# gist-ailab/QuBER

Hardware: AMD Instinct MI355X
Metric: refined masks/sec on 640x480 RGB-D (N=20 inst) (higher is better)
Workload: dtype f32; 1 GPU; batch=16 640x480 RGB-D, 20 initial instances/frame, ResNet-50 RGB-D refiner (boundary-error -> fg/centre/offset), encode+network+grouping+mask extraction; parallelism=dp1, hipgraph=False, foreground_filter=False

## Files before the change

### include/quber_hip.h

```cpp
#ifndef QUBER_HIP_H
#define QUBER_HIP_H

#include <stddef.h>
#include <stdint.h>

#ifdef __cplusplus
extern "C" {
#endif

typedef struct quber_ctx quber_ctx;

typedef struct quber_config {
    int32_t height, width;
    int32_t max_batch;
    int32_t max_instances;
    int32_t resnet_depth;
    int32_t res5_dilation;
    int32_t backbone_fusion_layers;
    int32_t head_fusion_layers;
    int32_t error_classes;
    int32_t gaussian_sigma;
    int32_t nms_kernel;
    int32_t top_k;
    int32_t stuff_area;
// ... 80 lines not shown

int quber_relabel_panoptic(quber_ctx* ctx, const float* dev_panoptic, const float* dev_labels, const int32_t* dev_count,
                           int32_t batch, int32_t mirror, int32_t* dev_ids, void* stream);
int quber_overlap_masks(quber_ctx* ctx, const uint8_t* dev_masks, const int32_t* dev_ids, int32_t batch, int32_t n_masks,
                        int32_t n_ids, uint32_t* dev_table, uint32_t* dev_area, void* stream);
int quber_overlap_ids(quber_ctx* ctx, const int32_t* dev_a, const int32_t* dev_b, int32_t batch, int32_t n_a, int32_t n_b,
                      uint32_t* dev_table, void* stream);

int quber_cleanup_ids(quber_ctx* ctx, int32_t* dev_ids, int32_t batch, int32_t n_ids, int32_t connectivity, int32_t keep_largest,
                      int32_t min_island_area, int32_t max_hole_area, uint32_t* dev_report, void* stream);
int quber_cleanup_postprocess(quber_ctx* ctx, const float* dev_logits, int32_t n_planes, int32_t batch, float* dev_panoptic,
                              const float* dev_labels, const int32_t* dev_count, float* dev_scores, float* dev_boxes,
                              int32_t connectivity, int32_t keep_largest, int32_t min_island_area, int32_t max_hole_area,
                              uint32_t* dev_report, void* stream);

int quber_perturb_masks(quber_ctx* ctx, const uint8_t* dev_masks, int32_t batch, int32_t n_masks, const int32_t* dev_programs,
                        int32_t n_ops, int32_t ops_per_round, const double* dev_iou_targets, uint8_t* dev_out, uint32_t* dev_report,
                        int32_t placement, void* stream);

int quber_mask_nms(quber_ctx* ctx, const uint8_t* dev_masks, const float* dev_scores, int32_t batch, int32_t n_masks, float thresh,
                   int32_t on_top, uint8_t* dev_out_masks, int32_t* dev_ids, int32_t* dev_source, float* dev_out_scores,
                   int32_t* dev_report, void* stream);

int quber_zoom_rois(quber_ctx* ctx, const int32_t* dev_ids, int32_t batch, int32_t n_ids, float padding, int32_t* dev_rois, void* stream);
int quber_zoom_crop(quber_ctx* ctx, const uint8_t* dev_bgr, const uint8_t* dev_depth, const int32_t* dev_ids, const int32_t* dev_slots,
                    const int32_t* dev_rois, int32_t batch, int32_t n_ids, int32_t n_slots, int32_t crop, uint8_t* dev_bgr_crop,
                    uint8_t* dev_depth_crop, uint8_t* dev_mask_crop, void* stream);
int quber_zoom_paste(quber_ctx* ctx, const int32_t* dev_crop_ids, const float* dev_crop_scores, const uint32_t* dev_table,
                     const uint32_t* dev_area, const uint8_t* dev_depth_crop, const int32_t* dev_slots, const int32_t* dev_rois,
                     int32_t batch, int32_t n_ids, int32_t n_slots, int32_t crop, int32_t n_crop_ids, float min_overlap, int32_t max_inst,
                     int32_t* dev_out_ids, uint8_t* dev_out_masks, int32_t* dev_source, float* dev_out_scores, float* dev_boxes,
                     int32_t* dev_report, void* stream);

int64_t quber_contingency_workspace_bytes(int32_t cap);
int quber_label_contingency(const int32_t* dev_pred, const int32_t* dev_gt, int64_t n_pixels, int32_t cap,
                            void* dev_workspace, void* stream);

int64_t quber_boundary_workspace_bytes(int32_t h, int32_t w, int32_t n_masks);
int quber_boundary_overlap(const int32_t* dev_pred, const int32_t* dev_gt, int32_t h, int32_t w, const int32_t* dev_labels,
                           int32_t n_pred, int32_t n_gt, int32_t bound_pix, void* dev_workspace, uint32_t* dev_out,
                           void* stream);

int64_t quber_eval_batch_workspace_bytes(int32_t batch, int32_t h, int32_t w, int32_t cap, int32_t with_boundary);
int quber_eval_batch(const int32_t* dev_pred, const int32_t* dev_gt, int32_t batch, int32_t h, int32_t w, int32_t cap, int32_t bound_pix,
                     int32_t with_boundary, int32_t placement, void* dev_workspace, void* dev_out, void* stream);
int quber_munkres_batch(const double* dev_score, const int32_t* dev_rows, const int32_t* dev_cols, int32_t batch, int32_t cap,
                        int32_t placement, void* dev_workspace, int32_t* dev_assign, int32_t* dev_status, void* stream);

int quber_foreground_filter(const float* dev_fg_logits, int32_t n_classes, int32_t fg_class, const uint8_t* dev_masks,
                            int32_t batch, int32_t n_masks, int64_t hw, uint8_t* dev_fg_mask, uint64_t* dev_counts,
                            void* stream);

int quber_normalize_depth(const void* dev_depth, int32_t is_float32, int64_t n_pixels, double min_val, double max_val,
                          uint8_t* dev_out3, uint8_t* dev_zero, void* stream);

int quber_resize_u8(const uint8_t* dev_src, int32_t src_h, int32_t src_w, int32_t channels, uint8_t* dev_dst,
                    int32_t dst_h, int32_t dst_w, int32_t linear, void* stream);

int quber_inpaint_telea_u8(const uint8_t* host_img, const uint8_t* host_mask, int32_t h, int32_t w, int32_t radius,
                           uint8_t* host_out);
int quber_inpaint_depth_u8(const uint8_t* host_depth3, int32_t h, int32_t w, int32_t kernel, uint8_t* host_out3);
int64_t quber_inpaint_depth_workspace_bytes(int32_t batch, int32_t h, int32_t w);
int quber_inpaint_depth_device(const uint8_t* dev_depth3, int32_t batch, int32_t h, int32_t w, int32_t kernel, void* dev_workspace,
                               int64_t workspace_bytes, uint8_t* dev_out3, void* stream);

int quber_debug_tensor(quber_ctx* ctx, const char* name, float** dev_ptr, int32_t* dims4, int32_t* channel_stride);
int32_t quber_debug_tensor_elem_size(quber_ctx* ctx, const char* name);
double quber_forward_flops(quber_ctx* ctx);
double quber_forward_flops_executed(quber_ctx* ctx);
double quber_forward_flops_padding(quber_ctx* ctx);
int quber_set_option(quber_ctx* ctx, int32_t key, int32_t value);
int quber_get_option(quber_ctx* ctx, int32_t key, int32_t* value);
void quber_set_tuning(int32_t key, int32_t value);
int32_t quber_debug_persistent_segments(int32_t tiles, int32_t blocks, int32_t k_slices, int32_t min_share, int32_t block,
                                        int32_t* out4, int32_t cap);
int32_t quber_debug_persistent_fixup(int32_t tiles, int32_t blocks, int32_t k_slices, int32_t min_share, int32_t xcd, int32_t j,
                                     int32_t* tile, int32_t* slots, int32_t cap);
int quber_num_ops(quber_ctx* ctx);
int quber_op_info(quber_ctx* ctx, int index, const char** name, int32_t* kind, double* flops, int32_t* launches);
int quber_op_conv2d(const float* dev_x, int32_t batch, int32_t h, int32_t w, int32_t cin, const float* dev_w_oihw,
                    int32_t cout, int32_t ksize, int32_t stride, int32_t pad, int32_t dil, const float* dev_scale,
                    const float* dev_shift, const float* dev_residual, int32_t relu, float* dev_packed_scratch,
                    float* dev_y, void* stream);
int quber_op_conv1x1_f16(const void* dev_x, int32_t batch, int32_t h, int32_t w, int32_t cin, const void* dev_w_oi,
                         int32_t cout, const float* dev_scale, const float* dev_shift, const void* dev_residual,
                         int32_t relu, void* dev_y, void* stream);
int quber_op_conv2d_f16(const void* dev_x, int32_t batch, int32_t h, int32_t w, int32_t cin, const void* dev_w_packed,
                        int32_t cout, int32_t ksize, int32_t stride, int32_t pad, int32_t dil, int32_t kmode,
                        const float* dev_scale, const float* dev_shift, const void* dev_residual, int32_t relu,
                        double* dev_gn_sums, int32_t gn_groups, void* dev_y, void* stream);
int quber_op_conv1x1_dual(const float* dev_y, const float* dev_x, int32_t batch, int32_t oh, int32_t ow, int32_t mid,
                          int32_t h2, int32_t w2, int32_t cin, int32_t stride, const float* dev_w, const float* dev_shift,
                          const float* dev_ones, int32_t cout, int32_t relu, float* dev_out, void* stream);
int quber_op_conv3x3_winograd(const float* dev_x, int32_t batch, int32_t h, int32_t w, int32_t cin,
                              const float* dev_w_oihw, int32_t cout, int32_t dil, int32_t m, const float* dev_scale,
                              const float* dev_shift,
                              int32_t relu, float* dev_u_scratch, float* dev_ws, int64_t ws_floats, float* dev_y,
                              void* stream);
int quber_op_groupnorm(const float* dev_x, int32_t batch, int32_t h, int32_t w, int32_t c, int32_t groups,
                       const float* dev_gamma, const float* dev_beta, float eps, int32_t relu,
                       double* dev_stats_scratch, float* dev_y, void* stream);
int quber_op_bilinear(const float* dev_x, int32_t batch, int32_t h, int32_t w, int32_t c, int32_t oh, int32_t ow,
                      float* dev_y, void* stream);
int quber_op_maxpool3x3s2(const float* dev_x, int32_t batch, int32_t h, int32_t w, int32_t c, float* dev_y,
                          void* stream);
int32_t quber_debug_gn_pixels_per_block(int32_t hw, int32_t c, int32_t batch, int32_t groups_of_launch, int32_t stats_pass);
int quber_op_gn_stats(const void* dev_x, int32_t x_cs, int64_t x_gs, int32_t es, int32_t batch, int32_t h, int32_t w, int32_t c,
                      int32_t groups_of_launch, int32_t groups, double* dev_stats, int32_t zero, void* stream);
int quber_op_gn_apply(const void* dev_x, int32_t x_cs, int64_t x_gs, int32_t x_es, void* dev_y, int32_t y_cs, int64_t y_gs, int32_t y_es,
                      int32_t batch, int32_t h, int32_t w, int32_t c, int32_t groups_of_launch, int32_t groups, const double* dev_stats,
                      const float* dev_gamma, const float* dev_beta, int32_t param_gs, float eps, int32_t relu, void* stream);
int quber_op_maxpool_view(const void* dev_x, int32_t x_cs, int64_t x_gs, int32_t x_es, void* dev_y, int32_t y_cs, int64_t y_gs, int32_t y_es,
                          int32_t batch, int32_t h, int32_t w, int32_t c, int32_t groups_of_launch, void* stream);
int quber_op_bilinear_view(const void* dev_x, int32_t x_cs, int32_t x_es, void* dev_y, int32_t y_cs, int32_t y_es, int32_t batch, int32_t h,
                           int32_t w, int32_t c, int32_t oh, int32_t ow, void* stream);
int quber_op_avgpool(const void* dev_x, int32_t x_cs, int32_t x_es, void* dev_y, int32_t y_cs, int32_t y_es, int32_t batch, int32_t h, int32_t w,
                     int32_t c, void* stream);
int quber_op_add_channels(const void* dev_a, int32_t a_cs, int32_t a_es, const void* dev_b, int32_t b_cs, int32_t b_es, void* dev_y, int32_t y_cs,
                          int32_t y_es, int32_t batch, int32_t h, int32_t w, int32_t c, void* stream);
int quber_op_copy_channels(const void* dev_x, int32_t x_cs, int32_t x_es, void* dev_y, int32_t y_cs, int32_t y_es, int32_t batch, int32_t h,
                           int32_t w, int32_t c, void* stream);
int quber_op_predictors(int32_t n, const void* const* dev_feat, const float* const* dev_w, const float* const* dev_bias, void* const* dev_act_dst,
                        const int32_t* cout, const int32_t* q_ch0, const int32_t* act, int32_t c, int32_t feat_cs, int32_t es, int32_t batch,
                        int32_t h, int32_t w, float* dev_q, int32_t q_nch, int32_t act_cs, void* stream);
int quber_op_upsample_logits(const float* dev_q, float* dev_out, int32_t batch, int32_t nch, int32_t h, int32_t w, int32_t scale, int32_t oh,
                             int32_t ow, uint32_t mul_mask, void* stream);
int quber_op_preprocess(const uint8_t* dev_bgr, const uint8_t* dev_depth, const float* dev_offsets, void* dev_x, int32_t x_c, int32_t es,
                        int32_t batch, int32_t batch_cap, int32_t h, int32_t w, const float* mean6, const float* std6, int32_t streams,
                        void* stream);
int quber_op_lmff_preprocess(const uint8_t* dev_bgr, const uint8_t* dev_depth, int64_t pixels, float* dev_x, void* stream);
int quber_op_lmff_dwconv(const float* dev_x, int32_t x_cs, float* dev_y, int32_t y_cs, int32_t batch, int32_t h, int32_t w, int32_t c, int32_t dil,
                         const float* dev_w9, const float* dev_scale, const float* dev_shift, const float* dev_slope, void* stream);
int quber_op_lmff_pool(const float* dev_x, int32_t x_cs, float* dev_y, int32_t y_cs, int32_t batch, int32_t h, int32_t w, int32_t c, int32_t oh,
                       int32_t ow, int32_t mode, void* stream);
int quber_op_lmff_affine(const float* dev_a, int32_t a_cs, const float* dev_b, int32_t b_cs, float* dev_y, int32_t y_cs, int32_t batch, int32_t h,
                         int32_t w, int32_t c, const float* dev_scale, const float* dev_shift, const float* dev_slope, void* stream);
int quber_op_lmff_pmca(const float* dev_x, int32_t x_cs, int32_t batch, int32_t h, int32_t w, int32_t c, const float* dev_w2x2, const float* dev_fc0,
                       const float* dev_alpha, const float* dev_fc2, float* dev_wts, double* dev_sums, void* stream);
int quber_op_lmff_scale(const float* dev_x, int32_t x_cs, const float* dev_wts, float* dev_y, int32_t y_cs, int32_t batch, int32_t h, int32_t w,
                        int32_t c, void* stream);
int quber_op_lmff_gate(const float* dev_o, int32_t o_cs, const float* dev_att, int32_t att_cs, float* dev_q, int32_t batch, int32_t h, int32_t w,
                       int32_t c, void* stream);
int quber_op_group_pixels(const float* dev_logits, int32_t n_planes, int32_t batch, int32_t h, int32_t w, int32_t cap,
                          const int32_t* dev_centers, const int32_t* dev_ncenters, uint8_t* dev_ids, uint32_t* dev_area,
                          void* stream);

#ifdef __cplusplus
}
#endif
#endif
```

### quber_amd/_lib.py

```python
import ctypes as C
import os

_HERE = os.path.dirname(os.path.abspath(__file__))
LIB_PATH = os.environ.get("QUBER_LIB") or os.path.join(_HERE, "libquber_hip.so")


class QuberConfig(C.Structure):
    _fields_ = [
        ("height", C.c_int32), ("width", C.c_int32), ("max_batch", C.c_int32), ("max_instances", C.c_int32),
        ("resnet_depth", C.c_int32), ("res5_dilation", C.c_int32), ("backbone_fusion_layers", C.c_int32),
        ("head_fusion_layers", C.c_int32), ("error_classes", C.c_int32), ("gaussian_sigma", C.c_int32),
        ("nms_kernel", C.c_int32), ("top_k", C.c_int32), ("stuff_area", C.c_int32),
        ("min_instance_area", C.c_int32), ("label_divisor", C.c_int32), ("with_network", C.c_int32),
        ("center_threshold", C.c_float), ("boundary_ratio", C.c_float),
        ("pixel_mean", C.c_float * 6), ("pixel_std", C.c_float * 6),
        ("eee_mask_on", C.c_int32), ("eee_boundary_on", C.c_int32), ("hierarchical", C.c_int32),
        ("fusion_feat", C.c_int32), ("fusion_pred", C.c_int32), ("n_levels", C.c_int32),
        ("level_heads", (C.c_int32 * 5) * 5), ("fusion_add", C.c_int32), ("streams", C.c_int32),
        ("compute_dtype", C.c_int32), ("encode_legacy_f32", C.c_int32),
        ("convs_dim", C.c_int32), ("head_channels", C.c_int32),
    ]


class QuberError(RuntimeError):
    pass


_P = C.c_void_p
_I = C.c_int32
SIGNATURES = {
    "quber_default_config": (None, [C.POINTER(QuberConfig)]),
    "quber_last_error": (C.c_char_p, []),
    "quber_version": (C.c_char_p, []),
    "quber_create": (C.c_int, [C.POINTER(QuberConfig), C.POINTER(_P)]),
    "quber_destroy": (None, [_P]),
    "quber_set_weight": (C.c_int, [_P, C.c_char_p, _P, C.c_int64]),
    "quber_finalize_weights": (C.c_int, [_P]),
    "quber_num_weights": (C.c_int, [_P]),
    "quber_weight_spec": (C.c_int, [_P, C.c_int, C.POINTER(C.c_char_p), C.POINTER(C.c_int64)]),
    "quber_encode_initial_masks": (C.c_int, [_P, _P, _I, _I, _P, _P]),
    "quber_encode_label_map": (C.c_int, [_P, _P, _I, _I, _P, _P]),
    "quber_workspace_bytes": (C.c_int64, [_P]),
    "quber_explicit_error_maps": (C.c_int, [_P, _P, _I, _P, _I, _I, _P, _P]),
    "quber_forward": (C.c_int, [_P, _P, _P, _P, _I, _P, _P]),
    "quber_forward_profiled": (C.c_int, [_P, _P, _P, _P, _I, _P, _P, C.POINTER(C.c_double * 3), C.POINTER(_I * 3)]),
    "quber_profile_begin": (C.c_int, [_P]),
    "quber_profile_end": (C.c_int, [_P, _P]),
    "quber_profile_num_stages": (C.c_int, [_P]),
    "quber_profile_stage": (C.c_int, [_P, C.c_int, C.POINTER(C.c_char_p), C.POINTER(C.c_double), C.POINTER(C.c_double),
                                      C.POINTER(C.c_double), C.POINTER(_I)]),
    "quber_postprocess": (C.c_int, [_P, _P, _I, _I, _P, _P, _P, _P, _P, _P, _P, _P]),
    "quber_extract_masks": (C.c_int, [_P, _P, _P, _I, _I, _P, _P]),
    "quber_tta_flip_inputs": (C.c_int, [_P, _P, _P, _P, _I, _I, _P]),
    "quber_tta_merge": (C.c_int, [_P, _P, _I, _I, _P, _P]),
    "quber_error_decode": (C.c_int, [_P, _P, _I, _I, _I, _I, _P, _P, _P]),
    "quber_error_mask_hist": (C.c_int, [_P, _P, _P, _I, _I, _I, _P, _P]),
    "quber_error_score": (C.c_int, [_P, _P, _P, _I, _I, _I, _I, _P, _P]),
    "quber_error_overlay": (C.c_int, [_P, _P, _P, _I, C.c_uint32, C.c_uint32, C.c_uint32, C.c_uint32, _P, _P]),
    "quber_relabel_panoptic": (C.c_int, [_P, _P, _P, _P, _I, _I, _P, _P]),
    "quber_overlap_masks": (C.c_int, [_P, _P, _P, _I, _I, _I, _P, _P, _P]),
    "quber_overlap_ids": (C.c_int, [_P, _P, _P, _I, _I, _I, _P, _P]),
    "quber_cleanup_ids": (C.c_int, [_P, _P, _I, _I, _I, _I, _I, _I, _P, _P]),
    "quber_cleanup_postprocess": (C.c_int, [_P, _P, _I, _I, _P, _P, _P, _P, _P, _I, _I, _I, _I, _P, _P]),
    "quber_perturb_masks": (C.c_int, [_P, _P, _I, _I, _P, _I, _I, _P, _P, _P, _I, _P]),
    "quber_mask_nms": (C.c_int, [_P, _P, _P, _I, _I, C.c_float, _I, _P, _P, _P, _P, _P, _P]),
    "quber_zoom_rois": (C.c_int, [_P, _P, _I, _I, C.c_float, _P, _P]),
    "quber_zoom_crop": (C.c_int, [_P, _P, _P, _P, _P, _P, _I, _I, _I, _I, _P, _P, _P, _P]),
    "quber_zoom_paste": (C.c_int, [_P, _P, _P, _P, _P, _P, _P, _P, _I, _I, _I, _I, _I, C.c_float, _I, _P, _P, _P, _P, _P, _P, _P]),
    "quber_contingency_workspace_bytes": (C.c_int64, [_I]),
    "quber_label_contingency": (C.c_int, [_P, _P, C.c_int64, _I, _P, _P]),
    "quber_boundary_workspace_bytes": (C.c_int64, [_I, _I, _I]),
    "quber_boundary_overlap": (C.c_int, [_P, _P, _I, _I, _P, _I, _I, _I, _P, _P, _P]),
    "quber_eval_batch_workspace_bytes": (C.c_int64, [_I, _I, _I, _I, _I]),
    "quber_eval_batch": (C.c_int, [_P, _P, _I, _I, _I, _I, _I, _I, _I, _P, _P, _P]),
    "quber_munkres_batch": (C.c_int, [_P, _P, _P, _I, _I, _I, _P, _P, _P, _P]),
    "quber_foreground_filter": (C.c_int, [_P, _I, _I, _P, _I, _I, C.c_int64, _P, _P, _P]),
    "quber_normalize_depth": (C.c_int, [_P, _I, C.c_int64, C.c_double, C.c_double, _P, _P, _P]),
    "quber_inpaint_telea_u8": (C.c_int, [_P, _P, _I, _I, _I, _P]),
    "quber_inpaint_depth_u8": (C.c_int, [_P, _I, _I, _I, _P]),
    "quber_inpaint_depth_workspace_bytes": (C.c_int64, [_I, _I, _I]),
    "quber_inpaint_depth_device": (C.c_int, [_P, _I, _I, _I, _I, _P, C.c_int64, _P, _P]),
    "quber_resize_u8": (C.c_int, [_P, _I, _I, _I, _P, _I, _I, _I, _P]),
    "quber_debug_tensor": (C.c_int, [_P, C.c_char_p, C.POINTER(_P), C.POINTER(_I * 4), C.POINTER(_I)]),
    "quber_debug_tensor_elem_size": (C.c_int32, [_P, C.c_char_p]),
    "quber_forward_flops": (C.c_double, [_P]),
    "quber_forward_flops_executed": (C.c_double, [_P]),
    "quber_forward_flops_padding": (C.c_double, [_P]),
    "quber_set_tuning": (None, [_I, _I]),
    "quber_set_option": (C.c_int, [_P, _I, _I]),
    "quber_get_option": (C.c_int, [_P, _I, C.POINTER(_I)]),
    "quber_num_ops": (C.c_int, [_P]),
    "quber_op_info": (C.c_int, [_P, C.c_int, C.POINTER(C.c_char_p), C.POINTER(_I), C.POINTER(C.c_double), C.POINTER(_I)]),
    "quber_debug_persistent_segments": (C.c_int32, [_I, _I, _I, _I, _I, _P, _I]),
    "quber_debug_persistent_fixup": (C.c_int32, [_I, _I, _I, _I, _I, _I, _P, _P, _I]),
    "quber_op_conv1x1_f16": (C.c_int, [_P, _I, _I, _I, _I, _P, _I, _P, _P, _P, _I, _P, _P]),
    "quber_op_conv2d_f16": (C.c_int, [_P, _I, _I, _I, _I, _P, _I, _I, _I, _I, _I, _I, _P, _P, _P, _I, _P, _I, _P, _P]),
    "quber_op_conv1x1_dual": (C.c_int, [_P, _P, _I, _I, _I, _I, _I, _I, _I, _I, _P, _P, _P, _I, _I, _P, _P]),
    "quber_op_conv2d": (C.c_int, [_P, _I, _I, _I, _I, _P, _I, _I, _I, _I, _I, _P, _P, _P, _I, _P, _P, _P]),
    "quber_op_conv3x3_winograd": (C.c_int, [_P, _I, _I, _I, _I, _P, _I, _I, _I, _P, _P, _I, _P, _P, C.c_int64, _P, _P]),
    "quber_op_groupnorm": (C.c_int, [_P, _I, _I, _I, _I, _I, _P, _P, C.c_float, _I, _P, _P, _P]),
    "quber_op_bilinear": (C.c_int, [_P, _I, _I, _I, _I, _I, _I, _P, _P]),
    "quber_op_maxpool3x3s2": (C.c_int, [_P, _I, _I, _I, _I, _P, _P]),
    "quber_debug_gn_pixels_per_block": (C.c_int32, [_I, _I, _I, _I, _I]),
    "quber_op_gn_stats": (C.c_int, [_P, _I, C.c_int64, _I, _I, _I, _I, _I, _I, _I, _P, _I, _P]),
    "quber_op_gn_apply": (C.c_int, [_P, _I, C.c_int64, _I, _P, _I, C.c_int64, _I, _I, _I, _I, _I, _I, _I, _P, _P, _P, _I, C.c_float, _I, _P]),
    "quber_op_maxpool_view": (C.c_int, [_P, _I, C.c_int64, _I, _P, _I, C.c_int64, _I, _I, _I, _I, _I, _I, _P]),
    "quber_op_bilinear_view": (C.c_int, [_P, _I, _I, _P, _I, _I, _I, _I, _I, _I, _I, _I, _P]),
    "quber_op_avgpool": (C.c_int, [_P, _I, _I, _P, _I, _I, _I, _I, _I, _I, _P]),
    "quber_op_add_channels": (C.c_int, [_P, _I, _I, _P, _I, _I, _P, _I, _I, _I, _I, _I, _I, _P]),
    "quber_op_copy_channels": (C.c_int, [_P, _I, _I, _P, _I, _I, _I, _I, _I, _I, _P]),
    "quber_op_predictors": (C.c_int, [_I, _P, _P, _P, _P, _P, _P, _P, _I, _I, _I, _I, _I, _I, _P, _I, _I, _P]),
    "quber_op_upsample_logits": (C.c_int, [_P, _P, _I, _I, _I, _I, _I, _I, _I, C.c_uint32, _P]),
    "quber_op_preprocess": (C.c_int, [_P, _P, _P, _P, _I, _I, _I, _I, _I, _I, _P, _P, _I, _P]),
    "quber_op_group_pixels": (C.c_int, [_P, _I, _I, _I, _I, _I, _P, _P, _P, _P, _P]),
    "quber_op_lmff_preprocess": (C.c_int, [_P, _P, C.c_int64, _P, _P]),
    "quber_op_lmff_dwconv": (C.c_int, [_P, _I, _P, _I, _I, _I, _I, _I, _I, _P, _P, _P, _P, _P]),
    "quber_op_lmff_pool": (C.c_int, [_P, _I, _P, _I, _I, _I, _I, _I, _I, _I, _I, _P]),
    "quber_op_lmff_affine": (C.c_int, [_P, _I, _P, _I, _P, _I, _I, _I, _I, _I, _P, _P, _P, _P]),
    "quber_op_lmff_pmca": (C.c_int, [_P, _I, _I, _I, _I, _I, _P, _P, _P, _P, _P, _P, _P]),
    "quber_op_lmff_scale": (C.c_int, [_P, _I, _P, _P, _I, _I, _I, _I, _I, _P]),
    "quber_op_lmff_gate": (C.c_int, [_P, _I, _P, _I, _P, _I, _I, _I, _I, _P]),
}

_lib = None


def load():
    global _lib
    if _lib is not None:
        return _lib
    if not os.path.exists(LIB_PATH):
        raise QuberError(
            f"{LIB_PATH} not found: build it with `make -C quber_amd/csrc` (or __graft_entry__.build()); "
            "quber_amd has no CPU fallback")
    import torch
    lib = C.CDLL(LIB_PATH)
    for name, (res, args) in SIGNATURES.items():
        fn = getattr(lib, name)
        fn.restype = res
        fn.argtypes = args
    mode = os.environ.get("QUBER_WINOGRAD", "auto").lower()
    if mode not in ("auto", "f6", "f4", "f2", "off"):
        raise QuberError(f"QUBER_WINOGRAD={mode!r}: expected auto, f6, f4, f2 or off")
    lib.quber_set_tuning(6, 1 if mode == "off" else 0)
    lib.quber_set_tuning(9, {"f2": 2, "f4": 4, "f6": 6}.get(mode, 0))
    if "QUBER_PERSIST" in os.environ:
        lib.quber_set_tuning(13, int(os.environ["QUBER_PERSIST"]))
    _lib = lib
    return lib


def check(rc):
    if rc != 0:
        raise QuberError(load().quber_last_error().decode())
```

### quber_amd/csrc/api.hip

```cpp
#include "plan.h"

#include <optional>

using namespace quber;

namespace quber { int wf_read_stamps(unsigned long long* dst, int n), h8_read_stamps(unsigned long long* dst, int n), x8_read_stamps(unsigned long long* dst, int n); }

int quber::check_cfg(const quber_config& c) {
    if (c.height <= 0 || c.width <= 0) return fail("height and width must be positive");
    if (c.with_network && (c.height < 16 || c.width < 16)) return fail("frames smaller than 16 x 16 are not supported");
    if (c.with_network == 2) {
        if (c.height % 8 || c.width % 8) return fail("LMFFNet needs height and width to be multiples of 8");
        return c.max_batch >= 1 ? 0 : fail("max_batch must be >= 1");
    }
    if (c.max_batch < 1) return fail("max_batch must be >= 1");
    if (c.max_instances < 1) return fail("max_instances must be >= 1");
    if (c.resnet_depth != 50 && c.resnet_depth != 101 && c.resnet_depth != 152) return fail("resnet_depth must be 50, 101 or 152");
    if (c.res5_dilation != 1 && c.res5_dilation != 2 && c.res5_dilation != 4) return fail("res5_dilation must be 1, 2 or 4");
    if (c.res5_dilation == 1) return fail("res5_dilation 1 (output stride 32) is not supported by this build");
    if (c.error_classes < 2 || c.error_classes > 4) return fail("error_classes must be 2..4");
    if (c.streams != 1 && c.streams != 2) return fail("streams must be 1 or 2");
    if (c.with_network == 1 && c.convs_dim != 128 && c.convs_dim != 256) return fail("convs_dim must be 128 or 256");
    if (c.with_network == 1 && c.head_channels != 32 && c.head_channels != 64) return fail("head_channels must be 32 or 64");
    if (c.compute_dtype < 0 || c.compute_dtype > 3)
// ... 186 lines not shown
#endif

int32_t quber_debug_persistent_segments(int32_t tiles, int32_t blocks, int32_t k_slices, int32_t min_share, int32_t block, int32_t* out4, int32_t cap) {
    return quber::conv_persistent_segments(tiles, blocks, k_slices, min_share, block, out4, cap);
}
int32_t quber_debug_persistent_fixup(int32_t tiles, int32_t blocks, int32_t k_slices, int32_t min_share, int32_t xcd, int32_t j, int32_t* tile, int32_t* slots, int32_t cap) {
    return quber::conv_persistent_fixup(tiles, blocks, k_slices, min_share, xcd, j, tile, slots, cap);
}

int quber_profile_begin(quber_ctx* c) {
    if (!c) return fail("null context");
    if (!c->prof) c->prof.reset(new quber::Profiler());
    c->prof->recs.clear(); c->prof->sums.clear(); c->prof->used = 0;
    quber::g_prof = c->prof.get();
    return 0;
}

int quber_profile_end(quber_ctx* c, void* stream) {
    if (!c || !c->prof || quber::g_prof != c->prof.get()) return fail("quber_profile_end without quber_profile_begin");
    quber::g_prof = nullptr;
    QB_CHECK(hipStreamSynchronize((hipStream_t)stream));
    quber::Profiler& p = *c->prof;
    p.sums.assign(p.tags.size(), quber::StageSum());
    for (size_t i = 0; i < p.tags.size(); ++i) p.sums[i].name = p.tags[i];
    for (const quber::ProfRec& r : p.recs) {
        float ms = 0.f;
        QB_CHECK(hipEventElapsedTime(&ms, r.e0, r.e1));
        quber::StageSum& s = p.sums[r.tag];
        s.ms += ms; s.bytes += r.bytes; s.flops += r.flops; s.launches += 1;
    }
    return 0;
}

int quber_profile_num_stages(quber_ctx* c) { return (c && c->prof) ? (int)c->prof->sums.size() : 0; }

int quber_profile_stage(quber_ctx* c, int i, const char** name, double* ms, double* bytes, double* flops, int32_t* launches) {
    if (!c || !c->prof || i < 0 || i >= (int)c->prof->sums.size()) return fail("stage index out of range");
    const quber::StageSum& s = c->prof->sums[i];
    *name = s.name.c_str(); *ms = s.ms; *bytes = s.bytes; *flops = s.flops; *launches = s.launches;
    return 0;
}

int quber_num_ops(quber_ctx* c) { return c ? (int)c->ops.size() : 0; }
int quber_op_info(quber_ctx* c, int i, const char** name, int32_t* kind, double* flops, int32_t* launches) {
    if (!c || i < 0 || i >= (int)c->ops.size()) return fail("op index out of range");
    const Op& o = c->ops[i];
    *name = o.name.c_str(); *kind = o.kind; *flops = o.flops; *launches = o.launches;
    return 0;
}

int quber_encode_initial_masks(quber_ctx* c, const uint8_t* masks, int32_t batch, int32_t n, float* out, void* stream) {
    if (check_batch(c, batch)) return -1;
    if (n > c->cfg.max_instances) return fail("more initial masks than max_instances");
    if (!masks && n > 0) return fail("null masks");
    return launch_encode(masks, batch, n, c->cfg.height, c->cfg.width, c->gauss, c->cfg.gaussian_sigma, c->cfg.encode_legacy_f32, c->enc_ws, out, (hipStream_t)stream);
}

int quber_encode_label_map(quber_ctx* c, const int32_t* labels, int32_t batch, int32_t n, float* out, void* stream) {
    if (check_batch(c, batch)) return -1;
    if (n > c->cfg.max_instances) return fail("more instances than max_instances");
    if (!labels && n > 0) return fail("null label map");
    return launch_encode_labels(labels, batch, n, c->cfg.height, c->cfg.width, c->gauss, c->cfg.gaussian_sigma, c->cfg.encode_legacy_f32, c->enc_ws, out, c->enc_bad, (hipStream_t)stream);
}

int64_t quber_workspace_bytes(quber_ctx* c) { return c ? (int64_t)c->alloc_bytes : 0; }

int quber_explicit_error_maps(quber_ctx* c, const uint8_t* init, int32_t n_init, const uint8_t* gt, int32_t n_gt, int32_t batch, uint8_t* out, void* stream) {
    if (check_batch(c, batch)) return -1;
    const int H = c->cfg.height, W = c->cfg.width;
    int d = (int)rint((double)c->cfg.boundary_ratio * sqrt((double)H * H + (double)W * W));
    if (d < 1) d = 1;
    return launch_errmaps(init, n_init, gt, n_gt, batch, c->cfg.max_instances > 0 ? c->cfg.max_instances : 1, H, W, d, c->err_ws, out, (hipStream_t)stream);
}

static int forward_begin(quber_ctx* c, const char* who, std::optional<quber::TuneScope>& scope, const uint8_t* bgr, const uint8_t* depth,
                         const float* offs, int batch, float* logits, bool lmff_own, bool rest_ok, const char* null_msg, hipStream_t st) {
    if (check_batch(c, batch)) return -1;
    if (!c->finalized) return fail(std::string(who) + " before quber_finalize_weights");
    scope.emplace(&c->tune);
    if (lmff_own && c->cfg.with_network == 2) return 1;
    if (!bgr || (!depth && c->cfg.streams == 2) || !offs || !logits || !rest_ok) return fail(null_msg);
    c->cur_out = logits;
    c->cur_bgr = bgr; c->cur_depth = depth; c->cur_off = offs;
    return c->stem_fused ? 0 : launch_preprocess(bgr, depth, offs, c->X, batch, c->cfg.max_batch, c->cfg.height, c->cfg.width,
                                                 c->cfg.pixel_mean, c->cfg.pixel_std, c->cfg.streams, st);
}

int quber_forward(quber_ctx* c, const uint8_t* bgr, const uint8_t* depth, const float* offs, int32_t batch, float* logits, void* stream) {
    hipStream_t st = (hipStream_t)stream;
    std::optional<quber::TuneScope> tscope;
    int rc = forward_begin(c, "quber_forward", tscope, bgr, depth, offs, batch, logits, true, true, "null tensor", st);
    if (rc == 1) {
        if (!bgr || !depth || !logits) return fail("null tensor");
        c->cur_out = logits;
        int r2 = launch_lmff_preprocess(bgr, depth, (long)batch * c->cfg.height * c->cfg.width, c->X.p, st);
        for (size_t i = 0; !r2 && i < c->ops.size(); ++i)
            if (!c->ops[i].ctl) r2 = c->ops[i].run(batch, st);
        return r2;
    }
    if (rc) return rc;
    c->lanes_on = c->lanes_built && tune().lanes && batch <= (c->cfg.compute_dtype == 0 || c->cfg.compute_dtype == 3 ? LANE_BATCH_F32 : LANE_BATCH) && c->lane_stream[1] != nullptr &&
                  quber::g_prof == nullptr;
    auto lane_used = [&](int l) { return c->lanes_on && l > 0; };
    for (auto& op : c->ops) {
        if (op.ctl == 1) {
            if (lane_used(op.lane)) {
                QB_CHECK(hipEventRecord(c->lane_fork[op.lane], st));
                QB_CHECK(hipStreamWaitEvent(c->lane_stream[op.lane], c->lane_fork[op.lane], 0));
            }
            continue;
        }
        if (op.ctl == 2) {
            if (lane_used(op.lane)) {
                QB_CHECK(hipEventRecord(c->lane_join[op.lane], c->lane_stream[op.lane]));
                QB_CHECK(hipStreamWaitEvent(st, c->lane_join[op.lane], 0));
            }
            continue;
        }
        c->lane_now = lane_used(op.lane) ? op.lane : 0;
        rc = op.run(batch, c->lane_now ? c->lane_stream[op.lane] : st);
        if (rc) return rc;
    }
    c->lane_now = 0;
    c->lanes_on = false;
    return 0;
}

int quber_forward_profiled(quber_ctx* c, const uint8_t* bgr, const uint8_t* depth, const float* offs, int32_t batch,
                           float* logits, void* stream, double* kind_ms, int32_t* kind_launches) {
    hipStream_t st = (hipStream_t)stream;
    std::optional<quber::TuneScope> tscope;
    int rc = forward_begin(c, "quber_forward_profiled", tscope, bgr, depth, offs, batch, logits, false, kind_ms && kind_launches, "null argument", st);
    if (rc) return rc;
    const size_t n = c->ops.size();
    if (c->prof_events.size() < 2 * n) {
        const size_t old = c->prof_events.size();
        c->prof_events.resize(2 * n);
        for (size_t i = old; i < 2 * n; ++i) QB_CHECK(hipEventCreate(&c->prof_events[i]));
    }
    c->lanes_on = false;
    for (size_t i = 0; i < n; ++i) {
        QB_CHECK(hipEventRecord(c->prof_events[2 * i], st));
        if (!c->ops[i].ctl) {
            rc = c->ops[i].run(batch, st);
            if (rc) return rc;
        }
        QB_CHECK(hipEventRecord(c->prof_events[2 * i + 1], st));
    }
    QB_CHECK(hipStreamSynchronize(st));
    for (int k = 0; k < OP_KINDS; ++k) { kind_ms[k] = 0.0; kind_launches[k] = 0; }
    for (size_t i = 0; i < n; ++i) {
        float ms = 0.f;
        QB_CHECK(hipEventElapsedTime(&ms, c->prof_events[2 * i], c->prof_events[2 * i + 1]));
        kind_ms[c->ops[i].kind] += ms;
        kind_launches[c->ops[i].kind] += 1;
    }
    return 0;
}

int quber_postprocess(quber_ctx* c, const float* logits, int32_t n_planes, int32_t batch, float* pan, int32_t* count,
                      float* labels, float* scores, float* boxes, int32_t* centers, int32_t* ncenters, void* stream) {
    if (check_batch(c, batch)) return -1;
    PostCfg pc;
    pc.threshold = c->cfg.center_threshold; pc.nms_kernel = c->cfg.nms_kernel; pc.top_k = c->cfg.top_k;
    pc.stuff_area = c->cfg.stuff_area; pc.min_area = c->cfg.min_instance_area; pc.label_divisor = c->cfg.label_divisor;
    pc.cap = c->cfg.top_k;
// ... 220 lines not shown
int quber_label_contingency(const int32_t* pred, const int32_t* gt, int64_t n_pixels, int32_t cap, void* workspace,
                            void* stream) {
    if (!pred || !gt || !workspace || n_pixels < 1 || cap < 1 || cap > 1024) return fail("bad argument to quber_label_contingency");
    return launch_contingency(pred, gt, n_pixels, cap, workspace, (hipStream_t)stream);
}

int64_t quber_boundary_workspace_bytes(int32_t h, int32_t w, int32_t n_masks) {
    return (int64_t)boundary_ws_bytes(h, w, n_masks);
}

int quber_boundary_overlap(const int32_t* pred, const int32_t* gt, int32_t h, int32_t w, const int32_t* labels, int32_t n_pred,
                           int32_t n_gt, int32_t bound_pix, void* workspace, uint32_t* out, void* stream) {
    if (!pred || !gt || !labels || !workspace || !out || h < 1 || w < 1) return fail("bad argument to quber_boundary_overlap");
    return launch_boundary_overlap(pred, gt, h, w, labels, n_pred, n_gt, bound_pix, workspace, out, (hipStream_t)stream);
}

int64_t quber_eval_batch_workspace_bytes(int32_t batch, int32_t h, int32_t w, int32_t cap, int32_t with_boundary) {
    if (batch < 1 || h < 1 || w < 1 || cap < 1 || cap > 256) return 0;
    return (int64_t)eval_batch_ws_bytes(batch, h, w, cap, with_boundary);
}

int quber_eval_batch(const int32_t* pred, const int32_t* gt, int32_t batch, int32_t h, int32_t w, int32_t cap, int32_t bound_pix,
                     int32_t with_boundary, int32_t placement, void* workspace, void* out, void* stream) {
    if (!pred || !gt || !workspace || !out) return fail("quber_eval_batch: null pointer");
    if (((uintptr_t)pred & 3) || ((uintptr_t)gt & 3) || ((uintptr_t)workspace & 7) || ((uintptr_t)out & 7))
        return fail("quber_eval_batch: label maps must be 4-byte aligned, workspace and out 8-byte aligned");
    return launch_eval_batch(pred, gt, batch, h, w, cap, bound_pix, with_boundary, placement, workspace, out, (hipStream_t)stream);
}

int quber_munkres_batch(const double* score, const int32_t* rows, const int32_t* cols, int32_t batch, int32_t cap, int32_t placement,
                        void* workspace, int32_t* assign, int32_t* status, void* stream) {
    if (!score || !rows || !cols || !assign || !status) return fail("quber_munkres_batch: null pointer");
    if (((uintptr_t)score & 7) || ((uintptr_t)workspace & 7) || ((uintptr_t)rows & 3) || ((uintptr_t)cols & 3) || ((uintptr_t)assign & 3) ||
        ((uintptr_t)status & 3))
        return fail("quber_munkres_batch: misaligned pointer");
    return launch_munkres_batch(score, rows, cols, batch, cap, placement, reinterpret_cast<double*>(workspace), assign, cap, status, 1,
                                (hipStream_t)stream);
}

int quber_foreground_filter(const float* fg_logits, int32_t n_classes, int32_t fg_class, const uint8_t* masks,
                            int32_t batch, int32_t n_masks, int64_t hw, uint8_t* fg_mask, uint64_t* counts, void* stream) {
    if (!fg_logits || !fg_mask || batch < 1 || hw < 1 || n_classes < 2) return fail("bad argument to quber_foreground_filter");
    if (n_masks < 0 || n_masks > 65535) return fail("quber_foreground_filter: n_masks outside 0..65535");
    hipStream_t st = (hipStream_t)stream;
    int rc = launch_argmax_fg(fg_logits, batch, hw, n_classes, fg_class, fg_mask, st);
    if (rc || n_masks == 0) return rc;
    if (!masks || !counts) return fail("null masks / counts");
    return launch_mask_overlap(masks, fg_mask, batch, n_masks, hw, (unsigned long long*)counts, st);
}

int quber_normalize_depth(const void* depth, int32_t is_float32, int64_t n_pixels, double min_val, double max_val,
                          uint8_t* out3, uint8_t* zero, void* stream) {
    if (!depth || !out3 || n_pixels <= 0) return fail("bad argument to quber_normalize_depth");
    if (!(max_val > min_val)) return fail("normalize_depth: max_val must exceed min_val");
    return launch_normalize_depth(depth, is_float32, n_pixels, min_val, max_val, out3, zero, (hipStream_t)stream);
}

int quber_inpaint_telea_u8(const uint8_t* host_img, const uint8_t* host_mask, int32_t h, int32_t w, int32_t radius,
                           uint8_t* host_out) {
    return inpaint_telea_u8_host(host_img, host_mask, h, w, radius, host_out);
}

int quber_inpaint_depth_u8(const uint8_t* host_depth3, int32_t h, int32_t w, int32_t kernel, uint8_t* host_out3) {
    return inpaint_depth_u8_host(host_depth3, h, w, kernel, host_out3);
}

int64_t quber_inpaint_depth_workspace_bytes(int32_t batch, int32_t h, int32_t w) { return (int64_t)inpaint_depth_ws_bytes(batch, h, w); }

int quber_inpaint_depth_device(const uint8_t* dev_depth3, int32_t batch, int32_t h, int32_t w, int32_t kernel, void* dev_workspace,
                               int64_t workspace_bytes, uint8_t* dev_out3, void* stream) {
    return launch_inpaint_depth(dev_depth3, batch, h, w, kernel, dev_workspace, (size_t)workspace_bytes, dev_out3, (hipStream_t)stream);
}

int quber_resize_u8(const uint8_t* src, int32_t src_h, int32_t src_w, int32_t channels, uint8_t* dst, int32_t dst_h,
                    int32_t dst_w, int32_t linear, void* stream) {
    if (!src || !dst) return fail("bad argument to quber_resize_u8");
    return launch_resize_u8(src, src_h, src_w, channels, dst, dst_h, dst_w, linear, (hipStream_t)stream);
}

int quber_debug_tensor(quber_ctx* c, const char* name, float** ptr, int32_t* dims4, int32_t* cs) {
    if (!c || !name) return fail("null argument");
    auto it = c->taps.find(name);
    if (it == c->taps.end()) return fail(std::string("no intermediate named '") + name + "'");
    *ptr = it->second.p;
    dims4[0] = it->second.B; dims4[1] = it->second.H; dims4[2] = it->second.W; dims4[3] = it->second.C;
    *cs = it->second.cs;
    return 0;
}
int32_t quber_debug_tensor_elem_size(quber_ctx* c, const char* name) {
    if (!c || !name) return 0;
    auto it = c->taps.find(name);
    return it == c->taps.end() ? 0 : it->second.es;
}

}
```

### quber_amd/csrc/api_ops.hip

```cpp
#include "plan.h"

using namespace quber;

static float* g_op_ws = nullptr;
static int g_op_skip_rows = 0;
static int g_op_bf16 = 0;
static const size_t g_op_ws_floats = (size_t)256 << 20;
static int g_op_wino_reuse = 0;

bool quber::op_set_tuning(int key, int value) {
    if (key == 2) {
        if (value && !g_op_ws) {
            if (hipMalloc((void**)&g_op_ws, sizeof(float) * g_op_ws_floats) != hipSuccess) g_op_ws = nullptr;
        } else if (!value && g_op_ws) {
            (void)hipFree(g_op_ws);
            g_op_ws = nullptr;
        }
        return true;
    }
    if (key == 26) { g_op_wino_reuse = value; return true; }
    if (key == 12) { g_op_bf16 = value; return true; }
    if (key == 11) { g_op_skip_rows = value; return true; }
    return false;
}

static void conv_geometry(ConvP& p, int B, int h, int w, int cin, int cout, int k, int stride, int pad, int dil) {
    p.B = B; p.H = h; p.W = w; p.Cin = cin; p.in_cs = cin;
    p.OH = (h + 2 * pad - dil * (k - 1) - 1) / stride + 1;
    p.OW = (w + 2 * pad - dil * (k - 1) - 1) / stride + 1;
    p.Cout = cout; p.out_cs = cout; p.K = k * k * cin;
    p.kh = k; p.kw = k; p.stride = stride; p.pad = pad; p.dil = dil;
    p.M = B * p.OH * p.OW; p.ohw = p.OH * p.OW;
}

struct PlaneScratch {
    void* planes = nullptr;
    size_t cap = 0;
    int split(const float* w, long n, ConvP& p, const char* who, hipStream_t st) {
        const size_t need = (size_t)n * 3 * sizeof(unsigned short);
        if (need > cap) {
            if (planes) (void)hipFree(planes);
            planes = nullptr; cap = 0;
            if (hipMalloc(&planes, need) != hipSuccess) return fail(std::string(who) + ": cannot allocate the bf16x3 weight planes");
            cap = need;
        }
        const int rc = launch_split_bf16x3(w, n, planes, st);
        if (rc) return rc;
        p.w3 = planes; p.w3_plane = n;
        return 0;
    }
};

static View mkview(const float* p, int B, int h, int w, int c) {
    View v;
    v.p = const_cast<float*>(p); v.B = B; v.H = h; v.W = w; v.C = c; v.cs = c; v.gs = 0;
    return v;
}

extern "C" {

__global__ void pack_oihw_kernel(const float* __restrict__ w, int O, int I, int k, int Kpad, int kmode, float* __restrict__ out) {
    const long total = (long)O * Kpad;
    for (long i = blockIdx.x * (long)blockDim.x + threadIdx.x; i < total; i += (long)gridDim.x * blockDim.x) {
        const int o = i / Kpad, kk = i % Kpad;
        float v = 0.f;
        if (kk < k * k * I) {
            int tap, ci;
            if (kmode) {
                const int cb = kk / (k * k * 32), rem = kk % (k * k * 32);
                tap = rem / 32;
                ci = cb * 32 + rem % 32;
            } else {
                tap = kk / I;
                ci = kk % I;
            }
            v = w[((long)o * I + ci) * k * k + tap];
        }
        out[i] = v;
    }
}

int quber_op_conv2d(const float* x, int32_t B, int32_t h, int32_t w, int32_t cin, const float* w_oihw, int32_t cout, int32_t k, int32_t stride, int32_t pad, int32_t dil,
                    const float* scale, const float* shift, const float* residual, int32_t relu, float* packed, float* y, void* stream) {
    hipStream_t st = (hipStream_t)stream;
    const int Kpad = (k * k * cin + 31) / 32 * 32;
    const bool skip_rows = g_op_skip_rows && k == 3 && stride == 1 && dil > 1 && cin % 32 == 0;
    const int kmode = (k > 1 && cin % 32 == 0 && !skip_rows) ? 1 : 0;
    hipLaunchKernelGGL(pack_oihw_kernel, dim3(256), dim3(256), 0, st, w_oihw, cout, cin, k, Kpad, kmode, packed);
    ConvP p{};
    p.in = x; p.w = packed; p.scale = scale; p.shift = shift; p.res = residual; p.out = y;
    conv_geometry(p, B, h, w, cin, cout, k, stride, pad, dil);
    p.res_cs = cout; p.Kpad = Kpad; p.relu = relu;
    p.kmode = kmode; p.skip_rows = skip_rows;
    p.bf16 = g_op_bf16; p.w_gs = 0; p.ss_gs = 0;
    p.ws = g_op_ws; p.ws_floats = g_op_ws ? g_op_ws_floats : 0;
    if (g_op_bf16 == 3 && k == 1 && tune().x8) {
        static PlaneScratch scratch;
        const int rc = scratch.split(packed, (long)cout * Kpad, p, "conv2d", st);
        if (rc) return rc;
    }
    return launch_conv(p, 1, st);
}

int quber_op_conv1x1_f16(const void* x, int32_t B, int32_t h, int32_t w, int32_t cin, const void* w_oi, int32_t cout,
                         const float* scale, const float* shift, const void* residual, int32_t relu, void* y, void* stream) {
    if (cin % 64) return fail("conv1x1_f16: cin must be a multiple of 64");
    ConvP p{};
    p.in = (const float*)x; p.w = (const float*)w_oi; p.scale = scale; p.shift = shift; p.res = (const float*)residual; p.out = (float*)y;
    conv_geometry(p, B, h, w, cin, cout, 1, 1, 0, 1);
    p.res_cs = cout; p.Kpad = cin; p.relu = relu;
    p.bf16 = 2; p.es = 2;
    return launch_conv(p, 1, (hipStream_t)stream);
}

int quber_op_conv2d_f16(const void* x, int32_t B, int32_t h, int32_t w, int32_t cin, const void* w_packed, int32_t cout, int32_t ksize, int32_t stride, int32_t pad, int32_t dil,
                        int32_t kmode, const float* scale, const float* shift, const void* residual, int32_t relu, double* gn_sums, int32_t gn_groups, void* y, void* stream) {
    if (cin % 8 || (kmode && cin % 64)) return fail("conv2d_f16: cin must be a multiple of 8 (slice-major K order: of 64)");
    if (ksize < 1 || stride < 1 || dil < 1 || pad < 0) return fail("conv2d_f16: bad geometry");
    ConvP p{};
    p.in = (const float*)x; p.w = (const float*)w_packed; p.scale = scale; p.shift = shift; p.res = (const float*)residual; p.out = (float*)y;
    conv_geometry(p, B, h, w, cin, cout, ksize, stride, pad, dil);
    if (p.OH < 1 || p.OW < 1) return fail("conv2d_f16: empty output");
    p.res_cs = cout; p.Kpad = (p.K + 63) / 64 * 64; p.relu = relu;
    p.kmode = kmode; p.bf16 = 2; p.es = 2;
    p.w_gs = (long)cout * p.Kpad; p.ss_gs = cout;
    if (gn_sums) {
        if (gn_groups < 1 || cout % gn_groups) return fail("conv2d_f16: channels must divide into the norm groups");
        p.gn_sum = gn_sums; p.gn_groups = gn_groups; p.gn_cpg = cout / gn_groups;
    }
    return launch_conv(p, 1, (hipStream_t)stream);
}

int quber_op_conv1x1_dual(const float* y, const float* x, int32_t B, int32_t oh, int32_t ow, int32_t mid, int32_t h2, int32_t w2, int32_t cin, int32_t stride,
                          const float* w, const float* shift, const float* ones, int32_t cout, int32_t relu, float* out, void* stream) {
    ConvP p{};
    p.in = y; p.in2 = x; p.w = w; p.scale = ones; p.shift = shift; p.out = out;
    conv_geometry(p, B, oh, ow, mid, cout, 1, 1, 0, 1);
    p.H2 = h2; p.W2 = w2; p.in2_cs = cin; p.stride2 = stride; p.K1 = mid;
    p.K = mid + cin; p.Kpad = mid + cin; p.relu = relu;
    p.bf16 = g_op_bf16; p.ss_gs = 0;
    p.ws = g_op_ws; p.ws_floats = g_op_ws ? g_op_ws_floats : 0;
    if (g_op_bf16 == 3 && tune().x8) {
        static PlaneScratch scratch;
        const int rs = scratch.split(w, (long)cout * p.Kpad, p, "conv1x1_dual", (hipStream_t)stream);
        if (rs) return rs;
    }
    const int rc = launch_conv_dual(p, 1, (hipStream_t)stream);
    if (rc == 1) return fail("conv1x1_dual: launch not covered by the dual kernel (workspace: tuning key 2)");
    return rc;
}

int quber_op_conv3x3_winograd(const float* x, int32_t B, int32_t h, int32_t w, int32_t cin, const float* w_oihw, int32_t cout, int32_t dil, int32_t m,
                              const float* scale, const float* shift, int32_t relu, float* u, float* ws, int64_t ws_floats, float* y, void* stream) {
    hipStream_t st = (hipStream_t)stream;
    if (!winograd_eligible(3, 1, dil, dil, cin, cout)) return fail("winograd: unsupported channel counts");
    if ((scale == nullptr) != (shift == nullptr)) return fail("winograd: scale and shift go together");
    if (m != 2 && m != 4 && m != 6) return fail("winograd: the output tile edge is 2, 4 or 6");
    int rc = g_op_wino_reuse ? 0 : launch_winograd_weights(w_oihw, cout, cin, m, u, st);
    if (rc) return rc;
    WinoP q{};
    q.in = mkview(x, B, h, w, cin); q.out = mkview(y, B, h, w, cout);
    q.u = u; q.scale = scale; q.shift = shift; q.ss_gs = 0; q.relu = relu; q.dil = dil; q.m = m;
    q.dtype = g_op_bf16;
    q.pack = tune().wino_pack;
    q.ws = ws; q.ws_floats = (size_t)ws_floats;
    if (m == 4 && tune().wino_fused && cout % 32 == 0 && (size_t)ws_floats >= (size_t)36 * cout * cin) {
        q.uf = ws;
        if (winograd_fused_ok(q, B, 1)) {
            rc = winograd_fused_prepare();
            if (rc) return rc;
            rc = g_op_wino_reuse ? 0 : launch_winograd_fused_pack(u, cout, cin, ws, st);
            if (rc) return rc;
            q.ws = ws + (size_t)36 * cout * cin; q.ws_floats = (size_t)ws_floats - (size_t)36 * cout * cin;
        } else {
            q.uf = nullptr;
        }
    }
    q.splitk_ws = g_op_ws; q.splitk_floats = g_op_ws ? g_op_ws_floats : 0;
    return launch_conv_winograd(q, B, 1, st);
}

int quber_op_groupnorm(const float* x, int32_t B, int32_t h, int32_t w, int32_t c, int32_t groups, const float* gamma,
                       const float* beta, float eps, int32_t relu, double* stats, float* y, void* stream) {
    View in = mkview(x, B, h, w, c), out = mkview(y, B, h, w, c);
    int rc = launch_gn_stats(in, B, 1, groups, stats, (hipStream_t)stream);
    if (rc) return rc;
    return launch_gn_apply(in, out, B, 1, groups, stats, gamma, beta, 0, eps, relu, (hipStream_t)stream);
}

int quber_op_bilinear(const float* x, int32_t B, int32_t h, int32_t w, int32_t c, int32_t oh, int32_t ow, float* y,
                      void* stream) {
    if (c % 4) return fail("bilinear: channels must be a multiple of 4");
    return launch_bilinear(mkview(x, B, h, w, c), mkview(y, B, oh, ow, c), B, (hipStream_t)stream);
}

static View opview(const void* p, int B, int h, int w, int c, int cs, long gs, int es) {
    View v;
    v.p = reinterpret_cast<float*>(const_cast<void*>(p)); v.B = B; v.H = h; v.W = w; v.C = c; v.cs = cs; v.gs = gs; v.es = es;
    return v;
}

int32_t quber_debug_gn_pixels_per_block(int32_t hw, int32_t c, int32_t batch, int32_t groups_of_launch, int32_t stats_pass) {
    return gn_pixels_per_block(hw, c, batch, groups_of_launch, stats_pass != 0);
}

int quber_op_gn_stats(const void* x, int32_t x_cs, int64_t x_gs, int32_t es, int32_t B, int32_t h, int32_t w, int32_t c, int32_t G, int32_t groups,
                      double* stats, int32_t zero, void* stream) {
    return launch_gn_stats(opview(x, B, h, w, c, x_cs, x_gs, es), B, G, groups, stats, (hipStream_t)stream, zero != 0);
}

int quber_op_gn_apply(const void* x, int32_t x_cs, int64_t x_gs, int32_t x_es, void* y, int32_t y_cs, int64_t y_gs, int32_t y_es, int32_t B, int32_t h,
                      int32_t w, int32_t c, int32_t G, int32_t groups, const double* stats, const float* gamma, const float* beta, int32_t param_gs,
                      float eps, int32_t relu, void* stream) {
    return launch_gn_apply(opview(x, B, h, w, c, x_cs, x_gs, x_es), opview(y, B, h, w, c, y_cs, y_gs, y_es), B, G, groups, stats, gamma, beta,
                           param_gs, eps, relu, (hipStream_t)stream);
}

int quber_op_maxpool_view(const void* x, int32_t x_cs, int64_t x_gs, int32_t x_es, void* y, int32_t y_cs, int64_t y_gs, int32_t y_es, int32_t B,
                          int32_t h, int32_t w, int32_t c, int32_t G, void* stream) {
    return launch_maxpool3x3s2(opview(x, B, h, w, c, x_cs, x_gs, x_es), opview(y, B, (h + 1) / 2, (w + 1) / 2, c, y_cs, y_gs, y_es), B, G,
                               (hipStream_t)stream);
}

int quber_op_bilinear_view(const void* x, int32_t x_cs, int32_t x_es, void* y, int32_t y_cs, int32_t y_es, int32_t B, int32_t h, int32_t w, int32_t c,
                           int32_t oh, int32_t ow, void* stream) {
    return launch_bilinear(opview(x, B, h, w, c, x_cs, 0, x_es), opview(y, B, oh, ow, c, y_cs, 0, y_es), B, (hipStream_t)stream);
}

int quber_op_avgpool(const void* x, int32_t x_cs, int32_t x_es, void* y, int32_t y_cs, int32_t y_es, int32_t B, int32_t h, int32_t w, int32_t c,
                     void* stream) {
    return launch_avgpool(opview(x, B, h, w, c, x_cs, 0, x_es), opview(y, B, 1, 1, c, y_cs, 0, y_es), B, (hipStream_t)stream);
}

int quber_op_add_channels(const void* a, int32_t a_cs, int32_t a_es, const void* b, int32_t b_cs, int32_t b_es, void* y, int32_t y_cs, int32_t y_es,
                          int32_t B, int32_t h, int32_t w, int32_t c, void* stream) {
    return launch_add_channels(opview(a, B, h, w, c, a_cs, 0, a_es), opview(b, B, h, w, c, b_cs, 0, b_es), opview(y, B, h, w, c, y_cs, 0, y_es), B,
                               (hipStream_t)stream);
}

int quber_op_copy_channels(const void* x, int32_t x_cs, int32_t x_es, void* y, int32_t y_cs, int32_t y_es, int32_t B, int32_t h, int32_t w, int32_t c,
                           void* stream) {
    return launch_copy_channels(opview(x, B, h, w, c, x_cs, 0, x_es), opview(y, B, h, w, c, y_cs, 0, y_es), B, (hipStream_t)stream);
}

int quber_op_predictors(int32_t n, const void* const* feat, const float* const* w, const float* const* bias, void* const* act_dst, const int32_t* cout,
                        const int32_t* q_ch0, const int32_t* act, int32_t c, int32_t feat_cs, int32_t es, int32_t B, int32_t h, int32_t wd, float* q,
                        int32_t q_nch, int32_t act_cs, void* stream) {
    PredHeads hs{};
    hs.n = n;
    for (int j = 0; j < n && j < 5; ++j) {
        hs.in[j] = feat[j]; hs.w[j] = w[j]; hs.bias[j] = bias[j]; hs.sm[j] = act_dst[j];
        hs.cout[j] = cout[j]; hs.q_ch0[j] = q_ch0[j]; hs.act[j] = act[j];
    }
    return launch_predictors(hs, c, feat_cs, es, h, wd, q, q_nch, act_cs, B, (hipStream_t)stream);
}

int quber_op_upsample_logits(const float* q, float* out, int32_t B, int32_t nch, int32_t h, int32_t w, int32_t scale, int32_t oh, int32_t ow,
                             uint32_t mul_mask, void* stream) {
    return launch_upsample_logits(q, out, B, nch, h, w, scale, oh, ow, mul_mask, (hipStream_t)stream);
}

int quber_op_preprocess(const uint8_t* rgb, const uint8_t* depth, const float* offs, void* x, int32_t x_c, int32_t es, int32_t B, int32_t batch_cap,
                        int32_t h, int32_t w, const float* mean6, const float* std6, int32_t streams, void* stream) {
    return launch_preprocess(rgb, depth, offs, opview(x, batch_cap, h, w, x_c, x_c, (long)batch_cap * h * w * x_c, es), B, batch_cap, h, w, mean6,
                             std6, streams, (hipStream_t)stream);
}

int quber_op_group_pixels(const float* logits, int32_t n_planes, int32_t batch, int32_t h, int32_t w, int32_t cap,
                          const int32_t* centers, const int32_t* ncenters, uint8_t* ids, uint32_t* area, void* stream) {
    if (!logits || !centers || !ncenters || !ids || !area || batch < 1 || h < 1 || w < 1) return fail("bad argument to quber_op_group_pixels");
    return launch_group_pixels(logits, n_planes, batch, h, w, cap, centers, ncenters, ids, area, (hipStream_t)stream);
}

static View lview(const void* p, int B, int h, int w, int c, int cs) { return opview(p, B, h, w, c, cs, 0, 4); }

int quber_op_lmff_preprocess(const uint8_t* bgr, const uint8_t* depth, int64_t pixels, float* x, void* stream) {
    return launch_lmff_preprocess(bgr, depth, (long)pixels, x, (hipStream_t)stream);
}

int quber_op_lmff_dwconv(const float* x, int32_t x_cs, float* y, int32_t y_cs, int32_t B, int32_t h, int32_t w, int32_t c, int32_t dil, const float* w9,
                         const float* scale, const float* shift, const float* slope, void* stream) {
    return launch_dwconv3x3(lview(x, B, h, w, c, x_cs), lview(y, B, h, w, c, y_cs), B, dil, w9, scale, shift, slope, (hipStream_t)stream);
}

int quber_op_lmff_pool(const float* x, int32_t x_cs, float* y, int32_t y_cs, int32_t B, int32_t h, int32_t w, int32_t c, int32_t oh, int32_t ow, int32_t mode,
                       void* stream) {
    return launch_pool_s2(lview(x, B, h, w, c, x_cs), lview(y, B, oh, ow, c, y_cs), B, mode, (hipStream_t)stream);
}

int quber_op_lmff_affine(const float* a, int32_t a_cs, const float* b, int32_t b_cs, float* y, int32_t y_cs, int32_t B, int32_t h, int32_t w, int32_t c,
                         const float* scale, const float* shift, const float* slope, void* stream) {
    const View bv = lview(b, B, h, w, c, b_cs);
    return launch_affine_prelu(lview(a, B, h, w, c, a_cs), b ? &bv : nullptr, lview(y, B, h, w, c, y_cs), B, scale, shift, slope, (hipStream_t)stream);
}

int quber_op_lmff_pmca(const float* x, int32_t x_cs, int32_t B, int32_t h, int32_t w, int32_t c, const float* w2x2, const float* fc0, const float* alpha,
                       const float* fc2, float* wts, double* sums, void* stream) {
    return launch_pmca(lview(x, B, h, w, c, x_cs), B, w2x2, fc0, alpha, fc2, wts, sums, (hipStream_t)stream);
}

int quber_op_lmff_scale(const float* x, int32_t x_cs, const float* wts, float* y, int32_t y_cs, int32_t B, int32_t h, int32_t w, int32_t c, void* stream) {
    return launch_scale_channels(lview(x, B, h, w, c, x_cs), wts, lview(y, B, h, w, c, y_cs), B, (hipStream_t)stream);
}

int quber_op_lmff_gate(const float* o, int32_t o_cs, const float* att, int32_t att_cs, float* q, int32_t B, int32_t h, int32_t w, int32_t c, void* stream) {
    return launch_mad_gate(lview(o, B, h, w, c, o_cs), lview(att, B, h, w, c, att_cs), q, B, c, (hipStream_t)stream);
}

int quber_op_maxpool3x3s2(const float* x, int32_t B, int32_t h, int32_t w, int32_t c, float* y, void* stream) {
    if (c % 4) return fail("maxpool: channels must be a multiple of 4");
    return launch_maxpool3x3s2(mkview(x, B, h, w, c), mkview(y, B, (h + 1) / 2, (w + 1) / 2, c), B, 1, (hipStream_t)stream);
}

}
```

### quber_amd/csrc/common.h

```cpp
#pragma once
#include <hip/hip_runtime.h>
#include <stdint.h>
#include <string>

namespace quber {

struct View {
    float* p = nullptr;
    int B = 0, H = 0, W = 0, C = 0;
    int cs = 0;
    long gs = 0;
    int es = 4;
    float* at(long elems) const { return p ? reinterpret_cast<float*>(reinterpret_cast<char*>(p) + elems * es) : nullptr; }
};

struct ConvP {
    const float* in;
    const float* w;
    const float* scale;
    const float* shift;
    const float* res;
    const float* prelu;
    float* out;
    int B, H, W, Cin, in_cs;
// ... 51 lines not shown
};

struct WinoNorm {
    const double* stats;
    const float* gamma;
    const float* beta;
    int groups, cpg, param_gs, relu;
    double n;
    float eps;
};

struct WinoP {
    View in, out;
    const float* u;
    const void* u3;
    long u3_plane;
    const float* uf;
    int algo;
    const float* scale;
    const float* shift;
    int ss_gs, relu;
    int dil;
    int m;
    int pack;
    int dtype;
    double* gn_sum;
    int gn_groups;
    WinoNorm norm;
    float* ws;
    size_t ws_floats;
    float* splitk_ws;
    size_t splitk_floats;
};

int launch_conv(const ConvP& p, int G, hipStream_t st);
int launch_conv_winograd(const WinoP& q, int B, int G, hipStream_t st);
int launch_winograd_weights(const float* w_oihw, int Cout, int Cin, int m, float* u, hipStream_t st);
void winograd_weights_host(const float* w_oihw, int Cout, int Cin, int m, float* u);
bool winograd_eligible(int k, int stride, int pad, int dil, int Cin, int Cout);
bool winograd_m6_channels_ok(int Cin, int Cout);
size_t winograd_ws_floats(int B, int H, int W, int Cin, int Cout, int G, int dil, int m);
double winograd_mac_ratio(int H, int W, int dil, int m);
double winograd_mac_ratio_run(int H, int W, int dil, int m, bool pack);
bool winograd_fused_ok(const WinoP& q, int B, int G);
int launch_conv_winograd_fused(const WinoP& q, int B, int G, hipStream_t st);
void winograd_fused_pack_host(const float* u, int Cout, int Cin, float* uf);
int launch_winograd_fused_pack(const float* u, int Cout, int Cin, float* uf, hipStream_t st);
size_t winograd_fused_ws_floats(int B, int Cin, int G);
int winograd_fused_prepare();

struct Tuning {
    int winograd = 0;
    int wino_min_cin = 32;
    int wino_max_ratio = 67;
    int wino_variant = 0;
    int wino_min_cout = 32;
    int wino_pairs = 0;
    int wino_chunk_mb = 0;
    int wino_pack = 1;
    int wino_fused = 1;
    int wino_fused_max_cin = 160;
    int acc_chunk = 2;
    int tile_128x64 = 1;
    int force_tile = 0;
    int force_split = 0;
    int tail_split = 1;
    int persist = 1;
    int persist_min_nk = 32;
    int persist_min_tiles = 256;
    int persist_debug = 0;
    int stem_fused = 1;
    int lean_loader = 1;
    int fuse_shortcut = 1;
    int lanes = 1;
    int h8 = 1;
    int x8 = 1;
    int x8_min_nk = 8;
    int x8_min_rounds = 2;
    int zone_cols = 1;
    int small_n_64 = 1;
    int aspp_lanes = 1;
    int h8_narrow = 1;
    int h8_norm = 1;
    int h8_min_tiles = 224;
};
extern Tuning g_tune;
extern thread_local const Tuning* t_tune;
inline const Tuning& tune() { return t_tune ? *t_tune : g_tune; }
struct TuneScope {
    const Tuning* prev;
    explicit TuneScope(const Tuning* t) : prev(t_tune) { t_tune = t; }
    ~TuneScope() { t_tune = prev; }
    TuneScope(const TuneScope&) = delete;
    TuneScope& operator=(const TuneScope&) = delete;
};
bool tuning_set(Tuning& t, int key, int value);
template <int BM, int BN, int WM, int WN> int launch_conv_persistent(ConvP p, int G, int bpc, hipStream_t st);
size_t conv_persistent_ws_floats(int BM, int BN, int bpc);
bool conv_persistent_ok(const ConvP& p);
int conv_persistent_segments(int T, int P, int nk, int min_slices, int bid, int* out4, int cap);
int conv_persistent_fixup(int T, int P, int nk, int min_slices, int xcd, int j, int* tile, int* slots, int cap);
int launch_conv_dual(ConvP p, int G, hipStream_t st);
bool conv_h8_patch_takes(const ConvP& p, int G, bool norm);
int launch_conv_x8(ConvP p, int G, hipStream_t st);
int launch_split_bf16x3(const float* w, long n, void* planes, hipStream_t st);
int launch_conv_h8(ConvP p, int G, hipStream_t st);
#ifdef PK_STAMPS
int pk_read_stamps(unsigned long long* dst, int n);
int pk_read_span(unsigned long long* dst, int n);
#endif
int launch_preprocess(const uint8_t* rgb, const uint8_t* depth, const float* offs, const View& x, int B, int Bcap,
                      int H, int W, const float* mean6, const float* std6, int streams, hipStream_t st);
int launch_maxpool3x3s2(const View& in, const View& out, int B, int G, hipStream_t st);
int launch_stem_conv1(const uint8_t* bgr, const uint8_t* depth, const float* offs, int B, int H, int W, int streams, const float* mean6,
                      const float* std6, const float* w, const float* scale, const float* shift, float* out, long out_gs, int es, hipStream_t st,
                      const void* wf16 = nullptr);
int launch_zero(void* p, size_t bytes, hipStream_t st);
int launch_gn_stats(const View& in, int B, int G, int groups, double* stats, hipStream_t st, bool zero = true);
int gn_pixels_per_block(int HW, int C, int B, int G, bool stats = false);
int launch_gn_apply(const View& in, const View& out, int B, int G, int groups, const double* stats,
                    const float* gamma, const float* beta, int param_gs, float eps, int relu, hipStream_t st);
int launch_bilinear(const View& in, const View& out, int B, hipStream_t st);
int launch_avgpool(const View& in, const View& out, int B, hipStream_t st);
struct PredHeads { int n; const void* in[5]; const float* w[5]; const float* bias[5]; void* sm[5]; int cout[5], q_ch0[5], act[5] ; };
int launch_predictors(const PredHeads& hs, int C, int in_cs, int es, int H, int W, float* q, int q_nch, int sm_cs, int B, hipStream_t st);
int launch_copy_channels(const View& in, const View& out, int B, hipStream_t st);
int launch_add_channels(const View& a, const View& b, const View& out, int B, hipStream_t st);
int launch_upsample_logits(const float* q, float* out, int B, int nch, int h, int w, int scale, int OH, int OW,
                           unsigned mul_mask, hipStream_t st);

int launch_normalize_depth(const void* depth, int is_float, long n, double lo, double hi, uint8_t* out3, uint8_t* zero,
                           hipStream_t st);

int inpaint_telea_u8_host(const uint8_t* img, const uint8_t* mask, int H, int W, int radius, uint8_t* out);
int inpaint_depth_u8_host(const uint8_t* depth3, int H, int W, int kernel, uint8_t* out3);
size_t inpaint_depth_ws_bytes(int B, int H, int W);
int launch_inpaint_depth(const uint8_t* depth3, int B, int H, int W, int kernel, void* ws, size_t ws_bytes, uint8_t* out3, hipStream_t st);
int launch_resize_u8(const uint8_t* src, int sh, int sw, int ch, uint8_t* dst, int dh, int dw, int linear, hipStream_t st);

int launch_lmff_preprocess(const uint8_t* bgr, const uint8_t* depth, long pixels, float* x, hipStream_t st);
int launch_dwconv3x3(const View& in, const View& out, int B, int dil, const float* w9, const float* scale,
                     const float* shift, const float* slope, hipStream_t st);
int launch_pool_s2(const View& in, const View& out, int B, int mode , hipStream_t st);
int launch_affine_prelu(const View& a, const View* b, const View& out, int B, const float* scale, const float* shift,
                        const float* slope, hipStream_t st);
int launch_pmca(const View& x, int B, const float* w2x2, const float* fc0, const float* alpha, const float* fc2, float* wts,
                double* sums , hipStream_t st);
int launch_scale_channels(const View& in, const float* wts, const View& out, int B, hipStream_t st);
int launch_mad_gate(const View& o, const View& att, float* q, int B, int C, hipStream_t st);
int launch_argmax_fg(const float* logits, int B, long HW, int nc, int cls, uint8_t* fg, hipStream_t st);
int launch_mask_overlap(const uint8_t* masks, const uint8_t* fg, int B, int K, long HW, unsigned long long* counts,
                        hipStream_t st);

int launch_boundary_overlap(const int* pred, const int* gt, int H, int W, const int* labels, int n_pred, int n_gt, int radius,
                            void* ws, unsigned* out, hipStream_t st);
size_t boundary_ws_bytes(int H, int W, int n_masks);
int launch_contingency(const int* pred, const int* gt, long n, int cap, void* ws, hipStream_t st);
size_t contingency_ws_bytes(int cap);
int launch_eval_batch(const int* pred, const int* gt, int batch, int H, int W, int cap, int radius, int with_boundary, int placement, void* ws,
                      void* out, hipStream_t st);
size_t eval_batch_ws_bytes(int batch, int H, int W, int cap, int with_boundary);
size_t eval_batch_out_bytes(int batch, int cap);
int launch_munkres_batch(const double* score, const int* rows, const int* cols, int batch, int cap, int placement, double* mat, int* assign,
                         long assign_stride, int* status, long status_stride, hipStream_t st);

int launch_encode(const uint8_t* masks, int B, int N, int H, int W, const float* gauss, int sigma, int legacy_f32,
                  void* ws, float* out, hipStream_t st);
int launch_encode_labels(const int* labels, int B, int N, int H, int W, const float* gauss, int sigma, int legacy_f32, void* ws,
                         float* out, int* bad, hipStream_t st);
size_t encode_ws_bytes(int B, int N, int H, int W);

int launch_errmaps(const uint8_t* init, int N, const uint8_t* gt, int Ng, int B, int Nmax, int H, int W, int d,
                   uint8_t* ws, uint8_t* out, hipStream_t st);
size_t errmaps_ws_bytes(int B, int Nmax, int H, int W);

struct InstStat {
    double prob;
    unsigned long long sy, sx;
    unsigned cnt;
    int xmin, ymin, xmax, ymax;
    int pad;
};
int launch_post_finalize(const float* logits, int nch, int B, int H, int W, int cap, const int* count, const InstStat* stats, float* scores,
                         float* boxes, hipStream_t st);
int launch_post_paint_finalize(const float* logits, int nch, int B, int H, int W, int cap, int label_divisor, const int* ids, const float* lut,
                               const int* count, float* pan, InstStat* stats, float* scores, float* boxes, hipStream_t st);
struct PostCfg {
    float threshold;
    int nms_kernel, top_k, stuff_area, min_area, label_divisor, cap;
};
int launch_postprocess(const float* logits, int nch, int B, int H, int W, const PostCfg& c, void* ws,
                       float* pan, int* count, float* labels, float* scores, float* boxes, int* centers,
                       int* ncenters, hipStream_t st);
size_t postprocess_ws_bytes(int B, int H, int W, int cap);
int launch_extract_masks(const float* pan, const float* labels, int B, int H, int W, int cap, int max_inst,
                         uint8_t* out, hipStream_t st);
int launch_tta_flip_u8(const uint8_t* src, uint8_t* dst, long planes, int H, int W, int C, hipStream_t st);
int launch_tta_merge(const float* logits2, int planes, int B, int H, int W, float* out, hipStream_t st);
int launch_error_decode(const float* logits, int n_planes, int first_plane, int classes, int B, int H, int W, uint8_t* cls,
                        unsigned* hist, hipStream_t st);
int launch_error_mask_hist(const uint8_t* cls, const uint8_t* masks, int B, int N, int classes, int H, int W, unsigned* out,
                           hipStream_t st);
int launch_error_score(const uint8_t* cls, const uint8_t* expl, int kind, int error_type, int classes, int B, int H, int W,
                       unsigned long long* table, hipStream_t st);
int launch_error_overlay(const uint8_t* bgr, const uint8_t* cls, int B, int H, int W, const unsigned* colors, uint8_t* out,
                         hipStream_t st);
int launch_relabel_panoptic(const float* pan, const float* labels, const int* count, int B, int top_k, int mirror, int H, int W,
// ... 38 lines not shown
```

### quber_amd/csrc/conv_igemm.hip

```cpp
#include "common.h"

namespace quber {

using f32x16 = __attribute__((ext_vector_type(16))) float;
using f32x4 = __attribute__((ext_vector_type(4))) float;

constexpr int BK = 32;
constexpr int PITCH = 36;
template <int DT> struct Half16 { using T = __bf16; };
template <> struct Half16<2> { using T = _Float16; };
template <> struct Half16<4> { using T = _Float16; };
constexpr int PITCH_H = 40;
constexpr int NPL(int dt) { return dt == 3 ? 3 : 1; }

#ifndef QB_H16_NBUF
#define QB_H16_NBUF 1
#endif
#ifndef QB_H16_OCC
#define QB_H16_OCC 3
#endif
#ifndef QB_F32_LEAN64_OCC
#define QB_F32_LEAN64_OCC 7
#endif
#ifndef QB_H16_LEAN64_OCC
#define QB_H16_LEAN64_OCC 8
#endif
#ifndef QB_H16_LEAN_OCC
#define QB_H16_LEAN_OCC 4
#endif
constexpr int igemm_occupancy(int BM, int BN, int DT = 0, bool LEAN = false) {
    if (DT == 4 && LEAN && BM == 128 && BN == 128) return QB_H16_LEAN_OCC;
    if (DT == 0 && LEAN && BM == 64 && BN == 64) return QB_F32_LEAN64_OCC;
    if (DT == 4 && BM * BN >= 128 * 128) return QB_H16_OCC;
    if (DT == 4 && LEAN && BM == 64 && BN == 64) return QB_H16_LEAN64_OCC;
    if (DT == 4 && BM == 64 && BN == 64) return 7;
    if (BM * BN >= 128 * 128 || (BM == 256 && DT == 3)) return 2;
    return BM == 64 ? (DT == 0 ? 6 : 5) : 3;
}

using u32x4 = __attribute__((ext_vector_type(4))) unsigned;

__device__ __forceinline__ void zone_pixel_of(const ConvP& p, int b, int rem, int& oy, int& ox) {
    if (b & 1) rem = p.ohw - 1 - rem;
    const int nA = p.zx1 * p.OH, nAB = p.zx2 * p.OH;
    const int zb = rem < nA ? 0 : rem < nAB ? nA : nAB;
    const int c0 = rem < nA ? 0 : rem < nAB ? p.zx1 : p.zx2;
    const int zw = rem < nA ? p.zx1 : rem < nAB ? p.zx2 - p.zx1 : p.OW - p.zx2;
    oy = (rem - zb) / zw;
    ox = c0 + (rem - zb) - oy * zw;
    if (rem >= nA && rem < nAB) oy = p.OH - 1 - oy;
}
__device__ __forceinline__ long zone_row_of(const ConvP& p, long m) {
    const int b = (int)(m / p.ohw), rem = (int)(m - (long)b * p.ohw);
    int oy, ox;
    zone_pixel_of(p, b, rem, oy, ox);
    return (long)b * p.ohw + oy * p.OW + ox;
}

template <int BM, int BN, int WM, int WN, int MODE, int DT = 0, bool LEAN = false>
__global__ __launch_bounds__(WM * WN * 64) __attribute__((amdgpu_waves_per_eu(igemm_occupancy(BM, BN, DT, LEAN)))) void conv_igemm_f32(const ConvP p) {
    constexpr int NTH = WM * WN * 64;
    constexpr int RPP = NTH / 8;
    constexpr int TM = BM / WM / 32;
    constexpr int TN = BN / WN / 32;
    constexpr int AL = BM / RPP;
    constexpr int BL = BN / RPP;
    constexpr int NBUF = ((DT == 0 || (DT == 4 && QB_H16_NBUF == 2)) && BM == 128 && BN == 128) ? 2 : 1;
    constexpr bool RAW = DT == 0 || DT == 4;
    static_assert(BM % RPP == 0 && BN % RPP == 0, "loader geometry");
    constexpr int SW = WN * 32;
    constexpr int SP = SW + 4;
    constexpr int KSLICE_FLOATS = !RAW ? NPL(DT) * NBUF * (BM + BN) * PITCH_H / 2 : NBUF * (BM + BN) * PITCH;
    constexpr int SMEM_FLOATS = KSLICE_FLOATS > BM * SP ? KSLICE_FLOATS : BM * SP;
    __shared__ __attribute__((aligned(16))) float smem[SMEM_FLOATS];
    float* const As = smem;
    float* const Bs = smem + NBUF * BM * PITCH;
    using H16 = typename Half16<DT>::T;
    using h16x8 = __attribute__((ext_vector_type(8))) H16;
    using h16x4 = __attribute__((ext_vector_type(4))) H16;
    H16* const Ah = reinterpret_cast<H16*>(smem);
    H16* const Bh = Ah + NPL(DT) * NBUF * BM * PITCH_H;

    const int t = threadIdx.x;
    const int g = blockIdx.z;

    int tile, part = 0;
    bool raw = MODE == 1 || MODE == 4;
    {
        const int bid = blockIdx.x, nblk = MODE == 2 ? p.nfull : gridDim.x;
        const int xcd = bid & 7, q = nblk >> 3, r = nblk & 7;
        tile = (xcd < r ? xcd * (q + 1) : r * (q + 1) + (xcd - r) * q) + (bid >> 3);
        if constexpr (MODE == 1 || MODE == 4) part = blockIdx.y;
        if constexpr (MODE == 2) {
            if (bid >= nblk) {
                const int u = bid - nblk;
                tile = nblk + (u >> p.tail_shift);
                part = u & ((1 << p.tail_shift) - 1);
                raw = true;
            }
        }
    }
    const int nt = tile % p.ntiles;
    const int mt = tile / p.ntiles;
    const int m0 = mt * BM, n0 = nt * BN;

    int k_begin = 0, nk = p.Kpad / BK;
    if (MODE == 1 || (MODE == 2 && raw)) {
        k_begin = part * p.kchunk;
        nk = min(nk - k_begin, p.kchunk);
    }
    constexpr bool ZON = (MODE == 3 || MODE == 4) && LEAN && DT == 0;
    int kx_lo = 0, kx_hi = 0, row_skip = 0, z_nA = 0, z_nAB = 0;
    bool zon = false;
    if constexpr (ZON) {
        zon = p.zones != 0;
        kx_hi = p.kw - 1;
        z_nA = p.zx1 * p.OH;
        z_nAB = p.zx2 * p.OH;
    }
    auto zone_pixel = [&](int b, int rem, int& oy, int& ox) __attribute__((always_inline)) { zone_pixel_of(p, b, rem, oy, ox); };
    if constexpr (MODE == 3 || MODE == 4) {
        const int rem0 = m0 % p.ohw;
        const int last = min(m0 + BM, p.M) - 1;
        const int rem1 = last % p.ohw;
        const bool one_image = m0 / p.ohw == last / p.ohw;
        int oy_min = one_image ? rem0 / p.OW : 0;
        int oy_hi = one_image ? rem1 / p.OW : p.OH - 1;
        if (ZON && zon) {
            oy_min = p.OH - 1; oy_hi = 0;
            kx_lo = 2; kx_hi = 0;
            for (int m = m0; m <= last;) {
                const int b = m / p.ohw, rem = m - b * p.ohw;
                const int rf = (b & 1) ? p.ohw - 1 - rem : rem;
                const int z = rf < z_nA ? 0 : rf < z_nAB ? 1 : 2;
                const int zs = z == 0 ? 0 : z == 1 ? z_nA : z_nAB, ze = z == 0 ? z_nA : z == 1 ? z_nAB : p.ohw;
                const int left = (b & 1) ? rf - zs + 1 : ze - rf;
                const int len = min(left, last - m + 1);
                int ya, yb, x;
                zone_pixel(b, rem, ya, x);
                zone_pixel(b, rem + len - 1, yb, x);
                oy_min = min(oy_min, min(ya, yb)); oy_hi = max(oy_hi, max(ya, yb));
                const int lo = z == 0 ? 1 : z == 2 ? 0 : (p.zones == 1 ? 0 : 1);
                const int hi = z == 0 ? 2 : z == 2 ? 1 : (p.zones == 1 ? 2 : 1);
// ... 4 lines not shown
        int ky_lo = 0, ky_hi = p.kh - 1;
        while (ky_lo < ky_hi && oy_hi * p.stride - p.pad + ky_lo * p.dil < 0) ++ky_lo;
        while (ky_hi > ky_lo && oy_min * p.stride - p.pad + ky_hi * p.dil >= p.H) --ky_hi;
        const int cpt = p.Cin / BK;
        const int per_row = p.kw * cpt;
        k_begin = ky_lo * per_row;
        nk = (ky_hi - ky_lo + 1) * per_row;
        if (ZON && zon) {
            k_begin += kx_lo * cpt;
            nk = (ky_hi - ky_lo + 1) * (kx_hi - kx_lo + 1) * cpt;
            row_skip = (p.kw - (kx_hi - kx_lo + 1)) * cpt;
        }
        if constexpr (MODE == 4) {
            const int chunk = (nk + (int)gridDim.y - 1) / (int)gridDim.y;
            const int done = min(part * chunk, nk);
            if (ZON && zon) {
                const int rowlen = (kx_hi - kx_lo + 1) * cpt;
                const int r = done / rowlen, w = done - r * rowlen;
                k_begin += r * per_row + w;
            } else {
                k_begin += done;
            }
            nk = min(nk - done, chunk);
            if (nk == 0) k_begin = ky_lo * per_row;
        }
    }
    const float* __restrict__ in = p.in + (long)g * p.in_gs;
    const float* __restrict__ wt = p.w + (long)g * p.w_gs + (long)k_begin * BK;

    const int kq = (t & 7) * 4;
    const int lrow = t >> 3;
    int iy0[AL], ix0[AL];
    const float* rowp[AL];
#pragma unroll
    for (int i = 0; i < AL; ++i) {
        const int m = m0 + lrow + RPP * i;
        if (m < p.M && p.kh == 1 && p.stride == 1 && p.pad == 0) {
            iy0[i] = 0;
            ix0[i] = 0;
            rowp[i] = in + (long)m * p.in_cs;
        } else if (m < p.M) {
            const int ohw = p.OH * p.OW;
            const int b = m / ohw;
            const int rem = m - b * ohw;
            const int oy = rem / p.OW;
            const int ox = rem - oy * p.OW;
            iy0[i] = oy * p.stride - p.pad;
            ix0[i] = ox * p.stride - p.pad;
            rowp[i] = in + ((long)b * p.H * p.W + (long)iy0[i] * p.W + ix0[i]) * p.in_cs;
        } else {
            iy0[i] = -(1 << 28);
            ix0[i] = 0;
            rowp[i] = in;
        }
    }
    const float* wrow[BL];
#pragma unroll
    for (int i = 0; i < BL; ++i) {
        const int n = n0 + lrow + RPP * i;
        wrow[i] = wt + (long)(n < p.Cout ? n : 0) * p.Kpad + kq;
    }
    int kc, kx, ky;
    if (p.kmode) {
        kc = kq; kx = 0; ky = 0;
        if (MODE != 0) {
            const int taps = p.kh * p.kw;
            const int cb = k_begin / taps, tap = k_begin - cb * taps;
            kc = cb * BK + kq;
            ky = tap / p.kw;
            kx = tap - ky * p.kw;
        }
    } else {
        const int k = k_begin * BK + kq;
        const int tap = k / p.Cin;
        kc = k - tap * p.Cin;
        ky = tap / p.kw;
        kx = tap - ky * p.kw;
    }

    int aoff[AL], boff[BL];
    unsigned amask[AL];
    int skc = 0, skx = 0, sky = 0;
    int swk = 0;
    __amdgpu_buffer_rsrc_t rsa, rsb;
    if constexpr (LEAN) {
#pragma unroll
        for (int i = 0; i < AL; ++i) {
            const int m = m0 + lrow + RPP * i;
            aoff[i] = 0;
            amask[i] = 0;
            if (m < p.M && p.kh == 1 && p.stride == 1 && p.pad == 0) {
                aoff[i] = (m * p.in_cs + kq) * 4;
                amask[i] = 1;
            } else if (m < p.M) {
                const int ohw = p.OH * p.OW;
                const int b = m / ohw;
                const int rem = m - b * ohw;
                int oy = rem / p.OW;
                int ox = rem - oy * p.OW;
                if (ZON && zon) zone_pixel(b, rem, oy, ox);
                const int y0 = oy * p.stride - p.pad, x0 = ox * p.stride - p.pad;
                aoff[i] = (((b * p.H + y0) * p.W + x0) * p.in_cs + kq) * 4;
                unsigned xbits = 0, mk = 0;
                for (int tx = 0; tx < p.kw; ++tx)
                    if ((unsigned)(x0 + tx * p.dil) < (unsigned)p.W) xbits |= 1u << tx;
                for (int ty = 0; ty < p.kh; ++ty)
                    if ((unsigned)(y0 + ty * p.dil) < (unsigned)p.H) mk |= xbits << (ty * p.kw);
                amask[i] = mk;
            }
        }
#pragma unroll
        for (int i = 0; i < BL; ++i) {
            const int n = n0 + lrow + RPP * i;
            boff[i] = ((n < p.Cout ? n : 0) * p.Kpad + kq) * 4;
        }
        {
            const int kb = __builtin_amdgcn_readfirstlane(k_begin);
            if (p.kmode) {
                const int taps = p.kh * p.kw;
                const int cb = kb / taps, tap = kb - cb * taps;
                skc = cb * BK;
                sky = tap / p.kw;
                skx = tap - sky * p.kw;
            } else {
                const int k = kb * BK;
                const int tap = k / p.Cin;
                skc = k - tap * p.Cin;
                sky = tap / p.kw;
                skx = tap - sky * p.kw;
            }
            skc = __builtin_amdgcn_readfirstlane(skc); skx = __builtin_amdgcn_readfirstlane(skx); sky = __builtin_amdgcn_readfirstlane(sky);
        }
        rsa = __builtin_amdgcn_make_buffer_rsrc(const_cast<float*>(in), 0, p.lean_in_bytes, 0x00020000);
        rsb = __builtin_amdgcn_make_buffer_rsrc(const_cast<float*>(wt), 0, 0x7ffffff0, 0x00020000);
    }

    f32x4 ra[AL], rb[BL];
    bool aok[AL];
    auto gload = [&](int kt) __attribute__((always_inline)) {
        if constexpr (LEAN) {
            const int tap = sky * p.kw + skx;
            const int soff = (((sky * p.dil) * p.W + skx * p.dil) * p.in_cs + skc) * 4;
#pragma unroll
            for (int i = 0; i < AL; ++i) {
                const bool ok = (amask[i] >> tap) & 1u;
                aok[i] = true;
                const u32x4 v = __builtin_amdgcn_raw_buffer_load_b128(rsa, ok ? aoff[i] + soff : (int)0x80000000, 0, 0);
                ra[i] = __builtin_bit_cast(f32x4, v);
            }
            const int wso = (ZON ? swk : kt) * BK * 4;
#pragma unroll
            for (int i = 0; i < BL; ++i) rb[i] = __builtin_bit_cast(f32x4, __builtin_amdgcn_raw_buffer_load_b128(rsb, boff[i], wso, 0));
            if (p.kmode) {
                if (++skx == p.kw) {
                    skx = 0;
                    if (++sky == p.kh) { sky = 0; skc += BK; }
                }
            } else {
                skc += BK;
                if constexpr (ZON) ++swk;
                if (skc >= p.Cin) {
                    skc = 0;
                    if constexpr (ZON) {
                        if (++skx > kx_hi) { skx = kx_lo; ++sky; swk += row_skip; }
                    } else {
                        if (++skx == p.kw) { skx = 0; ++sky; }
                    }
                }
            }
            return;
        }
        const bool kok = p.kmode || ky < p.kh;
        const int dy = ky * p.dil, dx = kx * p.dil;
        const long off = ((long)dy * p.W + dx) * p.in_cs + kc;
#pragma unroll
        for (int i = 0; i < AL; ++i) {
            const bool ok = kok && (unsigned)(iy0[i] + dy) < (unsigned)p.H && (unsigned)(ix0[i] + dx) < (unsigned)p.W;
            aok[i] = ok;
            ra[i] = *reinterpret_cast<const f32x4*>(ok ? rowp[i] + off : in);
        }
#pragma unroll
        for (int i = 0; i < BL; ++i) rb[i] = *reinterpret_cast<const f32x4*>(wrow[i] + kt * BK);
        if (p.kmode) {
            if (++kx == p.kw) {
                kx = 0;
                if (++ky == p.kh) { ky = 0; kc += BK; }
            }
        } else {
            kc += BK;
#pragma unroll
            for (int it = 0; it < BK / 8; ++it) {
                if (kc >= p.Cin) {
                    kc -= p.Cin;
                    if (++kx == p.kw) { kx = 0; ++ky; }
                }
            }
        }
    };
    auto lstore = [&](int buf) __attribute__((always_inline)) {
        if constexpr (DT == 3) {
            auto split = [&](const f32x4 v, H16* dst, int plane_stride) __attribute__((always_inline)) {
                h16x4 p1, p2, p3;
#pragma unroll
                for (int e = 0; e < 4; ++e) {
                    const float x = v[e];
                    const H16 x1 = (H16)x;
                    const float r1 = x - (float)x1;
                    const H16 x2 = (H16)r1;
                    const float r2 = r1 - (float)x2;
                    p1[e] = x1; p2[e] = x2; p3[e] = (H16)r2;
                }
                *reinterpret_cast<h16x4*>(dst) = p1;
                *reinterpret_cast<h16x4*>(dst + plane_stride) = p2;
                *reinterpret_cast<h16x4*>(dst + 2 * plane_stride) = p3;
            };
#pragma unroll
            for (int i = 0; i < AL; ++i)
                split((LEAN || aok[i]) ? ra[i] : f32x4{0.f, 0.f, 0.f, 0.f}, &Ah[(lrow + RPP * i) * PITCH_H + kq], BM * PITCH_H);
#pragma unroll
            for (int i = 0; i < BL; ++i) split(rb[i], &Bh[(lrow + RPP * i) * PITCH_H + kq], BN * PITCH_H);
            return;
        }
        if constexpr (!RAW) {
#pragma unroll
            for (int i = 0; i < AL; ++i) {
                const f32x4 v = (LEAN || aok[i]) ? ra[i] : f32x4{0.f, 0.f, 0.f, 0.f};
                *reinterpret_cast<h16x4*>(&Ah[buf * BM * PITCH_H + (lrow + RPP * i) * PITCH_H + kq]) =
                    h16x4{(H16)v.x, (H16)v.y, (H16)v.z, (H16)v.w};
            }
#pragma unroll
            for (int i = 0; i < BL; ++i)
                *reinterpret_cast<h16x4*>(&Bh[buf * BN * PITCH_H + (lrow + RPP * i) * PITCH_H + kq]) =
                    h16x4{(H16)rb[i].x, (H16)rb[i].y, (H16)rb[i].z, (H16)rb[i].w};
            return;
        }
#pragma unroll
        for (int i = 0; i < AL; ++i)
            *reinterpret_cast<f32x4*>(&As[buf * BM * PITCH + (lrow + RPP * i) * PITCH + kq]) =
                (LEAN || aok[i]) ? ra[i] : f32x4{0.f, 0.f, 0.f, 0.f};
#pragma unroll
        for (int i = 0; i < BL; ++i)
            *reinterpret_cast<f32x4*>(&Bs[buf * BN * PITCH + (lrow + RPP * i) * PITCH + kq]) = rb[i];
    };

    const int wave = t >> 6, lane = t & 63;
    const int wm = wave / WN, wn = wave % WN;
    const int r = lane & 31, h = lane >> 5;

    f32x16 acc[TM][TN];
#pragma unroll
    for (int i = 0; i < TM; ++i)
#pragma unroll
        for (int j = 0; j < TN; ++j)
#pragma unroll
            for (int e = 0; e < 16; ++e) acc[i][j][e] = 0.f;

    auto mma_h = [&](int buf, int ks) __attribute__((always_inline)) {
        const H16* ap = &Ah[buf * BM * PITCH_H + (wm * TM * 32 + r) * PITCH_H + 8 * h + ks * 16];
        const H16* bp = &Bh[buf * BN * PITCH_H + (wn * 32 + r) * PITCH_H + 8 * h + ks * 16];
        h16x8 a[TM], b[TN];
#pragma unroll
        for (int i = 0; i < TM; ++i) a[i] = *reinterpret_cast<const h16x8*>(ap + i * 32 * PITCH_H);
#pragma unroll
        for (int j = 0; j < TN; ++j) b[j] = *reinterpret_cast<const h16x8*>(bp + j * WN * 32 * PITCH_H);
#pragma unroll
        for (int i = 0; i < TM; ++i)
#pragma unroll
            for (int j = 0; j < TN; ++j) {
                if constexpr (DT == 2) acc[i][j] = __builtin_amdgcn_mfma_f32_32x32x16_f16(a[i], b[j], acc[i][j], 0, 0, 0);
                else acc[i][j] = __builtin_amdgcn_mfma_f32_32x32x16_bf16(a[i], b[j], acc[i][j], 0, 0, 0);
            }
    };
    auto mma_raw16 = [&](int buf, int ks) __attribute__((always_inline)) {
        const H16* ap = reinterpret_cast<const H16*>(&As[buf * BM * PITCH + (wm * TM * 32 + r) * PITCH]) + 8 * h + ks * 16;
        const H16* bp = reinterpret_cast<const H16*>(&Bs[buf * BN * PITCH + (wn * 32 + r) * PITCH]) + 8 * h + ks * 16;
        h16x8 a[TM], b[TN];
#pragma unroll
        for (int i = 0; i < TM; ++i) a[i] = *reinterpret_cast<const h16x8*>(ap + i * 32 * 2 * PITCH);
#pragma unroll
        for (int j = 0; j < TN; ++j) b[j] = *reinterpret_cast<const h16x8*>(bp + j * WN * 32 * 2 * PITCH);
#pragma unroll
        for (int i = 0; i < TM; ++i)
#pragma unroll
            for (int j = 0; j < TN; ++j) acc[i][j] = __builtin_amdgcn_mfma_f32_32x32x16_f16(a[i], b[j], acc[i][j], 0, 0, 0);
    };
    auto mma_x3 = [&](int ks) __attribute__((always_inline)) {
        const H16* ap = &Ah[(wm * TM * 32 + r) * PITCH_H + 8 * h + ks * 16];
        const H16* bp = &Bh[(wn * 32 + r) * PITCH_H + 8 * h + ks * 16];
        h16x8 a[3][TM], b[3][TN];
#pragma unroll
        for (int q = 0; q < 3; ++q) {
#pragma unroll
            for (int i = 0; i < TM; ++i) a[q][i] = *reinterpret_cast<const h16x8*>(ap + q * BM * PITCH_H + i * 32 * PITCH_H);
#pragma unroll
            for (int j = 0; j < TN; ++j) b[q][j] = *reinterpret_cast<const h16x8*>(bp + q * BN * PITCH_H + j * WN * 32 * PITCH_H);
        }
#pragma unroll
        for (int i = 0; i < TM; ++i)
#pragma unroll
            for (int j = 0; j < TN; ++j) {
                f32x16 c = acc[i][j];
                c = __builtin_amdgcn_mfma_f32_32x32x16_bf16(a[2][i], b[0][j], c, 0, 0, 0);
                c = __builtin_amdgcn_mfma_f32_32x32x16_bf16(a[0][i], b[2][j], c, 0, 0, 0);
                c = __builtin_amdgcn_mfma_f32_32x32x16_bf16(a[1][i], b[1][j], c, 0, 0, 0);
                c = __builtin_amdgcn_mfma_f32_32x32x16_bf16(a[1][i], b[0][j], c, 0, 0, 0);
                c = __builtin_amdgcn_mfma_f32_32x32x16_bf16(a[0][i], b[1][j], c, 0, 0, 0);
                c = __builtin_amdgcn_mfma_f32_32x32x16_bf16(a[0][i], b[0][j], c, 0, 0, 0);
                acc[i][j] = c;
            }
    };
    const f32x16 zero16 = {0.f, 0.f, 0.f, 0.f, 0.f, 0.f, 0.f, 0.f, 0.f, 0.f, 0.f, 0.f, 0.f, 0.f, 0.f, 0.f};
    auto mma = [&](int buf, int ks) __attribute__((always_inline)) {
        const float* ap = &As[buf * BM * PITCH + (wm * TM * 32 + r) * PITCH + 4 * h];
        const float* bp = &Bs[buf * BN * PITCH + (wn * 32 + r) * PITCH + 4 * h];
        f32x4 a[TM], b[TN];
#pragma unroll
        for (int i = 0; i < TM; ++i) a[i] = *reinterpret_cast<const f32x4*>(ap + i * 32 * PITCH + ks * 8);
#pragma unroll
        for (int j = 0; j < TN; ++j) b[j] = *reinterpret_cast<const f32x4*>(bp + j * WN * 32 * PITCH + ks * 8);
#pragma unroll
        for (int i = 0; i < TM; ++i)
#pragma unroll
// ... 348 lines not shown
        if (scale) { sc = *reinterpret_cast<const vec*>(scale + n); sh = *reinterpret_cast<const vec*>(shift + n); }
        if (prelu) sl = *reinterpret_cast<const vec*>(prelu + n);
        if (res) rr = *reinterpret_cast<const vec*>(res + pm * p.res_cs + n);
        const float* const w0 = p.ws + (long)g * MN + i;
        const long sstep = (long)G * MN;
        vec v = *reinterpret_cast<const vec*>(w0);
        int s = 1;
        for (; s + 3 < S; s += 4) {
            const vec a = *reinterpret_cast<const vec*>(w0 + s * sstep), b = *reinterpret_cast<const vec*>(w0 + (s + 1) * sstep);
            const vec c = *reinterpret_cast<const vec*>(w0 + (s + 2) * sstep), d = *reinterpret_cast<const vec*>(w0 + (s + 3) * sstep);
            v += a; v += b; v += c; v += d;
        }
        for (; s < S; ++s) v += *reinterpret_cast<const vec*>(w0 + s * sstep);
        float o[V];
#pragma unroll
        for (int e = 0; e < V; ++e) {
            float x = V == 1 ? v[0] : v[e];
            if (scale) x = fmaf(x, V == 1 ? sc[0] : sc[e], V == 1 ? sh[0] : sh[e]);
            if (res) x += V == 1 ? rr[0] : rr[e];
            if (p.relu) x = fmaxf(x, 0.f);
            if (prelu) x = x > 0.f ? x : x * (V == 1 ? sl[0] : sl[e]);
            o[e] = x;
        }
        if constexpr (V == 4) {
            *reinterpret_cast<vec*>(out + pm * p.out_cs + n) = vec{o[0], o[1], o[2], o[3]};
            if (gn) {
                const double a = (double)o[0] + (double)o[1] + (double)o[2] + (double)o[3];
                const double b = (double)o[0] * o[0] + (double)o[1] * o[1] + (double)o[2] * o[2] + (double)o[3] * o[3];
                const int slot = (m < m_next ? 0 : 64) + (n / p.gn_cpg) * 2;
                atomicAdd(&gacc[slot], a);
                atomicAdd(&gacc[slot + 1], b);
            }
        } else {
            out[pm * p.out_cs + n] = o[0];
        }
    }
    if (gn) {
        __syncthreads();
        if (threadIdx.x < 128) {
            const double v = gacc[threadIdx.x];
            const int b = b0 + (threadIdx.x >> 6);
            if (v != 0.0 && b < p.B)
                atomicAdd(&p.gn_sum[(((long)g * p.B + b) * p.gn_groups) * 2 + (threadIdx.x & 63)], v);
        }
    }
}


struct SplitModel { double c, thr1, thr2, per_float, lat; };
constexpr SplitModel kModel3 = {3.9, 0.74, 0.995, 1.09e-7, 13.7};
constexpr SplitModel kModel7 = {7.5, 0.0, 0.0, 6.05e-7, 40.0};
constexpr int kMinSlicesPerSplit = 6;

static double launch_cost(long blocks, int nk, double outputs, int S, int bpc, const SplitModel& m) {
    const long per_cu = (blocks * S + 255) / 256;
    const long q = per_cu / bpc, rem = per_cu % bpc;
    double W = (double)bpc * q;
    if (rem) W += bpc <= 3 ? (rem == 1 ? 1.0 / m.thr1 : 2.0 / m.thr2) : (rem > 0.55 * bpc ? (double)rem : 0.55 * bpc);
    double t = ((double)nk / S + m.c) * W;
    if (S > 1) t += m.lat + (2.0 * S + 1.0) * outputs * m.per_float;
    return t;
}

static int choose_split(const ConvP& p, int G, int BM, int BN, int bpc) {
    const int nk = p.Kpad / BK;
    if (!p.ws) return 1;
    const long blocks = (long)((p.M + BM - 1) / BM) * ((p.Cout + BN - 1) / BN) * G;
    const double outputs = (double)G * p.M * p.Cout;
    const SplitModel& m = bpc <= 3 ? kModel3 : kModel7;
    int best = 1;
    double best_t = launch_cost(blocks, nk, outputs, 1, bpc, m);
    for (int S = 2; S <= 16 && nk / S >= kMinSlicesPerSplit; ++S) {
        if ((double)S * outputs > (double)p.ws_floats) break;
        const double t = launch_cost(blocks, nk, outputs, S, bpc, m);
        if (t < 0.97 * best_t) { best_t = t; best = S; }
    }
    return best;
}

template <int BM, int BN, int WM, int WN, int MODE, int DT>
static void launch_igemm(bool lean, dim3 grid, dim3 block, hipStream_t st, const ConvP& p) {
    if (lean) hipLaunchKernelGGL((conv_igemm_f32<BM, BN, WM, WN, MODE, DT, true>), grid, block, 0, st, p);
    else hipLaunchKernelGGL((conv_igemm_f32<BM, BN, WM, WN, MODE, DT, false>), grid, block, 0, st, p);
}

static bool lean_loader(ConvP& p) {
    if (!tune().lean_loader || p.in2) return false;
    if (p.Cin % BK || p.K != p.Kpad || p.kh * p.kw > 32) return false;
    const long in_bytes = ((long)p.B * p.H * p.W * p.in_cs) * 4, w_bytes = (long)p.Cout * p.Kpad * 4;
    if (in_bytes >= 0x7fffff00L || w_bytes >= 0x7fffff00L) return false;
    p.lean_in_bytes = (int)in_bytes;
    return true;
}

template <int BM, int BN, int WM, int WN>
static int run(ConvP p, int G, int S, hipStream_t st) {
    p.mtiles = (p.M + BM - 1) / BM;
    p.ntiles = (p.Cout + BN - 1) / BN;
    p.vec_out = (p.Cout % 4 == 0) && (p.out_cs % 4 == 0) && (((uintptr_t)p.out & 15) == 0) && (p.out_gs % 4 == 0) &&
                (!p.res || ((p.res_cs % 4 == 0) && (((uintptr_t)p.res & 15) == 0) && (p.res_gs % 4 == 0))) &&
                (!p.scale || ((((uintptr_t)p.scale & 15) == 0) && (p.ss_gs % 4 == 0))) &&
                (!p.prelu || ((((uintptr_t)p.prelu & 15) == 0) && (p.ss_gs % 4 == 0)));
    if (p.es == 2 && p.vec_out && p.Cout % 8 == 0 && p.out_cs % 8 == 0 && p.out_gs % 8 == 0 && !p.prelu &&
        (!p.res || (p.res_cs % 8 == 0 && p.res_gs % 8 == 0)) && (!p.scale || (p.ss_gs % 8 == 0 && (((uintptr_t)p.scale & 31) == 0))))
        p.vec_out = 2;
    const bool gn_sep = p.gn_sum && !(p.vec_out && p.gn_cpg % 4 == 0 && p.gn_groups <= 32 && p.ohw >= BM && p.ohw >= 8);
    double* const gn_sum = p.gn_sum;
    if (gn_sep) p.gn_sum = nullptr;
    auto gn_separate = [&]() {
        if (!gn_sep) return 0;
        View o;
        o.p = p.out; o.B = p.B; o.H = p.OH; o.W = p.OW; o.C = p.Cout; o.cs = p.out_cs; o.gs = p.out_gs; o.es = p.es;
        return launch_gn_stats(o, p.B, G, p.gn_groups, gn_sum, st, false);
    };
    const int nk = p.Kpad / BK;
    if (p.ws && tune().force_split > 0) S = tune().force_split;
    if (!p.ws || S < 1 || p.es == 2) S = 1;
    if (S > nk) S = nk;
    while (S > 1 && (size_t)S * G * p.M * p.Cout > p.ws_floats) --S;
    p.kchunk = (nk + S - 1) / S;
    S = (nk + p.kchunk - 1) / p.kchunk;
    p.ksplit = S;
    p.ws_rows = p.M;
    p.ws_row0 = 0;
    p.nfull = p.mtiles * p.ntiles;
    p.tail_shift = 0;
    const dim3 block(WM * WN * 64);
    const double out_bytes = (double)p.es * G * (double)p.M * p.Cout;
    const double conv_bytes = 4.0 * G * ((double)p.B * p.H * p.W * p.Cin + (double)p.Cout * p.K) + out_bytes * (p.res ? 2.0 : 1.0);
    const double conv_flops = 2.0 * G * (double)p.M * p.K * p.Cout * (p.es == 2 ? 2.0 : 1.0);
    const char* tag = p.tag ? p.tag : "conv_gemm";
    auto exact_fallback = [&]() { p.bf16 = 0; tag = "conv_gemm_f32pipe"; };
    auto reduce = [&](int parts) {
        const long MN = (long)p.ws_rows * p.Cout;
        ProfScope prof("splitk_reduce", 4.0 * G * (double)MN * (parts + 1.0), 0.0, st);
        const int V = p.vec_out ? 4 : 1;
        long chunk = (MN + 2047) / 2048;
        if (chunk < 256L * V * 4) chunk = 256L * V * 4;
        chunk = (chunk + V - 1) / V * V;
        if (p.gn_sum && chunk / p.Cout + 2 > p.ohw) chunk = (long)(p.ohw - 2) * p.Cout / V * V;
        const int blocks = (int)((MN + chunk - 1) / chunk);
        if (p.vec_out)
            hipLaunchKernelGGL(splitk_reduce_kernel<4>, dim3(blocks, G), dim3(256), 0, st, p, parts, G, chunk);
        else
            hipLaunchKernelGGL(splitk_reduce_kernel<1>, dim3(blocks, G), dim3(256), 0, st, p, parts, G, chunk);
    };
    const bool skip = BM != 256 && p.skip_rows && p.kmode == 0 && p.kh > 1 && p.Cin % BK == 0 && p.K == p.Kpad && p.ohw > 0;
    if (p.es == 2) {
        ProfScope prof(tag, conv_bytes, conv_flops, st);
        const dim3 grid(p.mtiles * p.ntiles, 1, G);
        const bool lean = lean_loader(p);
        if (skip) launch_igemm<BM, BN, WM, WN, 3, 4>(lean, grid, block, st, p);
        else launch_igemm<BM, BN, WM, WN, 0, 4>(lean, grid, block, st, p);
        QB_CHECK(hipGetLastError());
        return gn_separate();
    }
    const bool lean = lean_loader(p);
    if (tune().persist && p.es != 2 && ((BM == 128 && BN == 128) || (tune().persist == 2 && (BM == BN || BM == 256))) && BN <= 128 && !skip && p.ws && conv_persistent_ok(p) &&
        (long)p.mtiles * p.ntiles * G >= tune().persist_min_tiles &&
        ((long)p.mtiles * p.ntiles * G >= 256L * (p.es == 2 ? 3 : BM == 64 ? 5 : 2) || nk >= tune().persist_min_nk)) {
        if (p.bf16 == 3 && (BM == 256 || (BM == 64 && nk <= 8))) exact_fallback();
        const int bpc = p.es == 2 ? 3 : BM == 64 ? 5 : 2;
        if (p.ws_floats >= conv_persistent_ws_floats(BM, BN, bpc)) {
            {
                ProfScope prof(tag, conv_bytes, conv_flops, st);
                int rc = 0;
                if constexpr (BM == BN || BM == 256) rc = launch_conv_persistent<BM, BN, WM, WN>(p, G, bpc, st);
                if (rc) return rc;
            }
            return gn_separate();
        }
    }
    constexpr int BPC = igemm_occupancy(BM, BN);
    const long slots = 256L * BPC, tiles = (long)p.mtiles * p.ntiles, blocks_all = tiles * G;
    if (p.ws && !p.bf16 && tune().tail_split && tune().force_split == 0 && BM == 128 && blocks_all > slots && nk >= 32) {
        const long nfull = (blocks_all / slots) * slots / G / p.ntiles * p.ntiles;
        const long rem = tiles - nfull;
        int shift = 0;
        while (shift < 3 && (rem * G << (shift + 1)) <= slots + slots / 8 && (nk >> (shift + 1)) >= 8) ++shift;
        const long row0 = nfull / p.ntiles * BM;
        const double rem_outputs = (double)G * (p.M - row0) * p.Cout;
        if (rem > 0 && shift > 0 && rem_outputs * (1 << shift) <= (double)p.ws_floats) {
            const double whole = launch_cost(blocks_all, nk, (double)G * p.M * p.Cout, S, BPC, kModel3);
            const double tail = (nk + kModel3.c) * BPC * ((double)nfull * G / slots) +
                                launch_cost(rem * G, nk, rem_outputs, 1 << shift, BPC, kModel3);
            if (tail < 0.995 * whole || tune().tail_split == 2) {
                p.nfull = (int)nfull;
                p.tail_shift = shift;
                p.kchunk = (nk + (1 << shift) - 1) >> shift;
                p.ws_row0 = (int)row0;
                p.ws_rows = p.M - (int)row0;
                {
                    ProfScope prof(tag, conv_bytes, conv_flops, st);
                    launch_igemm<BM, BN, WM, WN, 2, 0>(lean, dim3((unsigned)(nfull + (rem << shift)), 1, G), block, st, p);
                }
                reduce(1 << shift);
                QB_CHECK(hipGetLastError());
                return gn_separate();
            }
        }
    }
    if (p.bf16 == 3 && (BM == 256 || (BM == 64 && (nk <= 8 || skip)))) exact_fallback();
    if (p.bf16) {
        {
            ProfScope prof(tag, conv_bytes, conv_flops, st);
            const dim3 grid(p.mtiles * p.ntiles, S, G);
            if (p.bf16 == 3) {
                if (S > 1) launch_igemm<BM, BN, WM, WN, 1, 3>(lean, grid, block, st, p);
                else launch_igemm<BM, BN, WM, WN, 0, 3>(lean, grid, block, st, p);
            } else if (p.bf16 == 2) {
                if (S > 1) launch_igemm<BM, BN, WM, WN, 1, 2>(lean, grid, block, st, p);
                else launch_igemm<BM, BN, WM, WN, 0, 2>(lean, grid, block, st, p);
            } else {
                if (S > 1) launch_igemm<BM, BN, WM, WN, 1, 1>(lean, grid, block, st, p);
                else launch_igemm<BM, BN, WM, WN, 0, 1>(lean, grid, block, st, p);
            }
        }
        if (S > 1) reduce(S);
        QB_CHECK(hipGetLastError());
        return gn_separate();
    }
    p.zones = 0;
    if (skip && tune().zone_cols && lean && BM == 64 && p.kh == 3 && p.kw == 3 && p.stride == 1 && p.pad == p.dil && p.OH == p.H && p.OW == p.W) {
        const int a = p.dil, b = p.W - p.dil;
        p.zx1 = std::max(0, std::min(std::min(a, b), p.W));
        p.zx2 = std::max(0, std::min(std::max(a, b), p.W));
        if (a > b || 8 * p.zx1 >= p.W) p.zones = a <= b ? 1 : 2;
        if (S > 1 && p.mtiles < 32) p.zones = 0;
    }
    if (S > 1) {
        {
            ProfScope prof(tag, conv_bytes, conv_flops, st);
            if (skip) launch_igemm<BM, BN, WM, WN, 4, 0>(lean, dim3(p.mtiles * p.ntiles, S, G), block, st, p);
            else launch_igemm<BM, BN, WM, WN, 1, 0>(lean, dim3(p.mtiles * p.ntiles, S, G), block, st, p);
        }
        reduce(S);
    } else {
        ProfScope prof(tag, conv_bytes, conv_flops, st);
        if (skip) launch_igemm<BM, BN, WM, WN, 3, 0>(lean, dim3(p.mtiles * p.ntiles, 1, G), block, st, p);
        else launch_igemm<BM, BN, WM, WN, 0, 0>(lean, dim3(p.mtiles * p.ntiles, 1, G), block, st, p);
    }
    QB_CHECK(hipGetLastError());
    return gn_separate();
}


int launch_conv(const ConvP& p0, int G, hipStream_t st) {
    ConvP p = p0;
    p.acc_chunk = tune().acc_chunk;
    if (p.es != 2) p.es = 4;
    if (p.es == 2) {
        if (p.bf16 != 2) return fail("conv: fp16 tensors need compute_dtype 2");
        if (p.Cin % 8 || p.in_cs % 8 || p.Kpad % 64 || p.K % 2 || (p.in_gs & 7) || (p.w_gs & 1) || p.in2 || p.prelu)
            return fail("conv (fp16 data path): Cin / channel stride must be multiples of 8 and Kpad a multiple of 64");
        p.Cin /= 2; p.in_cs /= 2; p.K /= 2; p.Kpad /= 2; p.in_gs /= 2; p.w_gs /= 2;
    }
    if (p.Cin % 4 || p.in_cs % 4 || p.Kpad % BK || p.K > p.Kpad)
        return fail("conv: Cin / channel stride must be multiples of 4 and Kpad a multiple of 32");
    if (((uintptr_t)p.in & 15) || ((uintptr_t)p.w & 15) || (p.in_gs & 3) || (p.w_gs & 3))
        return fail("conv: operands must be 16-byte aligned");
    if (p.M <= 0 || p.Cout <= 0) return fail("conv: empty problem");
    if (p.kh * p.kw > 1 && p.Cin < 8) return fail("conv: filters larger than 1x1 need at least 8 input channels (pad the input)");
    if (p.kmode && (p.Cin % BK || p.K != p.Kpad)) return fail("conv: slice-major weights need Cin % 32 == 0");
    if ((p.scale == nullptr) != (p.shift == nullptr)) return fail("conv: scale and shift go together");
    if (p.es == 2 && tune().force_tile == 0) {
        const int rc = launch_conv_h8(p, G, st);
        if (rc != 1) return rc;
    }
    if (p.n_stats) return fail("conv: a launch that normalises its input needs the fp16 patch kernel (conv_h8.hip)");
    if (p0.dil_g[0]) {
        for (int g = 0; g < G; ++g) {
            ConvP q = p0;
            const long es = p0.es == 2 ? 2 : 4;
            q.dil = q.pad = p0.dil_g[g];
            q.dil_g[0] = 0;
            q.in = reinterpret_cast<const float*>(reinterpret_cast<const char*>(p0.in) + (long)g * p0.in_gs * es);
            q.w = reinterpret_cast<const float*>(reinterpret_cast<const char*>(p0.w) + (long)g * p0.w_gs * es);
            q.out = reinterpret_cast<float*>(reinterpret_cast<char*>(p0.out) + (long)g * p0.out_gs * es);
            if (p0.res) q.res = reinterpret_cast<const float*>(reinterpret_cast<const char*>(p0.res) + (long)g * p0.res_gs * es);
            if (p0.scale) { q.scale = p0.scale + (long)g * p0.ss_gs; q.shift = p0.shift + (long)g * p0.ss_gs; }
            if (p0.gn_sum) q.gn_sum = p0.gn_sum + (long)g * p0.B * p0.gn_groups * 2;
            const int rc = launch_conv(q, 1, st);
            if (rc) return rc;
        }
        return 0;
    }
    if (p.es == 4 && p.bf16 == 3 && tune().force_tile == 0 && tune().force_split == 0) {
        const int rc = launch_conv_x8(p, G, st);
        if (rc != 1) return rc;
    }
    switch (tune().force_tile) {
        case 1: return run<64, 64, 2, 2>(p, G, 1, st);
        case 2: return run<128, 128, 2, 2>(p, G, 1, st);
        case 4: return run<256, 32, 4, 1>(p, G, 1, st);
        case 3: return run<128, 64, 2, 2>(p, G, 1, st);
        default: break;
    }
    const int nk = p.Kpad / BK;
    if (p.Cout <= 32) return run<256, 32, 4, 1>(p, G, choose_split(p, G, 256, 32, igemm_occupancy(256, 32)), st);
    if (tune().tile_128x64 && p.Cout <= 64 && p.Cout > 32 && !p.res && (long)((p.M + 127) / 128) * G >= 1024) return run<128, 64, 2, 2>(p, G, 1, st);
    if (p.Cout <= 64 || (p.res && nk <= 8 && p.Cout >= 128)) return run<64, 64, 2, 2>(p, G, choose_split(p, G, 64, 64, igemm_occupancy(64, 64)), st);
    if (p.skip_rows && p.es != 2 && p.kmode == 0 && p.kh > 1 && p.dil * 5 >= p.H * 2)
        return run<64, 64, 2, 2>(p, G, choose_split(p, G, 64, 64, igemm_occupancy(64, 64)), st);
    const long tiles128 = (long)((p.M + 127) / 128) * ((p.Cout + 127) / 128) * G;
    const int s128 = choose_split(p, G, 128, 128, igemm_occupancy(128, 128));
    if (tiles128 < 64 || (tiles128 < 384 && s128 == 1)) return run<64, 64, 2, 2>(p, G, choose_split(p, G, 64, 64, igemm_occupancy(64, 64)), st);
    if (tune().small_n_64 && p.es != 2 && p.kh == 1 && p.kw == 1 && !p.in2 && nk >= 16 && tiles128 <= 1280)
        return run<64, 64, 2, 2>(p, G, choose_split(p, G, 64, 64, igemm_occupancy(64, 64)), st);
    if (tune().small_n_64 == 1 && p.es != 2 && p.bf16 == 0 && p.kh == 1 && p.kw == 1 && !p.in2 && nk <= 32)
        return run<64, 64, 2, 2>(p, G, choose_split(p, G, 64, 64, igemm_occupancy(64, 64)), st);
    return run<128, 128, 2, 2>(p, G, s128, st);
}

}
```

### quber_amd/csrc/elementwise.hip

```cpp
#include "common.h"

namespace quber {

using half_t = _Float16;
template <class T> __device__ inline float4 ldv4(const T* p);
template <> __device__ inline float4 ldv4<float>(const float* p) { return *reinterpret_cast<const float4*>(p); }
template <> __device__ inline float4 ldv4<half_t>(const half_t* p) {
    using h4 = __attribute__((ext_vector_type(4))) half_t;
    const h4 v = *reinterpret_cast<const h4*>(p);
    return make_float4((float)v.x, (float)v.y, (float)v.z, (float)v.w);
}
template <class T> __device__ inline void stv4(T* p, float4 v);
template <> __device__ inline void stv4<float>(float* p, float4 v) { *reinterpret_cast<float4*>(p) = v; }
template <> __device__ inline void stv4<half_t>(half_t* p, float4 v) {
    using h4 = __attribute__((ext_vector_type(4))) half_t;
    *reinterpret_cast<h4*>(p) = h4{(half_t)v.x, (half_t)v.y, (half_t)v.z, (half_t)v.w};
}
template <class T> static inline const T* cptr(const View& v) { return reinterpret_cast<const T*>(v.p); }
template <class T> struct Vec16;
template <> struct Vec16<float> {
    static constexpr int N = 4;
    static __device__ inline void load(const float* p, float* v) { *reinterpret_cast<float4*>(v) = *reinterpret_cast<const float4*>(p); }
    static __device__ inline void store(float* p, const float* v) { *reinterpret_cast<float4*>(p) = *reinterpret_cast<const float4*>(v); }
};
// ... 363 lines not shown
    };
    ld(base + ((long)y0 * W + x0) * in_cs, v00);
    ld(base + ((long)y0 * W + x1) * in_cs, v01);
    ld(base + ((long)y1 * W + x0) * in_cs, v10);
    ld(base + ((long)y1 * W + x1) * in_cs, v11);
#pragma unroll
    for (int e = 0; e < V; ++e) r[e] = hy * (hx * v00[e] + lx * v01[e]) + ly * (hx * v10[e] + lx * v11[e]);
    T* dst = out + ((long)(b * OH + oy) * OW + ox) * out_cs + cv * V;
    if constexpr (V == Vec16<T>::N) Vec16<T>::store(dst, r);
    else stv4(dst, make_float4(r[0], r[1], r[2], r[3]));
}

int launch_bilinear(const View& in, const View& out, int B, hipStream_t st) {
    ProfScope prof("bilinear", (double)in.es * B * in.C * ((double)in.H * in.W + (double)out.H * out.W), 0.0, st);
    if (in.es != out.es) return fail("bilinear: mixed element types");
    if (!quads_ok(in) || !quads_ok(out) || in.C != out.C) return fail("bilinear: channels must come in aligned groups of 4");
    const float sy = (float)in.H / (float)out.H, sx = (float)in.W / (float)out.W;
    if (in.es == 2) {
        const bool wide = in.C % 8 == 0 && in.cs % 8 == 0 && out.cs % 8 == 0 && (((uintptr_t)in.p | (uintptr_t)out.p) & 15) == 0;
        const int V = wide ? 8 : 4, CV = in.C / V;
        const dim3 grid((out.W * CV + 255) / 256, out.H, B);
        if (wide)
            hipLaunchKernelGGL((bilinear_kernel<half_t, 8>), grid, dim3(256), 0, st, cptr<half_t>(in), (half_t*)out.p, in.H, in.W, CV, in.cs,
                               out.H, out.W, out.cs, sy, sx);
        else
            hipLaunchKernelGGL((bilinear_kernel<half_t, 4>), grid, dim3(256), 0, st, cptr<half_t>(in), (half_t*)out.p, in.H, in.W, CV, in.cs,
                               out.H, out.W, out.cs, sy, sx);
    } else {
        const int CV = in.C / 4;
        hipLaunchKernelGGL((bilinear_kernel<float, 4>), dim3((out.W * CV + 255) / 256, out.H, B), dim3(256), 0, st, in.p, out.p, in.H, in.W,
                           CV, in.cs, out.H, out.W, out.cs, sy, sx);
    }
    QB_CHECK(hipGetLastError());
    return 0;
}

template <class T>
__global__ __launch_bounds__(256) void avgpool_kernel(const T* __restrict__ in, T* __restrict__ out, int HW,
                                                      int C, int in_cs, int out_cs) {
    __shared__ double part[16][64];
    const int col = threadIdx.x & 15, lane = threadIdx.x >> 4;
    const int c = blockIdx.x * 64 + col * 4;
    const int b = blockIdx.y;
    double s[4] = {0.0, 0.0, 0.0, 0.0};
    if (c < C) {
        int p = lane;
        for (; p + 7 * 16 < HW; p += 8 * 16) {
            float4 v[8];
#pragma unroll
            for (int u = 0; u < 8; ++u) v[u] = ldv4(in + ((long)b * HW + p + 16 * u) * in_cs + c);
#pragma unroll
            for (int u = 0; u < 8; ++u) { s[0] += (double)v[u].x; s[1] += (double)v[u].y; s[2] += (double)v[u].z; s[3] += (double)v[u].w; }
        }
        for (; p < HW; p += 16) {
            const float4 v = ldv4(in + ((long)b * HW + p) * in_cs + c);
            s[0] += (double)v.x; s[1] += (double)v.y; s[2] += (double)v.z; s[3] += (double)v.w;
        }
    }
#pragma unroll
    for (int e = 0; e < 4; ++e) part[lane][col * 4 + e] = s[e];
    __syncthreads();
    if (threadIdx.x < 64 && blockIdx.x * 64 + threadIdx.x < C) {
        double t = 0.0;
#pragma unroll
        for (int l = 0; l < 16; ++l) t += part[l][threadIdx.x];
        out[(long)b * out_cs + blockIdx.x * 64 + threadIdx.x] = (T)(float)(t / (double)HW);
    }
}

int launch_avgpool(const View& in, const View& out, int B, hipStream_t st) {
    if (in.es != out.es) return fail("avgpool: mixed element types");
    if (!quads_ok(in)) return fail("avgpool: channels must come in aligned groups of 4");
    ProfScope prof("avgpool", (double)in.es * B * in.C * ((double)in.H * in.W + 1.0), 0.0, st);
    if (in.es == 2)
        hipLaunchKernelGGL(avgpool_kernel<half_t>, dim3((in.C + 63) / 64, B), dim3(256), 0, st, cptr<half_t>(in), (half_t*)out.p,
                           in.H * in.W, in.C, in.cs, out.cs);
    else
        hipLaunchKernelGGL(avgpool_kernel<float>, dim3((in.C + 63) / 64, B), dim3(256), 0, st, in.p, out.p, in.H * in.W, in.C,
                           in.cs, out.cs);
    QB_CHECK(hipGetLastError());
    return 0;
}

template <class T, int CIN>
__global__ void predictor_kernel(const PredHeads hs, int in_cs, float* __restrict__ q, int q_nch, int sm_cs, int B, int HW) {
    const int hd = blockIdx.y;
    const T* __restrict__ in = reinterpret_cast<const T*>(hs.in[hd]);
    const float* __restrict__ w = hs.w[hd];
    const float* __restrict__ bias = hs.bias[hd];
    T* __restrict__ sm = reinterpret_cast<T*>(hs.sm[hd]);
    const int cout = hs.cout[hd], q_ch0 = hs.q_ch0[hd], act = hs.act[hd];
    __shared__ float ws[4 * CIN + 4];
    for (int i = threadIdx.x; i < cout * CIN; i += blockDim.x) ws[i] = w[i];
    if ((int)threadIdx.x < cout) ws[4 * CIN + threadIdx.x] = bias[threadIdx.x];
    __syncthreads();
    const long total = (long)B * HW;
    for (long i = blockIdx.x * (long)blockDim.x + threadIdx.x; i < total; i += (long)gridDim.x * blockDim.x) {
        float x[CIN];
        const T* src = in + i * in_cs;
#pragma unroll
        for (int j = 0; j < CIN / 4; ++j) {
            const float4 v = ldv4(src + 4 * j);
            x[4 * j] = v.x; x[4 * j + 1] = v.y; x[4 * j + 2] = v.z; x[4 * j + 3] = v.w;
        }
        const long b = i / HW, pix = i - b * HW;
        float o[4];
        for (int k = 0; k < cout; ++k) {
            float a = 0.f;
#pragma unroll
            for (int j = 0; j < CIN; ++j) a = fmaf(x[j], ws[k * CIN + j], a);
            a += ws[4 * CIN + k];
            o[k] = a;
            q[((long)b * q_nch + q_ch0 + k) * HW + pix] = a;
        }
        if (sm && act == 2) {
            for (int k = 0; k < cout; ++k) sm[i * sm_cs + k] = (T)(1.f / (1.f + expf(-o[k])));
        } else if (sm) {
            float mx = o[0];
            for (int k = 1; k < cout; ++k) mx = fmaxf(mx, o[k]);
            float e[4], s = 0.f;
            for (int k = 0; k < cout; ++k) { e[k] = expf(o[k] - mx); s += e[k]; }
            for (int k = 0; k < cout; ++k) sm[i * sm_cs + k] = (T)(e[k] / s);
        }
    }
}

int launch_predictors(const PredHeads& hs, int C, int in_cs, int es, int H, int W, float* q, int q_nch, int sm_cs, int B, hipStream_t st) {
    if ((C != 32 && C != 64) || hs.n < 1 || hs.n > 5) return fail("predictor: expects 32 or 64 input channels and 1..5 heads");
    if ((es != 4 && es != 2) || in_cs % 4) return fail("predictor: features must come in aligned groups of 4");
    double couts = 0.0, acts = 0.0;
    for (int j = 0; j < hs.n; ++j) {
        if (hs.cout[j] < 1 || hs.cout[j] > 4) return fail("predictor: 1..4 outputs per head");
        if (hs.q_ch0[j] < 0 || hs.q_ch0[j] + hs.cout[j] > q_nch) return fail("predictor: logit planes outside q");
        if ((uintptr_t)hs.in[j] & (uintptr_t)(4 * es - 1)) return fail("predictor: features must come in aligned groups of 4");
        couts += hs.cout[j];
        if (hs.sm[j]) acts += hs.cout[j];
    }
    const long total = (long)B * H * W;
    ProfScope prof("predictor", total * ((double)es * C * hs.n + 4.0 * couts + (double)es * acts), 2.0 * total * C * couts, st);
    const dim3 grid(cap_grid(total, 256), hs.n), block(256);
    if (es == 2 && C == 32) hipLaunchKernelGGL((predictor_kernel<half_t, 32>), grid, block, 0, st, hs, in_cs, q, q_nch, sm_cs, B, H * W);
    else if (es == 2) hipLaunchKernelGGL((predictor_kernel<half_t, 64>), grid, block, 0, st, hs, in_cs, q, q_nch, sm_cs, B, H * W);
    else if (C == 32) hipLaunchKernelGGL((predictor_kernel<float, 32>), grid, block, 0, st, hs, in_cs, q, q_nch, sm_cs, B, H * W);
    else hipLaunchKernelGGL((predictor_kernel<float, 64>), grid, block, 0, st, hs, in_cs, q, q_nch, sm_cs, B, H * W);
    QB_CHECK(hipGetLastError());
    return 0;
}

template <class T>
__global__ void copy_channels_kernel(const T* __restrict__ in, T* __restrict__ out, long pixels, int C4,
                                     int in_cs, int out_cs) {
    const long total = pixels * C4;
    for (long i = blockIdx.x * (long)blockDim.x + threadIdx.x; i < total; i += (long)gridDim.x * blockDim.x) {
        const long pix = i / C4;
        const int c4 = (int)(i - pix * C4);
        stv4(out + pix * out_cs + c4 * 4, ldv4(in + pix * in_cs + c4 * 4));
    }
}

template <class T>
__global__ void add_channels_kernel(const T* __restrict__ a, const T* __restrict__ b, T* __restrict__ out,
                                    long pixels, int C4, int a_cs, int b_cs, int out_cs) {
    const long total = pixels * C4;
    for (long i = blockIdx.x * (long)blockDim.x + threadIdx.x; i < total; i += (long)gridDim.x * blockDim.x) {
        const long pix = i / C4;
        const int c4 = (int)(i - pix * C4);
        const float4 x = ldv4(a + pix * a_cs + c4 * 4);
        const float4 y = ldv4(b + pix * b_cs + c4 * 4);
        stv4(out + pix * out_cs + c4 * 4, make_float4(x.x + y.x, x.y + y.y, x.z + y.z, x.w + y.w));
    }
}

int launch_add_channels(const View& a, const View& b, const View& out, int B, hipStream_t st) {
    const long pixels = (long)B * a.H * a.W;
    ProfScope prof("add_channels", 3.0 * a.es * pixels * a.C, 0.0, st);
    if (a.es != b.es || a.es != out.es) return fail("add: mixed element types");
    if (!quads_ok(a) || !quads_ok(b) || !quads_ok(out) || a.C != b.C || a.C != out.C) return fail("add: channels must come in aligned groups of 4");
    if (a.es == 2)
        hipLaunchKernelGGL(add_channels_kernel<half_t>, dim3(cap_grid(pixels * (a.C / 4), 256)), dim3(256), 0, st, cptr<half_t>(a),
                           cptr<half_t>(b), (half_t*)out.p, pixels, a.C / 4, a.cs, b.cs, out.cs);
    else
        hipLaunchKernelGGL(add_channels_kernel<float>, dim3(cap_grid(pixels * (a.C / 4), 256)), dim3(256), 0, st, a.p, b.p, out.p,
                           pixels, a.C / 4, a.cs, b.cs, out.cs);
    QB_CHECK(hipGetLastError());
    return 0;
}

int launch_copy_channels(const View& in, const View& out, int B, hipStream_t st) {
    const long pixels = (long)B * in.H * in.W;
    ProfScope prof("copy_channels", 2.0 * in.es * pixels * in.C, 0.0, st);
    if (in.es != out.es) return fail("copy: mixed element types");
    if (!quads_ok(in) || !quads_ok(out) || in.C != out.C) return fail("copy: channels must come in aligned groups of 4");
    if (in.es == 2)
        hipLaunchKernelGGL(copy_channels_kernel<half_t>, dim3(cap_grid(pixels * (in.C / 4), 256)), dim3(256), 0, st, cptr<half_t>(in),
                           (half_t*)out.p, pixels, in.C / 4, in.cs, out.cs);
    else
        hipLaunchKernelGGL(copy_channels_kernel<float>, dim3(cap_grid(pixels * (in.C / 4), 256)), dim3(256), 0, st, in.p, out.p,
                           pixels, in.C / 4, in.cs, out.cs);
    QB_CHECK(hipGetLastError());
    return 0;
}

template <int V>
__global__ __launch_bounds__(256) void upsample_logits_kernel(const float* __restrict__ q, float* __restrict__ out, int h,
                                                              int w, int nch, int scale, int OH, int OW,
                                                              unsigned mul_mask) {
    const int pl = blockIdx.y;
    const unsigned per_row = (unsigned)OW / V;
    const unsigned idx = blockIdx.x * 256u + threadIdx.x;
    if (idx >= per_row * (unsigned)OH) return;
    const int oy = idx / per_row;
    const int ox0 = (idx - oy * per_row) * V;
    const float inv = 1.f / (float)scale;
    int y0, y1;
    float ly;
    bilin_src(oy, inv, h, y0, y1, ly);
    const float hy = 1.f - ly;
    const float* s0 = q + (long)pl * h * w + (long)y0 * w;
    const float* s1 = q + (long)pl * h * w + (long)y1 * w;
    const float mul = ((mul_mask >> (pl % nch)) & 1u) ? (float)scale : 1.f;
    float o[V];
#pragma unroll
    for (int e = 0; e < V; ++e) {
// ... 37 lines not shown
```

### quber_amd/csrc/plan.h

```cpp
#pragma once
#include <math.h>
#include <string.h>

#include <functional>
#include <map>
#include <memory>
#include <string>
#include <vector>

#include "../../include/quber_hip.h"
#include "common.h"

namespace quber {

int* tuning_field(Tuning& t, int key);
bool tuning_plan_time(int key);

struct ProfRec { int tag; hipEvent_t e0, e1; double bytes, flops; };
struct StageSum { std::string name; double ms = 0.0, bytes = 0.0, flops = 0.0; int launches = 0; };
struct Profiler {
    std::vector<std::string> tags;
    std::vector<ProfRec> recs;
    std::vector<hipEvent_t> pool;
    size_t used = 0;
    std::vector<StageSum> sums;
    hipEvent_t get() {
        if (used == pool.size()) {
            hipEvent_t e = nullptr;
            if (hipEventCreate(&e) != hipSuccess) return nullptr;
            pool.push_back(e);
        }
        return pool[used++];
    }
    ~Profiler() { for (hipEvent_t e : pool) (void)hipEventDestroy(e); }
};
extern thread_local Profiler* g_prof;

constexpr int GN_SLOTS = 64;
inline size_t gn_slot_doubles(int max_batch) { return (size_t)2 * 32 * max_batch * 4; }

enum OpKind { OP_CONV = 0, OP_NORM = 1, OP_OTHER = 2, OP_KINDS = 3 };
struct Op {
    std::function<int(int, hipStream_t)> run;
    int kind;
    std::string name;
    double flops;
    int launches;
    int lane = 0;
    int ctl = 0;
};
constexpr int LANES = 3;
constexpr int LANE_BATCH = 16;
constexpr int LANE_BATCH_F32 = 12;

}

struct quber_ctx {
    quber_config cfg;
    quber::Tuning tune;
    std::map<std::string, std::vector<float>> hostw;
    std::vector<std::pair<std::string, int64_t>> specs;
    std::vector<void*> allocs;
    size_t alloc_bytes = 0;
    int* enc_bad = nullptr;
    std::vector<quber::Op> ops;
    std::map<std::string, quber::View> taps;
    float* gauss = nullptr;
    void* enc_ws = nullptr;
    uint8_t* err_ws = nullptr;
    void* post_ws = nullptr;
    void* cleanup_ws = nullptr;
    void* perturb_ws = nullptr;
    size_t perturb_ws_bytes = 0;
    void* masknms_ws = nullptr;
    size_t masknms_ws_bytes = 0;
    void* zoom_ws = nullptr;
    double* gn_stats = nullptr;
    int gn_slots = 0;
    float* splitk_ws = nullptr;
    size_t splitk_floats = 0;
    float* wino_ws = nullptr;
    size_t wino_floats = 0;
    hipStream_t lane_stream[quber::LANES] = {};
    hipEvent_t lane_fork[quber::LANES] = {}, lane_join[quber::LANES] = {};
    float* lane_wino_ws[quber::LANES] = {};
    size_t lane_wino_floats[quber::LANES] = {};
    float* lane_splitk_ws[quber::LANES] = {};
    size_t lane_splitk_floats = 0;
    bool lanes_built = false;
    bool lanes_on = false;
    int lane_now = 0;
    quber::View X;
    float* q = nullptr;
    const uint8_t* cur_bgr = nullptr;
    const uint8_t* cur_depth = nullptr;
    const float* cur_off = nullptr;
    float* cur_out = nullptr;
    double flops = 0.0;
    double wino_flops = 0.0;
    double wino_saved = 0.0;
    double wino_pad = 0.0;
    std::vector<hipEvent_t> prof_events;
    std::unique_ptr<quber::Profiler> prof;
    bool stem_fused = false;
    bool finalized = false;
    int device = 0;
};

namespace quber {

enum Affine { AF_NONE, AF_FROZEN_BN, AF_BIAS, AF_BIAS_BN };

struct GnFuse { double* sums = nullptr; int groups = 0; };
struct DeferredNorm {
    View in, out;
    const double* stats = nullptr;
    const float *gamma = nullptr, *beta = nullptr;
    int C = 0, G = 0;
    bool absorbed = false;
};
struct LastConv { std::shared_ptr<GnFuse> fuse; const float* out = nullptr; int G = 0, C = 0; };

struct Builder {
    quber_ctx* c;
    bool dry;
    LastConv last_conv;
    std::shared_ptr<DeferredNorm> pending_norm;
    std::string err;
    int Bmax, H, W;
    int cur_lane = 0;
    int aes = 4;

    Builder(quber_ctx* ctx, bool d) : c(ctx), dry(d), Bmax(ctx->cfg.max_batch), H(ctx->cfg.height), W(ctx->cfg.width) {
        if (ctx->cfg.compute_dtype == 2 && ctx->cfg.with_network == 1) aes = 2;
    }

    const float* hw(const std::string& name, int64_t numel);
    void* dalloc_bytes(size_t bytes);
    float* upload16(const std::vector<_Float16>& v);
    float* upload(const std::vector<float>& v);
    const float* upload_weights(const std::vector<float>& packed);
    const void* split3(const float* dev_w, size_t n);
    View make(int C, int h, int w, int G = 1);
    static View slice(View v, int coff, int C, long gs = -1);

    void emit_conv(const std::string& name, const std::vector<const float*>& w, const View& in, int cin_real, const View& out, int k, int stride, int pad, int dil, bool affine,
                   const std::vector<float>& scale, const std::vector<float>& shift, const std::vector<float>& prelu, const View* res, bool relu, const std::vector<int>& dil_g = {});
    void conv(const std::vector<std::string>& names, const View& in, int cin_real, const View& out, int k, int stride, int pad, int dil, Affine af, const View* res, bool relu,
              const std::vector<int>& dil_g = {});
    void fuse_shortcut(const std::vector<std::string>& n3, const std::vector<std::string>& ns, const View& y, int mid, const View& x, int cin, int stride, const View& out);
    void gn_relu(const std::vector<std::string>& names, const View& in, const View& out, bool single_consumer = false);
    void op(std::function<int(int, hipStream_t)> f);
    void fork(int L);
    void back_to_main() { cur_lane = 0; }
    void join(int L);
    void conv_gn(const std::string& n, const View& in, const View& tmp, const View& out, int k, int dil, bool single_consumer = false, int cin_real = -1);
    void emit_stem_fused(const std::vector<std::string>& names, const View& out);
    void build();
};
void build_lmff(Builder& b);

int check_cfg(const quber_config& c);
bool op_set_tuning(int key, int value);

inline int check_batch(quber_ctx* c, int batch) {
    if (!c) return fail("null context");
    if (batch < 1 || batch > c->cfg.max_batch) return fail("batch outside 1..max_batch");
    return 0;
}
inline int check_tta_batch(quber_ctx* c, int batch) {
    if (!c) return fail("null context");
    if (batch < 1 || 2L * batch > c->cfg.max_batch) return fail("test-time augmentation: 2 * batch outside 2..max_batch");
    return 0;
}

}
```

### quber_amd/csrc/plan.hip

```cpp
#include "plan.h"

namespace quber {
namespace {

constexpr int BLOCKS50[4] = {3, 4, 6, 3}, BLOCKS101[4] = {3, 4, 23, 3}, BLOCKS152[4] = {3, 8, 36, 3};

struct BnFold {
    const float *w, *b, *m, *v;
    bool ok() const { return w && b && m && v; }
    float scale(int o) const { return w[o] * (1.0f / sqrtf(v[o] + 1e-5f)); }
    float shift(int o, float sc) const { return b[o] - m[o] * sc; }
};
BnFold frozen_bn(Builder& b, const std::string& n, int C) {
    return {b.hw(n + ".norm.weight", C), b.hw(n + ".norm.bias", C), b.hw(n + ".norm.running_mean", C), b.hw(n + ".norm.running_var", C)};
}

struct WinoChoice { bool take = false; int m = 0; double ratio = 0.0; bool one_kernel = false; };
WinoChoice choose_winograd(int H, int W, int k, int stride, int pad, int dil, int Cin, int Cout, bool plain, int dtype) {
    WinoChoice r;
    if (!winograd_eligible(k, stride, pad, dil, Cin, Cout) || !plain || tune().winograd == 1 || (dtype != 0 && dtype != 3)) return r;
    const double lim = (double)tune().wino_max_ratio / 100.0;
    const double r6 = winograd_m6_channels_ok(Cin, Cout) ? winograd_mac_ratio(H, W, dil, 6) : 1e9;
    const double r4 = winograd_mac_ratio(H, W, dil, 4), r2 = winograd_mac_ratio(H, W, dil, 2);
    double best = lim;
// ... 79 lines not shown
                        const std::vector<float>& scale, const std::vector<float>& shift, const std::vector<float>& prelu, const View* res, bool relu, const std::vector<int>& dil_g) {
    const int G = (int)w.size();
    const int Cin = in.C, Cout = out.C;
    const int KS = aes == 2 ? 64 : 32;
    const int K = k * k * Cin, Kpad = (K + KS - 1) / KS * KS;
    const int OH = (in.H + 2 * pad - dil * (k - 1) - 1) / stride + 1;
    const int OW = (in.W + 2 * pad - dil * (k - 1) - 1) / stride + 1;
    const bool skip_rows = k == 3 && stride == 1 && dil > 1 && Cin % KS == 0 && cin_real == Cin && 10 * 2 * pad >= 2 * 3 * OH &&
                           !(winograd_eligible(k, stride, pad, dil, Cin, out.C) && !res && prelu.empty() &&
                             std::min(winograd_mac_ratio(in.H, in.W, dil, 4), winograd_mac_ratio(in.H, in.W, dil, 2)) <= tune().wino_max_ratio / 100.0 && tune().winograd != 1);
    const int kmode = (k > 1 && Cin % KS == 0 && !skip_rows) ? 1 : 0;
    if (dry) return;
    const double fl = 2.0 * OH * OW * (double)cin_real * k * k * Cout * G;
    c->flops += fl;
    if (OH != out.H || OW != out.W) { if (err.empty()) err = "internal: conv output geometry mismatch at " + name; return; }
    for (const float* p : w)
        if (!p) return;
    std::vector<float> packed((size_t)G * Cout * Kpad, 0.f);
    for (int g = 0; g < G; ++g)
        for (int o = 0; o < Cout; ++o) {
            float* dst = &packed[((size_t)g * Cout + o) * Kpad];
            for (int ci = 0; ci < cin_real; ++ci)
                for (int t = 0; t < k * k; ++t) {
                    const size_t kk = kmode ? ((size_t)(ci / KS) * k * k + t) * KS + ci % KS : (size_t)t * Cin + ci;
                    dst[kk] = w[g][((size_t)o * cin_real + ci) * k * k + t];
                }
        }
    ConvP p{};
    p.in = in.p;
    p.w = upload_weights(packed);
    if (aes != 2 && k == 1) { p.w3 = split3(p.w, packed.size()); p.w3_plane = (long)packed.size(); }
    p.es = aes;
    if (in.es != aes || out.es != aes || (res && res->es != aes)) { if (err.empty()) err = "internal: element type mismatch at " + name; return; }
    const bool ident = !affine && aes == 2 && Cout >= 32;
    p.scale = affine ? upload(scale) : ident ? upload(std::vector<float>((size_t)G * Cout, 1.f)) : nullptr;
    p.shift = affine ? upload(shift) : ident ? upload(std::vector<float>((size_t)G * Cout, 0.f)) : nullptr;
    for (size_t g = 0; g < dil_g.size() && g < 4; ++g) p.dil_g[g] = dil_g[g];
    p.prelu = prelu.empty() ? nullptr : upload(prelu);
    p.res = res ? res->p : nullptr;
    p.out = out.p;
    p.H = in.H; p.W = in.W; p.Cin = Cin; p.in_cs = in.cs;
    p.OH = OH; p.OW = OW; p.Cout = Cout; p.out_cs = out.cs;
    p.res_cs = res ? res->cs : 0;
    p.K = K; p.Kpad = Kpad;
    p.kh = k; p.kw = k; p.stride = stride; p.pad = pad; p.dil = dil;
    p.relu = relu; p.kmode = kmode; p.skip_rows = skip_rows;
    p.bf16 = c->cfg.compute_dtype;
    p.in_gs = in.gs; p.out_gs = out.gs; p.res_gs = res ? res->gs : 0;
    p.w_gs = (long)Cout * Kpad; p.ss_gs = Cout;
    p.ohw = OH * OW;
    quber_ctx* ctx = c;
    const WinoChoice wc = choose_winograd(in.H, in.W, k, stride, pad, dil, Cin, Cout, cin_real == Cin && !res && prelu.empty(), c->cfg.compute_dtype);
    const bool wino = wc.take;
    WinoP wq{};
    if (wino) {
        const int m = wc.m, P = (m + 2) * (m + 2);
        c->wino_flops += fl;
        std::vector<float> u((size_t)G * P * Cout * Cin);
        for (int g = 0; g < G; ++g) winograd_weights_host(w[g], Cout, Cin, m, &u[(size_t)g * P * Cout * Cin]);
        wq.in = in; wq.out = out; wq.u = upload(u);
        wq.u3 = split3(wq.u, u.size()); wq.u3_plane = (long)u.size();
        if (wc.one_kernel) {
            std::vector<float> uf(u.size());
            for (int g = 0; g < G; ++g) winograd_fused_pack_host(&u[(size_t)g * P * Cout * Cin], Cout, Cin, &uf[(size_t)g * P * Cout * Cin]);
            wq.uf = upload(uf);
        }
        wq.scale = p.scale; wq.shift = p.shift; wq.ss_gs = Cout; wq.relu = relu; wq.dil = dil; wq.m = m;
        wq.dtype = c->cfg.compute_dtype;
        wq.pack = tune().wino_pack;
    }
    std::shared_ptr<DeferredNorm> norm, norm16;
    if (wino && pending_norm && pending_norm->out.p == in.p && pending_norm->C == Cin && pending_norm->G == G) {
        norm = pending_norm;
        norm->absorbed = true;
    }
    float* coef16 = nullptr;
    if (!wino && aes == 2 && tune().h8_norm && tune().h8 && tune().h8_narrow && pending_norm && pending_norm->out.p == in.p && pending_norm->C == Cin &&
        pending_norm->G == G && k == 3 && stride == 1 && pad == 1 && dil == 1 && dil_g.empty() && Cin % 64 == 0 && Cin >= 128 && Cin <= 512 && cin_real == Cin &&
        (Cout == 128 || Cout == 64 || Cout == 32 || (Cout >= 256 && Cout % 8 == 0 && tune().h8_narrow != 2)) && !res && prelu.empty() && in.cs == pending_norm->in.cs && in.gs == pending_norm->in.gs) {
        norm16 = pending_norm;
        norm16->absorbed = true;
        coef16 = (float*)dalloc_bytes(sizeof(float) * (size_t)G * Bmax * Cin * 2);
    }
    pending_norm.reset();
    if (wino) {
        WinoP probe = wq;
        if (norm) probe.in = norm->in;
        const bool fusedk = wq.uf && winograd_fused_ok(probe, Bmax, G);
        wq.algo = fusedk ? 2 : 1;
        const double ratio = fusedk ? wc.ratio : winograd_mac_ratio_run(in.H, in.W, dil, wq.m, wq.pack != 0);
        c->wino_saved += fl * (1.0 - ratio);
        c->wino_pad += fl * (ratio - (double)((wq.m + 2) * (wq.m + 2)) / (9.0 * wq.m * wq.m));
        if (wq.uf && winograd_fused_prepare() && err.empty()) err = "winograd (fused): cannot raise the kernels' LDS limit";
        const size_t need = fusedk ? winograd_fused_ws_floats(Bmax, Cin, G) : winograd_ws_floats(Bmax, in.H, in.W, Cin, Cout, G, dil, wq.m);
        if (need > c->wino_floats) c->wino_floats = need;
        if (cur_lane) {
            const int lb = std::min(Bmax, LANE_BATCH);
            const size_t ln = fusedk ? winograd_fused_ws_floats(lb, Cin, G) : winograd_ws_floats(lb, in.H, in.W, Cin, Cout, G, dil, wq.m);
            if (ln > c->lane_wino_floats[cur_lane]) c->lane_wino_floats[cur_lane] = ln;
        }
    }
    auto fuse = std::make_shared<GnFuse>();
    last_conv = {fuse, out.p, G, Cout};
    const int L = cur_lane;
    c->ops.push_back({[p, G, ctx, fuse, wq, wino, norm, norm16, coef16, L](int B, hipStream_t st) mutable {
        const bool side = L && ctx->lane_now == L;
        float* const sk_ws = side ? ctx->lane_splitk_ws[L] : ctx->splitk_ws;
        const size_t sk_floats = side ? ctx->lane_splitk_floats : ctx->splitk_floats;
        if (wino) {
            wq.ws = side ? ctx->lane_wino_ws[L] : ctx->wino_ws; wq.ws_floats = side ? ctx->lane_wino_floats[L] : ctx->wino_floats;
            wq.splitk_ws = sk_ws; wq.splitk_floats = sk_floats;
            wq.gn_sum = fuse->sums; wq.gn_groups = fuse->groups;
            if (norm) {
                wq.in = norm->in;
                wq.norm = WinoNorm{norm->stats, norm->gamma, norm->beta, 32, 0, norm->C, 1, 0.0, 1e-5f};
            }
            return launch_conv_winograd(wq, B, G, st);
        }
        p.B = B;
        p.M = B * p.OH * p.OW;
        p.ws = sk_ws;
        p.ws_floats = sk_floats;
        p.gn_sum = fuse->sums;
        p.gn_groups = fuse->groups;
        p.gn_cpg = fuse->groups ? p.Cout / fuse->groups : 0;
        if (norm16) {
            ConvP q = p;
            q.in = norm16->in.p;
            q.n_stats = norm16->stats; q.n_gamma = norm16->gamma; q.n_beta = norm16->beta; q.n_coef = coef16;
            q.n_groups = 32; q.n_param_gs = norm16->C; q.n_relu = 1; q.n_eps = 1e-5f;
            if (conv_h8_patch_takes(q, G, true)) return launch_conv(q, G, st);
            const int rc = launch_gn_apply(norm16->in, norm16->out, B, G, 32, norm16->stats, norm16->gamma, norm16->beta, norm16->C, 1e-5f, 1, st);
            if (rc) return rc;
        }
        return launch_conv(p, G, st);
    }, OP_CONV, name, fl, 1});
    c->ops.back().lane = cur_lane;
}

void Builder::conv(const std::vector<std::string>& names, const View& in, int cin_real, const View& out, int k, int stride, int pad, int dil, Affine af, const View* res, bool relu,
                   const std::vector<int>& dil_g) {
    const int G = (int)names.size(), Cout = out.C;
    std::vector<float> scale((size_t)G * Cout, 1.f), shift((size_t)G * Cout, 0.f);
    std::vector<const float*> w;
    for (int g = 0; g < G; ++g) {
        const std::string& n = names[g];
        w.push_back(hw(n + ".weight", (int64_t)Cout * cin_real * k * k));
        const bool has_bn = af == AF_FROZEN_BN || af == AF_BIAS_BN;
        const float* bias = (af == AF_BIAS || af == AF_BIAS_BN) ? hw(n + ".bias", Cout) : nullptr;
        const BnFold bn = has_bn ? frozen_bn(*this, n, Cout) : BnFold{};
        if (dry || (has_bn && !bn.ok())) continue;
        for (int o = 0; o < Cout; ++o) {
            float sc = 1.f, sh = 0.f;
            if (has_bn) {
                sc = bn.scale(o);
                sh = bn.shift(o, sc);
                if (af == AF_BIAS_BN && bias) sh = fmaf(bias[o], sc, sh);
            } else if (af == AF_BIAS && bias) {
                sh = bias[o];
            }
            scale[(size_t)g * Cout + o] = sc;
            shift[(size_t)g * Cout + o] = sh;
        }
    }
    emit_conv(names[0], w, in, cin_real, out, k, stride, pad, dil, af != AF_NONE, scale, shift, {}, res, relu, dil_g);
}

void Builder::fuse_shortcut(const std::vector<std::string>& n3, const std::vector<std::string>& ns, const View& y, int mid, const View& x, int cin, int stride, const View& out) {
    if (dry || !tune().fuse_shortcut || c->ops.size() < 2) return;
    const int G = (int)n3.size(), Cout = out.C, Kd = mid + cin;
    const int KS = aes == 2 ? 64 : 32;
    if (mid % KS || cin % KS || y.C != mid || x.C != cin) return;
    std::vector<float> packed((size_t)G * Cout * Kd), ones((size_t)G * Cout, 1.f), shift((size_t)G * Cout);
    for (int g = 0; g < G; ++g) {
        const float* w3 = hw(n3[g] + ".weight", (int64_t)Cout * mid);
        const float* wsh = hw(ns[g] + ".weight", (int64_t)Cout * cin);
        const BnFold b3 = frozen_bn(*this, n3[g], Cout), bs = frozen_bn(*this, ns[g], Cout);
        if (!w3 || !wsh || !b3.ok() || !bs.ok()) return;
        for (int o = 0; o < Cout; ++o) {
            const float s3 = b3.scale(o), h3 = b3.shift(o, s3), ss = bs.scale(o), hs = bs.shift(o, ss);
            float* dst = &packed[((size_t)g * Cout + o) * Kd];
            for (int ci = 0; ci < mid; ++ci) dst[ci] = s3 * w3[(size_t)o * mid + ci];
            for (int ci = 0; ci < cin; ++ci) dst[mid + ci] = ss * wsh[(size_t)o * cin + ci];
            shift[(size_t)g * Cout + o] = h3 + hs;
        }
    }
    ConvP p{};
    p.in = y.p; p.in2 = x.p; p.scale = upload(ones); p.shift = upload(shift); p.out = out.p;
    p.w = upload_weights(packed);
    if (aes != 2) { p.w3 = split3(p.w, packed.size()); p.w3_plane = (long)packed.size(); }
    p.es = aes;
    p.H = y.H; p.W = y.W; p.Cin = mid; p.in_cs = y.cs; p.in_gs = y.gs;
    p.H2 = x.H; p.W2 = x.W; p.in2_cs = x.cs; p.in2_gs = x.gs; p.stride2 = stride; p.K1 = mid;
    p.OH = out.H; p.OW = out.W; p.Cout = Cout; p.out_cs = out.cs; p.out_gs = out.gs;
    p.K = Kd; p.Kpad = Kd; p.kh = 1; p.kw = 1; p.stride = 1; p.pad = 0; p.dil = 1; p.relu = 1;
    p.bf16 = c->cfg.compute_dtype;
    p.w_gs = (long)Cout * Kd; p.ss_gs = Cout; p.ohw = out.H * out.W;
    Op op3 = c->ops.back();
    c->ops.pop_back();
    Op ops = c->ops.back();
    c->ops.pop_back();
    quber_ctx* ctx = c;
    c->ops.push_back({[p, G, ctx, op3, ops](int B, hipStream_t st) mutable {
        p.B = B;
        p.M = B * p.OH * p.OW;
        p.ws = ctx->splitk_ws;
        p.ws_floats = ctx->splitk_floats;
        const int rc = launch_conv_dual(p, G, st);
        if (rc != 1) return rc;
        const int r1 = ops.run(B, st);
        return r1 ? r1 : op3.run(B, st);
    }, OP_CONV, op3.name + " + shortcut", op3.flops + ops.flops, 1});
}

void Builder::gn_relu(const std::vector<std::string>& names, const View& in, const View& out, bool single_consumer) {
    const int G = (int)names.size(), C = in.C;
    std::vector<float> gamma, beta;
    for (int g = 0; g < G; ++g) {
        const float* w = hw(names[g] + ".weight", C);
        const float* b = hw(names[g] + ".bias", C);
        if (dry || !w || !b) continue;
        gamma.insert(gamma.end(), w, w + C);
        beta.insert(beta.end(), b, b + C);
    }
    if (dry) return;
    const float* dg = upload(gamma);
    const float* db = upload(beta);
    if (c->gn_slots >= GN_SLOTS) { if (err.empty()) err = "more GroupNorm layers than accumulator slots"; return; }
    double* stats = c->gn_stats + (size_t)c->gn_slots++ * gn_slot_doubles(c->cfg.max_batch);
    const bool fused = last_conv.fuse && last_conv.out == in.p && last_conv.G == G && last_conv.C == C;
    if (fused) {
        last_conv.fuse->sums = stats;
        last_conv.fuse->groups = 32;
        last_conv.fuse.reset();
    }
    std::shared_ptr<DeferredNorm> dn;
    if (single_consumer && C % 32 == 0 && (C / 32) % 4 == 0) {
        dn = std::make_shared<DeferredNorm>();
        dn->in = in; dn->out = out; dn->stats = stats; dn->gamma = dg; dn->beta = db; dn->C = C; dn->G = G;
    }
    pending_norm = dn;
    c->ops.push_back({[=](int B, hipStream_t st) {
        if (!fused) {
            int rc = launch_gn_stats(in, B, G, 32, stats, st, false);
            if (rc) return rc;
        }
        if (dn && dn->absorbed) return 0;
        return launch_gn_apply(in, out, B, G, 32, stats, dg, db, C, 1e-5f, 1, st);
    }, OP_NORM, names[0], 0.0, fused ? 1 : 2});
    c->ops.back().lane = cur_lane;
}

void Builder::op(std::function<int(int, hipStream_t)> f) {
    if (!dry) c->ops.push_back({std::move(f), OP_OTHER, "elementwise", 0.0, 1, cur_lane});
}
void Builder::fork(int L) {
    if (dry) return;
    c->ops.push_back({nullptr, OP_OTHER, "fork", 0.0, 0, L, 1});
    cur_lane = L;
    c->lanes_built = true;
}
void Builder::join(int L) {
    if (dry) return;
    c->ops.push_back({nullptr, OP_OTHER, "join", 0.0, 0, L, 2});
}

void Builder::conv_gn(const std::string& n, const View& in, const View& tmp, const View& out, int k, int dil, bool single_consumer, int cin_real) {
    conv({n}, in, cin_real > 0 ? cin_real : in.C, tmp, k, 1, k == 3 ? dil : 0, dil, AF_NONE, nullptr, false);
    gn_relu({n + ".norm"}, tmp, out, single_consumer);
}

void Builder::emit_stem_fused(const std::vector<std::string>& names, const View& out) {
    const int G = (int)names.size();
    std::vector<float> packed((size_t)G * 9 * 6 * 32), scale((size_t)G * 32, 1.f), shift((size_t)G * 32, 0.f);
    bool ok = true;
    for (int g = 0; g < G; ++g) {
        const std::string& n = names[g];
        const float* w = hw(n + ".weight", (int64_t)32 * 6 * 9);
        const BnFold bn = frozen_bn(*this, n, 32);
        if (dry) continue;
        if (!w || !bn.ok()) { ok = false; continue; }
        for (int o = 0; o < 32; ++o) {
            for (int ci = 0; ci < 6; ++ci)
                for (int t = 0; t < 9; ++t) {
                    const float v = w[((size_t)o * 6 + ci) * 9 + t];
                    packed[(((size_t)g * 9 + t) * 6 + ci) * 32 + o] = out.es == 2 ? (float)(_Float16)v : v;
                }
            const float sc = bn.scale(o);
            scale[(size_t)g * 32 + o] = sc;
            shift[(size_t)g * 32 + o] = bn.shift(o, sc);
        }
    }
    if (dry || !ok) return;
    const int OH = (H + 1) / 2, OW = (W + 1) / 2;
    if (out.C != 32 || out.cs != 32 || out.H != OH || out.W != OW || (out.es != 4 && out.es != 2)) { if (err.empty()) err = "internal: fused stem output geometry"; return; }
    const double fl = 2.0 * OH * OW * 6.0 * 9.0 * 32.0 * G;
    c->flops += fl;
    const float *dw = upload(packed), *ds = upload(scale), *dh = upload(shift);
    const float* dwf = nullptr;
    if (out.es == 2 && tune().stem_fused != 2) {
        std::vector<_Float16> wf((size_t)G * 2 * 3 * 64 * 8, (_Float16)0.f);
        for (int g = 0; g < G; ++g)
            for (int jj = 0; jj < 2; ++jj)
                for (int ks = 0; ks < 3; ++ks)
                    for (int l = 0; l < 64; ++l) {
                        const int fr = l & 15, tap = 4 * ks + (l >> 4), n = 8 * (fr >> 2) + 4 * jj + (fr & 3);
                        if (tap < 9)
                            for (int ci = 0; ci < 6; ++ci)
                                wf[((((size_t)g * 2 + jj) * 3 + ks) * 64 + l) * 8 + ci] = (_Float16)packed[(((size_t)g * 9 + tap) * 6 + ci) * 32 + n];
                    }
        dwf = upload16(wf);
    }
    quber_ctx* ctx = c;
    const View o = out;
    c->stem_fused = true;
    c->ops.push_back({[=](int B, hipStream_t st) {
        return launch_stem_conv1(ctx->cur_bgr, ctx->cur_depth, ctx->cur_off, B, ctx->cfg.height, ctx->cfg.width, G, ctx->cfg.pixel_mean,
                                 ctx->cfg.pixel_std, dw, ds, dh, o.p, o.gs, o.es, st, dwf);
    }, OP_CONV, names[0], fl, 1});
    last_conv = {nullptr, nullptr, 0, 0};
    pending_norm.reset();
}

void Builder::build() {
    const quber_config& cf = c->cfg;
    const int* nb = cf.resnet_depth == 50 ? BLOCKS50 : cf.resnet_depth == 101 ? BLOCKS101 : BLOCKS152;
    const int h2 = (H + 1) / 2, w2 = (W + 1) / 2, h4 = (h2 + 1) / 2, w4 = (w2 + 1) / 2;
    const int h8 = (h4 + 1) / 2, w8 = (w4 + 1) / 2, h16 = (h8 + 1) / 2, w16 = (w8 + 1) / 2;
    const std::string R = "backbone.rgb_backbone.", D = "backbone.depth_backbone.";
    const int NS = cf.streams;
    auto two = [&](const std::string& tail, bool stage_prefix) -> std::vector<std::string> {
        if (NS == 1) return {"backbone." + tail};
        return {R + tail, D + (stage_prefix ? "depth_" : "") + tail};
    };
    if (!dry) {
        c->gn_stats = (double*)dalloc_bytes(sizeof(double) * GN_SLOTS * gn_slot_doubles(Bmax));
        quber_ctx* ctx = c;
        fork(2);
        op([ctx](int, hipStream_t st) {
            return launch_zero(ctx->gn_stats, sizeof(double) * ctx->gn_slots * gn_slot_doubles(ctx->cfg.max_batch), st);
        });
        back_to_main();
    }
    if (!dry) {
        c->splitk_floats = (size_t)40 << 20;
        c->splitk_ws = (float*)dalloc_bytes(sizeof(float) * c->splitk_floats);
    }

    const bool stem_one = tune().stem_fused != 0 && !(aes == 4 && (cf.compute_dtype == 1 || cf.compute_dtype == 2));
    View s1 = make(32, h2, w2, NS), s2 = make(32, h2, w2, NS), s3 = make(64, h2, w2, NS);
    if (stem_one) {
        emit_stem_fused(two("stem.conv1", false), s1);
    } else {
        View X = make(aes == 2 ? 16 : 8, H, W, NS);
        if (!dry) c->X = X;
        conv(two("stem.conv1", false), X, 6, s1, 3, 2, 1, 1, AF_FROZEN_BN, nullptr, true);
    }
    if (!dry) c->taps["stem1"] = s1;
    conv(two("stem.conv2", false), s1, 32, s2, 3, 1, 1, 1, AF_FROZEN_BN, nullptr, true);
    conv(two("stem.conv3", false), s2, 32, s3, 3, 1, 1, 1, AF_FROZEN_BN, nullptr, true);
    View x = make(64, h4, w4, NS);
    op([=](int B, hipStream_t st) { return launch_maxpool3x3s2(s3, x, B, NS, st); });

    View cat[4];
    View F[4];
    const int fch[4] = {256, 512, 1024, 2048};
    auto emit_fusion = [&](int s) {
        if (NS == 1) {
            F[s] = cat[s];
            if (!dry) c->taps["res" + std::to_string(s + 2)] = F[s];
            return;
        }
        const std::string n = "backbone.fusion_res" + std::to_string(s + 2) + ".";
        const int C = fch[s], fh = cat[s].H, fw = cat[s].W;
        View t = make(C, fh, fw), a = make(C, fh, fw);
        if (cf.fusion_add) {
            View ra = slice(cat[s], 0, C), rb = slice(cat[s], C, C);
            op([=](int B, hipStream_t st) { return launch_add_channels(ra, rb, a, B, st); });
        } else {
            conv({n + "conv"}, cat[s], 2 * C, t, 1, 1, 0, 1, AF_BIAS, nullptr, false);
            gn_relu({n + "gn"}, t, a, s != 3 && cf.backbone_fusion_layers > 0);
        }
        if (s != 3) {
            View b2 = make(C, fh, fw), t2 = make(C, fh, fw);
            View cur = a, nxt = b2, traw = t2, tprev = t;
            for (int i = 0; i < cf.backbone_fusion_layers; ++i) {
                conv({n + "conv" + std::to_string(i)}, cur, C, traw, 3, 1, 1, 1, AF_BIAS, nullptr, false);
                gn_relu({n + "gn" + std::to_string(i)}, traw, nxt, i + 1 < cf.backbone_fusion_layers);
                std::swap(cur, nxt);
                std::swap(traw, tprev);
            }
            a = cur;
        }
        F[s] = a;
        if (!dry) c->taps["res" + std::to_string(s + 2)] = a;
    };
    const std::string Hd = "ins_embed_head.";
    const int CD = cf.convs_dim, HC = cf.head_channels;
    View cat3 = make(64 + 256, h8, w8), t64 = make(64, h8, w8);
    View cat2 = make(aes == 2 ? (32 + CD + 63) / 64 * 64 : 32 + CD, h4, w4), t32 = make(32, h4, w4);
    int cin = 64, cout = 256, mid = 64, ch = h4, cw = w4;
    for (int s = 0; s < 4; ++s) {
        const int stage = s + 2;
        const int sdil = stage == 5 ? cf.res5_dilation : 1;
        const int first = (s == 0 || sdil > 1) ? 1 : 2;
        const int oh = first == 2 ? (ch + 1) / 2 : ch, ow = first == 2 ? (cw + 1) / 2 : cw;
        View t1 = make(mid, oh, ow, NS), t2 = make(mid, oh, ow, NS), sc = make(cout, oh, ow, NS);
        View oa = make(cout, oh, ow, NS), ob = make(cout, oh, ow, NS);
        const bool tapped = stage != 4;
        if (tapped) {
            View cb = make(NS * cout, oh, ow, 1);
            cat[s] = cb;
        }
        static const int mg[3] = {1, 2, 4};
        for (int i = 0; i < nb[s]; ++i) {
            const int stride = i == 0 ? first : 1;
            const int dil = stage == 5 ? sdil * mg[i % 3] : 1;
            const std::string tail = "res" + std::to_string(stage) + "." + std::to_string(i) + ".";
            const bool last = i == nb[s] - 1;
            View out = (last && tapped) ? slice(cat[s], 0, cout, cout) : ((i & 1) ? ob : oa);
            conv(two(tail + "conv1", true), x, cin, t1, 1, stride, 0, 1, AF_FROZEN_BN, nullptr, true);
            conv(two(tail + "conv2", true), t1, mid, t2, 3, 1, dil, dil, AF_FROZEN_BN, nullptr, true);
            View resv = x;
            if (cin != cout) {
                conv(two(tail + "shortcut", true), x, cin, sc, 1, stride, 0, 1, AF_FROZEN_BN, nullptr, false);
                resv = sc;
            }
            conv(two(tail + "conv3", true), t2, mid, out, 1, 1, 0, 1, AF_FROZEN_BN, &resv, true);
            if (cin != cout) fuse_shortcut(two(tail + "conv3", true), two(tail + "shortcut", true), t2, mid, x, cin, stride, out);
            x = out;
            cin = cout;
        }
        ch = oh; cw = ow;
        cout *= 2; mid *= 2;
        if (s == 0 || s == 1) {
            if (s == 0) join(2);
            fork(1 + s);
            emit_fusion(s);
            if (s == 1) conv_gn(Hd + "decoder.res3.project_conv", F[1], t64, slice(cat3, 0, 64), 1, 1);
            else conv_gn(Hd + "decoder.res2.project_conv", F[0], t32, slice(cat2, 0, 32), 1, 1);
            back_to_main();
        } else if (s == 3) {
            emit_fusion(3);
        }
    }

    const std::string A = Hd + "decoder.res5.project_conv.";
    View catA = make(1280, h16, w16), tA = make(256, h16, w16);
    fork(2);
    {
        View pooled = make(2048, 1, 1), pc = make(256, 1, 1);
        View f5 = F[3];
        op([=](int B, hipStream_t st) { return launch_avgpool(f5, pooled, B, st); });
        conv({A + "convs.4.1"}, pooled, 2048, pc, 1, 1, 0, 1, AF_BIAS, nullptr, true);
        View dst = slice(catA, 1024, 256);
        op([=](int B, hipStream_t st) { return launch_bilinear(pc, dst, B, st); });
    }
    back_to_main();
    conv_gn(A + "convs.0", F[3], tA, slice(catA, 0, 256), 1, 1);
    const int adil[3] = {6, 12, 18};
    const int aspp_oh = F[3].H;
    const bool aspp_grouped = aes == 2 && tune().h8 && 10 * 2 * adil[2] < 2 * 3 * aspp_oh;
    if (aspp_grouped) {
        View tA3 = make(256, h16, w16, 3);
        View xin = F[3];
        xin.gs = 0;
        const std::vector<std::string> an = {A + "convs.1", A + "convs.2", A + "convs.3"};
        conv(an, xin, F[3].C, tA3, 3, 1, adil[2], adil[2], AF_NONE, nullptr, false, {adil[0], adil[1], adil[2]});
        gn_relu({an[0] + ".norm", an[1] + ".norm", an[2] + ".norm"}, tA3, slice(catA, 256, 256, 256));
    } else if (tune().aspp_lanes) {
        View tA1 = make(256, h16, w16), tA2 = make(256, h16, w16);
        fork(1);
        conv_gn(A + "convs.1", F[3], tA1, slice(catA, 256, 256), 3, adil[0]);
        back_to_main();
        fork(2);
        conv_gn(A + "convs.2", F[3], tA2, slice(catA, 512, 256), 3, adil[1]);
        back_to_main();
        conv_gn(A + "convs.3", F[3], tA, slice(catA, 768, 256), 3, adil[2]);
// ... 14 lines not shown
    conv_gn(Hd + "decoder.res3.fuse_conv.0", cat3, t128a, u3, 3, 1, true);
    View t128b = make(CD, F[1].H, F[1].W);
    conv_gn(Hd + "decoder.res3.fuse_conv.1", u3, t128b, y3, 3, 1);

    static const char* HN[5] = {"foreground", "center", "offset", "eee_mask", "eee_boundary"};
    const int ncls = cf.error_classes;
    const int hch[5] = {1, 1, 2, ncls, ncls};
    const int hplane[5] = {0, 1, 2, QUBER_LOGIT_BASE + (cf.eee_boundary_on ? ncls : 0), QUBER_LOGIT_BASE};
    const bool enabled[5] = {true, true, true, cf.eee_mask_on != 0, cf.eee_boundary_on != 0};
    std::vector<std::vector<int>> levels;
    if (cf.hierarchical) {
        for (int i = 0; i < cf.n_levels; ++i) {
            std::vector<int> l;
            for (int j = 0; j < 5 && cf.level_heads[i][j] >= 0; ++j) l.push_back(cf.level_heads[i][j]);
            levels.push_back(l);
        }
    } else {
        std::vector<int> l;
        for (int k : {3, 4, 0, 1, 2})
            if (enabled[k]) l.push_back(k);
        levels.push_back(l);
    }
    const int nlev = (int)levels.size();
    std::vector<View> YP(nlev);
    std::vector<int> ypw(nlev, 0);
    for (int i = 1; i < nlev; ++i) {
        int wd = CD;
        if (cf.fusion_feat) wd += HC * (int)levels[i - 1].size();
        if (cf.fusion_pred)
            for (int k : levels[i - 1]) wd += hch[k];
        ypw[i] = wd;
        YP[i] = make(aes == 2 ? (wd + 63) / 64 * 64 : (wd + 3) / 4 * 4, h4, w4);
    }
    View t128 = make(CD, h4, w4);
    join(1);
    {
        View dst = slice(cat2, 32, CD);
        op([=](int B, hipStream_t st) { return launch_bilinear(y3, dst, B, st); });
    }
    View u2 = make(CD, h4, w4);
    conv_gn(Hd + "decoder.res2.fuse_conv.0", cat2, t128, u2, 3, 1, true, 32 + CD);
    View y = nlev > 1 ? slice(YP[1], 0, CD) : make(CD, h4, w4);
    View t128c = make(CD, h4, w4);
    conv_gn(Hd + "decoder.res2.fuse_conv.1", u2, t128c, y, 3, 1);
    for (int i = 2; i < nlev; ++i) {
        View dst = slice(YP[i], 0, CD);
        op([=](int B, hipStream_t st) { return launch_copy_channels(y, dst, B, st); });
    }
    if (!dry) c->taps["y"] = y;

    const int planes = QUBER_LOGIT_BASE + ncls * ((cf.eee_mask_on ? 1 : 0) + (cf.eee_boundary_on ? 1 : 0));
    if (!dry) c->q = (float*)dalloc_bytes(sizeof(float) * (size_t)Bmax * planes * h4 * w4);
    float* q = c->q;
    for (int i = 0; i < nlev; ++i) {
        const int G = (int)levels[i].size();
        View x = y;
        if (i > 0) {
            const std::string FL = Hd + "fusion_layers_" + std::to_string(i) + ".fusion_layers.";
            View za = make(CD, h4, w4), zb = make(CD, h4, w4);
            conv({FL + "0"}, YP[i], ypw[i], za, 1, 1, 0, 1, AF_BIAS_BN, nullptr, true);
            View cur = za, nxt = zb;
            for (int j = 0; j < cf.head_fusion_layers; ++j) {
                conv({FL + std::to_string(j + 1)}, cur, CD, nxt, 3, 1, 1, 1, AF_BIAS_BN, nullptr, true);
                std::swap(cur, nxt);
            }
            x = cur;
            if (!dry) c->taps["z" + std::to_string(i)] = x;
        }
        std::vector<std::string> h0, h1, n0, n1;
        for (int k : levels[i]) {
            h0.push_back(Hd + HN[k] + "_pred_head.head.0");
            h1.push_back(Hd + HN[k] + "_pred_head.head.1");
            n0.push_back(h0.back() + ".norm");
            n1.push_back(h1.back() + ".norm");
        }
        View g128 = make(CD, h4, w4, G), g128n = make(CD, h4, w4, G), g32 = make(HC, h4, w4, G);
        const bool next = i + 1 < nlev;
        View feat = (next && cf.fusion_feat) ? slice(YP[i + 1], CD, HC, HC) : make(HC, h4, w4, G);
        View xin = x;
        xin.gs = 0;
        conv(h0, xin, CD, g128, 3, 1, 1, 1, AF_NONE, nullptr, false);
        gn_relu(n0, g128, g128n, true);
        conv(h1, g128n, CD, g32, 3, 1, 1, 1, AF_NONE, nullptr, false);
        gn_relu(n1, g32, feat);
        int act_off = CD + (cf.fusion_feat ? HC * G : 0);
        PredHeads ph{};
        int ph_act_cs = 0;
        for (int j = 0; j < G; ++j) {
            const int k = levels[i][j];
            const float* pw = hw(Hd + HN[k] + "_predictor.predictor.weight", (int64_t)hch[k] * HC);
            const float* pb = hw(Hd + HN[k] + "_predictor.predictor.bias", hch[k]);
            View in = feat;
            in.p = feat.at((long)j * feat.gs);
            if (!dry) c->taps[std::string("feat_") + HN[k]] = in;
            float* act_dst = nullptr;
            int act_cs = 0;
            if (next && cf.fusion_pred) {
                act_dst = YP[i + 1].at(act_off);
                act_cs = YP[i + 1].cs;
                act_off += hch[k];
            }
            if (dry || !pw || !pb) continue;
            const float* dw = upload(std::vector<float>(pw, pw + hch[k] * HC));
            const float* db = upload(std::vector<float>(pb, pb + hch[k]));
            ph.in[ph.n] = in.p; ph.w[ph.n] = dw; ph.bias[ph.n] = db; ph.sm[ph.n] = act_dst; ph.cout[ph.n] = hch[k];
            ph.q_ch0[ph.n] = hplane[k]; ph.act[ph.n] = act_dst ? (k >= 3 ? 1 : 2) : 0;
            if (act_dst) ph_act_cs = act_cs;
            ++ph.n;
        }
        if (!dry && ph.n == G) {
            const int fcs = feat.cs, fes = feat.es, fh = feat.H, fw = feat.W;
            op([=](int B, hipStream_t st) { return launch_predictors(ph, HC, fcs, fes, fh, fw, q, planes, ph_act_cs, B, st); });
        }
    }
    quber_ctx* ctx = c;
    op([=](int B, hipStream_t st) {
        return launch_upsample_logits(q, ctx->cur_out, B, planes, h4, w4, 4, ctx->cfg.height, ctx->cfg.width, 0xCu, st);
    });
}

}
```

### quber_amd/csrc/runtime.hip

```cpp
#include <atomic>

#include "plan.h"

namespace quber {

Tuning g_tune;
thread_local const Tuning* t_tune = nullptr;

struct TuneKey { int key; int Tuning::*field; bool plan; };
constexpr TuneKey TUNE_KEYS[] = {
    {3, &Tuning::force_split, false},           {4, &Tuning::force_tile, false},
    {5, &Tuning::tail_split, false},            {6, &Tuning::winograd, true},
    {7, &Tuning::wino_min_cin, true},           {8, &Tuning::wino_max_ratio, true},
    {9, &Tuning::wino_variant, true},           {10, &Tuning::wino_min_cout, true},
    {13, &Tuning::persist, false},              {14, &Tuning::persist_min_nk, false},
    {15, &Tuning::persist_min_tiles, false},    {16, &Tuning::persist_debug, false},
    {17, &Tuning::wino_pairs, false},           {18, &Tuning::fuse_shortcut, true},
    {19, &Tuning::tile_128x64, false},          {20, &Tuning::wino_chunk_mb, false},
    {21, &Tuning::acc_chunk, false},            {24, &Tuning::lanes, false},
    {25, &Tuning::wino_fused, true},            {27, &Tuning::wino_fused_max_cin, true},
    {29, &Tuning::stem_fused, true},            {30, &Tuning::lean_loader, false},
    {31, &Tuning::h8, false},                   {32, &Tuning::h8_min_tiles, false},
    {35, &Tuning::x8, false},                   {36, &Tuning::x8_min_rounds, false},
    {37, &Tuning::x8_min_nk, false},            {38, &Tuning::h8_narrow, false},
    {39, &Tuning::h8_norm, true},               {41, &Tuning::aspp_lanes, true},
    {42, &Tuning::small_n_64, false},           {43, &Tuning::zone_cols, false},
    {51, &Tuning::wino_pack, true},
};
int* tuning_field(Tuning& t, int key) {
    for (const TuneKey& k : TUNE_KEYS)
        if (k.key == key) return &(t.*k.field);
    return nullptr;
}
bool tuning_set(Tuning& t, int key, int value) {
    int* f = tuning_field(t, key);
    if (f) *f = value;
    return f != nullptr;
}
bool tuning_plan_time(int key) {
    for (const TuneKey& k : TUNE_KEYS)
        if (k.key == key) return k.plan;
    return false;
}

int device_cus() {
    static std::atomic<int> cache[64];
    int dev = 0;
    if (hipGetDevice(&dev) != hipSuccess) return -1;
    const bool cached = dev >= 0 && dev < 64;
    if (cached) {
        const int v = cache[dev].load(std::memory_order_relaxed);
        if (v > 0) return v;
    }
    hipDeviceProp_t prop;
    if (hipGetDeviceProperties(&prop, dev) != hipSuccess) return -1;
    const int cus = prop.multiProcessorCount > 0 ? prop.multiProcessorCount : 256;
    if (cached) cache[dev].store(cus, std::memory_order_relaxed);
    return cus;
}

static thread_local std::string g_err;
extern "C" const char* quber_last_error(void) { return g_err.c_str(); }
void set_error(const std::string& m) { g_err = m; }
int fail(const std::string& m) { g_err = m; return -1; }

thread_local Profiler* g_prof = nullptr;

ProfScope::ProfScope(const char* tag, double bytes, double flops, hipStream_t s) : rec(-1), st(s) {
    Profiler* p = g_prof;
    if (!p) return;
    int ti = -1;
    for (size_t i = 0; i < p->tags.size(); ++i)
        if (p->tags[i] == tag) { ti = (int)i; break; }
    if (ti < 0) { ti = (int)p->tags.size(); p->tags.emplace_back(tag); }
    ProfRec r{ti, p->get(), p->get(), bytes, flops};
    if (!r.e0 || !r.e1 || hipEventRecord(r.e0, s) != hipSuccess) return;
    rec = (int)p->recs.size();
    p->recs.push_back(r);
}
ProfScope::~ProfScope() {
    if (rec >= 0 && g_prof) (void)hipEventRecord(g_prof->recs[rec].e1, st);
}

}
```

Baseline: 10180 refined masks/s.

## Fold deferred GroupNorm+ReLU into 1x1 conv loads and predictor heads

Defers the GroupNorm+ReLU that follows the last backbone fusion conv and the last head conv. The normalisation is applied on load inside the consumer instead: a LEAN fp32 1x1 implicit-GEMM variant reads per-channel scale/shift coefficients, and the predictor heads kernel normalises on the fly. This drops the separate gn_apply pass and its activation write/read. The cost is an extra coefficient kernel, extra coefficient loads and register pressure in the GEMM loader, and debug taps that must now run gn_apply lazily to return correct data.

```diff
diff --git a/include/quber_hip.h b/include/quber_hip.h
--- a/include/quber_hip.h
+++ b/include/quber_hip.h
@@ -186,6 +186,10 @@
                     int32_t cout, int32_t ksize, int32_t stride, int32_t pad, int32_t dil, const float* dev_scale,
                     const float* dev_shift, const float* dev_residual, int32_t relu, float* dev_packed_scratch,
                     float* dev_y, void* stream);
+int quber_op_conv1x1_gn(const float* dev_x, int32_t batch, int32_t h, int32_t w, int32_t cin, const double* dev_stats, const float* dev_gamma,
+                        const float* dev_beta, int32_t groups, float eps, float* dev_coef_scratch, const float* dev_w_oihw, int32_t cout,
+                        const float* dev_scale, const float* dev_shift, int32_t relu, double* dev_gn_sums, int32_t gn_groups,
+                        float* dev_packed_scratch, float* dev_y, void* stream);
 int quber_op_conv1x1_f16(const void* dev_x, int32_t batch, int32_t h, int32_t w, int32_t cin, const void* dev_w_oi,
                          int32_t cout, const float* dev_scale, const float* dev_shift, const void* dev_residual,
                          int32_t relu, void* dev_y, void* stream);
@@ -227,6 +231,10 @@
 int quber_op_predictors(int32_t n, const void* const* dev_feat, const float* const* dev_w, const float* const* dev_bias, void* const* dev_act_dst,
                         const int32_t* cout, const int32_t* q_ch0, const int32_t* act, int32_t c, int32_t feat_cs, int32_t es, int32_t batch,
                         int32_t h, int32_t w, float* dev_q, int32_t q_nch, int32_t act_cs, void* stream);
+int quber_op_predictors_gn(int32_t n, const void* const* dev_feat, const double* const* dev_stats, const float* const* dev_gamma,
+                           const float* const* dev_beta, int32_t cpg, float eps, const float* const* dev_w, const float* const* dev_bias,
+                           void* const* dev_act_dst, const int32_t* cout, const int32_t* q_ch0, const int32_t* act, int32_t c, int32_t feat_cs,
+                           int32_t batch, int32_t h, int32_t w, float* dev_q, int32_t q_nch, int32_t act_cs, void* stream);
 int quber_op_upsample_logits(const float* dev_q, float* dev_out, int32_t batch, int32_t nch, int32_t h, int32_t w, int32_t scale, int32_t oh,
                              int32_t ow, uint32_t mul_mask, void* stream);
 int quber_op_preprocess(const uint8_t* dev_bgr, const uint8_t* dev_depth, const float* dev_offsets, void* dev_x, int32_t x_c, int32_t es,
diff --git a/quber_amd/_lib.py b/quber_amd/_lib.py
--- a/quber_amd/_lib.py
+++ b/quber_amd/_lib.py
@@ -97,6 +97,7 @@
     "quber_op_conv2d_f16": (C.c_int, [_P, _I, _I, _I, _I, _P, _I, _I, _I, _I, _I, _I, _P, _P, _P, _I, _P, _I, _P, _P]),
     "quber_op_conv1x1_dual": (C.c_int, [_P, _P, _I, _I, _I, _I, _I, _I, _I, _I, _P, _P, _P, _I, _I, _P, _P]),
     "quber_op_conv2d": (C.c_int, [_P, _I, _I, _I, _I, _P, _I, _I, _I, _I, _I, _P, _P, _P, _I, _P, _P, _P]),
+    "quber_op_conv1x1_gn": (C.c_int, [_P, _I, _I, _I, _I, _P, _P, _P, _I, C.c_float, _P, _P, _I, _P, _P, _I, _P, _I, _P, _P, _P]),
     "quber_op_conv3x3_winograd": (C.c_int, [_P, _I, _I, _I, _I, _P, _I, _I, _I, _P, _P, _I, _P, _P, C.c_int64, _P, _P]),
     "quber_op_groupnorm": (C.c_int, [_P, _I, _I, _I, _I, _I, _P, _P, C.c_float, _I, _P, _P, _P]),
     "quber_op_bilinear": (C.c_int, [_P, _I, _I, _I, _I, _I, _I, _P, _P]),
@@ -110,6 +111,7 @@
     "quber_op_add_channels": (C.c_int, [_P, _I, _I, _P, _I, _I, _P, _I, _I, _I, _I, _I, _I, _P]),
     "quber_op_copy_channels": (C.c_int, [_P, _I, _I, _P, _I, _I, _I, _I, _I, _I, _P]),
     "quber_op_predictors": (C.c_int, [_I, _P, _P, _P, _P, _P, _P, _P, _I, _I, _I, _I, _I, _I, _P, _I, _I, _P]),
+    "quber_op_predictors_gn": (C.c_int, [_I, _P, _P, _P, _P, _I, C.c_float, _P, _P, _P, _P, _P, _P, _I, _I, _I, _I, _I, _P, _I, _I, _P]),
     "quber_op_upsample_logits": (C.c_int, [_P, _P, _I, _I, _I, _I, _I, _I, _I, C.c_uint32, _P]),
     "quber_op_preprocess": (C.c_int, [_P, _P, _P, _P, _I, _I, _I, _I, _I, _I, _P, _P, _I, _P]),
     "quber_op_group_pixels": (C.c_int, [_P, _I, _I, _I, _I, _I, _P, _P, _P, _P, _P]),
diff --git a/quber_amd/csrc/api.hip b/quber_amd/csrc/api.hip
--- a/quber_amd/csrc/api.hip
+++ b/quber_amd/csrc/api.hip
@@ -292,6 +292,7 @@
     if (!bgr || (!depth && c->cfg.streams == 2) || !offs || !logits || !rest_ok) return fail(null_msg);
     c->cur_out = logits;
     c->cur_bgr = bgr; c->cur_depth = depth; c->cur_off = offs;
+    c->last_stream = st; c->last_batch = batch;
     return c->stem_fused ? 0 : launch_preprocess(bgr, depth, offs, c->X, batch, c->cfg.max_batch, c->cfg.height, c->cfg.width,
                                                  c->cfg.pixel_mean, c->cfg.pixel_std, c->cfg.streams, st);
 }
@@ -678,6 +679,15 @@
     if (!c || !name) return fail("null argument");
     auto it = c->taps.find(name);
     if (it == c->taps.end()) return fail(std::string("no intermediate named '") + name + "'");
+    auto nt = c->tap_norms.find(name);
+    if (nt != c->tap_norms.end() && nt->second->absorbed && c->last_batch > 0) {
+        const quber::DeferredNorm& dn = *nt->second;
+        quber::TuneScope tscope(&c->tune);
+        QB_CHECK(hipDeviceSynchronize());
+        const int rc = launch_gn_apply(dn.in, dn.out, c->last_batch, dn.G, 32, dn.stats, dn.gamma, dn.beta, dn.C, 1e-5f, 1, c->last_stream);
+        if (rc) return rc;
+        QB_CHECK(hipStreamSynchronize(c->last_stream));
+    }
     *ptr = it->second.p;
     dims4[0] = it->second.B; dims4[1] = it->second.H; dims4[2] = it->second.W; dims4[3] = it->second.C;
     *cs = it->second.cs;
diff --git a/quber_amd/csrc/api_ops.hip b/quber_amd/csrc/api_ops.hip
--- a/quber_amd/csrc/api_ops.hip
+++ b/quber_amd/csrc/api_ops.hip
@@ -100,6 +100,31 @@
         if (rc) return rc;
     }
     return launch_conv(p, 1, st);
+}
+
+int quber_op_conv1x1_gn(const float* x, int32_t B, int32_t h, int32_t w, int32_t cin, const double* stats, const float* gamma, const float* beta, int32_t groups, float eps,
+                        float* coef, const float* w_oihw, int32_t cout, const float* scale, const float* shift, int32_t relu, double* gn_sums, int32_t gn_groups,
+                        float* packed, float* y, void* stream) {
+    hipStream_t st = (hipStream_t)stream;
+    if (cin % 32) return fail("conv1x1_gn: cin must be a multiple of 32");
+    hipLaunchKernelGGL(pack_oihw_kernel, dim3(256), dim3(256), 0, st, w_oihw, cout, cin, 1, cin, 0, packed);
+    ConvP p{};
+    p.in = x; p.w = packed; p.scale = scale; p.shift = shift; p.out = y;
+    conv_geometry(p, B, h, w, cin, cout, 1, 1, 0, 1);
+    p.Kpad = cin; p.relu = relu; p.bf16 = 0; p.w_gs = 0; p.ss_gs = 0;
+    p.ws = g_op_ws; p.ws_floats = g_op_ws ? g_op_ws_floats : 0;
+    if (gn_sums) {
+        if (gn_groups < 1 || cout % gn_groups) return fail("conv1x1_gn: channels must divide into the norm groups");
+        p.gn_sum = gn_sums; p.gn_groups = gn_groups; p.gn_cpg = cout / gn_groups;
+    }
+    if (stats) {
+        if (!gamma || !beta || !coef || groups < 1 || cin % groups) return fail("conv1x1_gn: the folded norm needs gamma, beta, a coefficient scratch and groups that divide cin");
+        p.n_stats = stats; p.n_gamma = gamma; p.n_beta = beta; p.n_coef = coef;
+        p.n_groups = groups; p.n_param_gs = cin; p.n_relu = 1; p.n_eps = eps;
+    }
+    const int rc = launch_conv(p, 1, st);
+    if (rc == 1) return fail("conv1x1_gn: this launch has no kernel that normalises on load");
+    return rc;
 }
 
 int quber_op_conv1x1_f16(const void* x, int32_t B, int32_t h, int32_t w, int32_t cin, const void* w_oi, int32_t cout,
@@ -255,6 +280,21 @@
     return launch_predictors(hs, c, feat_cs, es, h, wd, q, q_nch, act_cs, B, (hipStream_t)stream);
 }
 
+int quber_op_predictors_gn(int32_t n, const void* const* feat, const double* const* stats, const float* const* gamma, const float* const* beta, int32_t cpg, float eps,
+                           const float* const* w, const float* const* bias, void* const* act_dst, const int32_t* cout, const int32_t* q_ch0, const int32_t* act, int32_t c,
+                           int32_t feat_cs, int32_t B, int32_t h, int32_t wd, float* q, int32_t q_nch, int32_t act_cs, void* stream) {
+    PredHeads hs{};
+    hs.n = n;
+    for (int j = 0; j < n && j < 5; ++j) {
+        hs.in[j] = feat[j]; hs.w[j] = w[j]; hs.bias[j] = bias[j]; hs.sm[j] = act_dst[j];
+        hs.cout[j] = cout[j]; hs.q_ch0[j] = q_ch0[j]; hs.act[j] = act[j];
+        hs.n_stats[j] = stats[j]; hs.n_gamma[j] = gamma[j]; hs.n_beta[j] = beta[j];
+    }
+    if (n < 1 || !hs.n_stats[0]) return fail("predictors_gn: the sums of every head's features are required");
+    hs.n_cpg = cpg; hs.n_eps = eps;
+    return launch_predictors(hs, c, feat_cs, 4, h, wd, q, q_nch, act_cs, B, (hipStream_t)stream);
+}
+
 int quber_op_upsample_logits(const float* q, float* out, int32_t B, int32_t nch, int32_t h, int32_t w, int32_t scale, int32_t oh, int32_t ow,
                              uint32_t mul_mask, void* stream) {
     return launch_upsample_logits(q, out, B, nch, h, w, scale, oh, ow, mul_mask, (hipStream_t)stream);
diff --git a/quber_amd/csrc/common.h b/quber_amd/csrc/common.h
--- a/quber_amd/csrc/common.h
+++ b/quber_amd/csrc/common.h
@@ -157,6 +157,8 @@
     int aspp_lanes = 1;
     int h8_narrow = 1;
     int h8_norm = 1;
+    int fold_norm_1x1 = 1;
+    int fold_norm_pred = 1;
     int h8_min_tiles = 224;
 };
 extern Tuning g_tune;
@@ -197,7 +199,11 @@
                     const float* gamma, const float* beta, int param_gs, float eps, int relu, hipStream_t st);
 int launch_bilinear(const View& in, const View& out, int B, hipStream_t st);
 int launch_avgpool(const View& in, const View& out, int B, hipStream_t st);
-struct PredHeads { int n; const void* in[5]; const float* w[5]; const float* bias[5]; void* sm[5]; int cout[5], q_ch0[5], act[5] ; };
+struct PredHeads {
+    int n; const void* in[5]; const float* w[5]; const float* bias[5]; void* sm[5]; int cout[5], q_ch0[5], act[5] ;
+    const double* n_stats[5]; const float* n_gamma[5]; const float* n_beta[5]; int n_cpg; float n_eps;
+};
+constexpr int PRED_NORM_PAIRS = 1024;
 int launch_predictors(const PredHeads& hs, int C, int in_cs, int es, int H, int W, float* q, int q_nch, int sm_cs, int B, hipStream_t st);
 int launch_copy_channels(const View& in, const View& out, int B, hipStream_t st);
 int launch_add_channels(const View& a, const View& b, const View& out, int B, hipStream_t st);
diff --git a/quber_amd/csrc/conv_igemm.hip b/quber_amd/csrc/conv_igemm.hip
--- a/quber_amd/csrc/conv_igemm.hip
+++ b/quber_amd/csrc/conv_igemm.hip
@@ -28,7 +28,8 @@
 #ifndef QB_H16_LEAN_OCC
 #define QB_H16_LEAN_OCC 4
 #endif
-constexpr int igemm_occupancy(int BM, int BN, int DT = 0, bool LEAN = false) {
+constexpr int igemm_occupancy(int BM, int BN, int DT = 0, bool LEAN = false, bool NORM = false) {
+    if (NORM) return BM == 64 ? 5 : 2;
     if (DT == 4 && LEAN && BM == 128 && BN == 128) return QB_H16_LEAN_OCC;
     if (DT == 0 && LEAN && BM == 64 && BN == 64) return QB_F32_LEAN64_OCC;
     if (DT == 4 && BM * BN >= 128 * 128) return QB_H16_OCC;
@@ -57,8 +58,9 @@
     return (long)b * p.ohw + oy * p.OW + ox;
 }
 
-template <int BM, int BN, int WM, int WN, int MODE, int DT = 0, bool LEAN = false>
-__global__ __launch_bounds__(WM * WN * 64) __attribute__((amdgpu_waves_per_eu(igemm_occupancy(BM, BN, DT, LEAN)))) void conv_igemm_f32(const ConvP p) {
+template <int BM, int BN, int WM, int WN, int MODE, int DT = 0, bool LEAN = false, bool NORM = false>
+__global__ __launch_bounds__(WM * WN * 64) __attribute__((amdgpu_waves_per_eu(igemm_occupancy(BM, BN, DT, LEAN, NORM)))) void conv_igemm_f32(const ConvP p) {
+    static_assert(!NORM || (LEAN && DT == 0 && (MODE == 0 || MODE == 1)), "normalise-on-load: exact fp32 LEAN kernel, whole tiles or split-K");
     constexpr int NTH = WM * WN * 64;
     constexpr int RPP = NTH / 8;
     constexpr int TM = BM / WM / 32;
@@ -229,7 +231,8 @@
     unsigned amask[AL];
     int skc = 0, skx = 0, sky = 0;
     int swk = 0;
-    __amdgpu_buffer_rsrc_t rsa, rsb;
+    __amdgpu_buffer_rsrc_t rsa, rsb, rsn;
+    int coff[NORM ? AL : 1];
     if constexpr (LEAN) {
 #pragma unroll
         for (int i = 0; i < AL; ++i) {
@@ -280,14 +283,31 @@
         }
         rsa = __builtin_amdgcn_make_buffer_rsrc(const_cast<float*>(in), 0, p.lean_in_bytes, 0x00020000);
         rsb = __builtin_amdgcn_make_buffer_rsrc(const_cast<float*>(wt), 0, 0x7ffffff0, 0x00020000);
+        if constexpr (NORM) {
+#pragma unroll
+            for (int i = 0; i < AL; ++i) {
+                const int m = m0 + lrow + RPP * i;
+                coff[i] = m < p.M ? ((m / p.ohw) * p.Cin + kq) * 8 : 0;
+            }
+            rsn = __builtin_amdgcn_make_buffer_rsrc(p.n_coef + (long)g * (p.n_coef_bytes / 4), 0, p.n_coef_bytes, 0x00020000);
+        }
     }
 
     f32x4 ra[AL], rb[BL];
+    f32x4 rn0[NORM ? AL : 1], rn1[NORM ? AL : 1];
     bool aok[AL];
     auto gload = [&](int kt) __attribute__((always_inline)) {
         if constexpr (LEAN) {
             const int tap = sky * p.kw + skx;
             const int soff = (((sky * p.dil) * p.W + skx * p.dil) * p.in_cs + skc) * 4;
+            if constexpr (NORM) {
+#pragma unroll
+                for (int i = 0; i < AL; ++i) {
+                    const int o = amask[i] ? coff[i] + skc * 8 : (int)0x80000000;
+                    rn0[i] = __builtin_bit_cast(f32x4, __builtin_amdgcn_raw_buffer_load_b128(rsn, o, 0, 0));
+                    rn1[i] = __builtin_bit_cast(f32x4, __builtin_amdgcn_raw_buffer_load_b128(rsn, o + 16, 0, 0));
+                }
+            }
 #pragma unroll
             for (int i = 0; i < AL; ++i) {
                 const bool ok = (amask[i] >> tap) & 1u;
@@ -381,10 +401,18 @@
                     h16x4{(H16)rb[i].x, (H16)rb[i].y, (H16)rb[i].z, (H16)rb[i].w};
             return;
         }
-#pragma unroll
-        for (int i = 0; i < AL; ++i)
-            *reinterpret_cast<f32x4*>(&As[buf * BM * PITCH + (lrow + RPP * i) * PITCH + kq]) =
-                (LEAN || aok[i]) ? ra[i] : f32x4{0.f, 0.f, 0.f, 0.f};
+        if constexpr (NORM) {
+#pragma unroll
+            for (int i = 0; i < AL; ++i)
+                *reinterpret_cast<f32x4*>(&As[buf * BM * PITCH + (lrow + RPP * i) * PITCH + kq]) =
+                    f32x4{fmaxf(fmaf(ra[i].x, rn0[i].x, rn0[i].y), 0.f), fmaxf(fmaf(ra[i].y, rn0[i].z, rn0[i].w), 0.f),
+                          fmaxf(fmaf(ra[i].z, rn1[i].x, rn1[i].y), 0.f), fmaxf(fmaf(ra[i].w, rn1[i].z, rn1[i].w), 0.f)};
+        } else {
+#pragma unroll
+            for (int i = 0; i < AL; ++i)
+                *reinterpret_cast<f32x4*>(&As[buf * BM * PITCH + (lrow + RPP * i) * PITCH + kq]) =
+                    (LEAN || aok[i]) ? ra[i] : f32x4{0.f, 0.f, 0.f, 0.f};
+        }
 #pragma unroll
         for (int i = 0; i < BL; ++i)
             *reinterpret_cast<f32x4*>(&Bs[buf * BN * PITCH + (lrow + RPP * i) * PITCH + kq]) = rb[i];
@@ -899,6 +927,30 @@
 static void launch_igemm(bool lean, dim3 grid, dim3 block, hipStream_t st, const ConvP& p) {
     if (lean) hipLaunchKernelGGL((conv_igemm_f32<BM, BN, WM, WN, MODE, DT, true>), grid, block, 0, st, p);
     else hipLaunchKernelGGL((conv_igemm_f32<BM, BN, WM, WN, MODE, DT, false>), grid, block, 0, st, p);
+}
+
+template <int BM, int BN> constexpr bool igemm_norm_tile() { return (BM == 256 && BN == 32) || (BM == 64 && BN == 64) || (BM == 128 && BN == 64); }
+template <int BM, int BN, int WM, int WN, int MODE>
+static void launch_igemm_norm(dim3 grid, dim3 block, hipStream_t st, const ConvP& p) {
+    if constexpr (igemm_norm_tile<BM, BN>()) hipLaunchKernelGGL((conv_igemm_f32<BM, BN, WM, WN, MODE, 0, true, true>), grid, block, 0, st, p);
+}
+__global__ void igemm_norm_coef_kernel(const double* __restrict__ stats, const float* __restrict__ gamma, const float* __restrict__ beta, int G, int B, int C,
+                                       int groups, int param_gs, double n, float eps, float* __restrict__ coef) {
+    const long total = (long)G * B * C;
+    const int cpg = C / groups;
+    for (long i = blockIdx.x * (long)blockDim.x + threadIdx.x; i < total; i += (long)gridDim.x * blockDim.x) {
+        const int c = (int)(i % C);
+        const long gb = i / C;
+        const int g = (int)(gb / B);
+        const double* sb = stats + (gb * groups + c / cpg) * 2;
+        const double mean = sb[0] / n;
+        double var = sb[1] / n - mean * mean;
+        if (var < 0.0) var = 0.0;
+        const float rstd = (float)(1.0 / sqrt(var + (double)eps));
+        const float sc = rstd * gamma[g * param_gs + c];
+        coef[i * 2] = sc;
+        coef[i * 2 + 1] = beta[g * param_gs + c] - (float)mean * sc;
+    }
 }
 
 static bool lean_loader(ConvP& p) {
@@ -973,12 +1025,15 @@
         return gn_separate();
     }
     const bool lean = lean_loader(p);
+    const bool fold = p.n_stats != nullptr;
+    if (fold && !(lean && igemm_norm_tile<BM, BN>() && p.bf16 == 0 && !skip && p.n_coef && p.n_groups > 0 && p.Cin % p.n_groups == 0 && (long)p.B * p.Cin * 8 < 0x7fffff00L)) return 1;
     if (tune().persist && p.es != 2 && ((BM == 128 && BN == 128) || (tune().persist == 2 && (BM == BN || BM == 256))) && BN <= 128 && !skip && p.ws && conv_persistent_ok(p) &&
         (long)p.mtiles * p.ntiles * G >= tune().persist_min_tiles &&
         ((long)p.mtiles * p.ntiles * G >= 256L * (p.es == 2 ? 3 : BM == 64 ? 5 : 2) || nk >= tune().persist_min_nk)) {
         if (p.bf16 == 3 && (BM == 256 || (BM == 64 && nk <= 8))) exact_fallback();
         const int bpc = p.es == 2 ? 3 : BM == 64 ? 5 : 2;
         if (p.ws_floats >= conv_persistent_ws_floats(BM, BN, bpc)) {
+            if (fold) return 1;
             {
                 ProfScope prof(tag, conv_bytes, conv_flops, st);
                 int rc = 0;
@@ -1002,6 +1057,7 @@
             const double tail = (nk + kModel3.c) * BPC * ((double)nfull * G / slots) +
                                 launch_cost(rem * G, nk, rem_outputs, 1 << shift, BPC, kModel3);
             if (tail < 0.995 * whole || tune().tail_split == 2) {
+                if (fold) return 1;
                 p.nfull = (int)nfull;
                 p.tail_shift = shift;
                 p.kchunk = (nk + (1 << shift) - 1) >> shift;
@@ -1045,7 +1101,18 @@
         if (a > b || 8 * p.zx1 >= p.W) p.zones = a <= b ? 1 : 2;
         if (S > 1 && p.mtiles < 32) p.zones = 0;
     }
-    if (S > 1) {
+    if (fold) {
+        p.n_coef_bytes = p.B * p.Cin * 8;
+        {
+            ProfScope prof(tag, conv_bytes, conv_flops, st);
+            const long n = (long)G * p.B * p.Cin;
+            hipLaunchKernelGGL(igemm_norm_coef_kernel, dim3((unsigned)((n + 255) / 256)), dim3(256), 0, st, p.n_stats, p.n_gamma, p.n_beta, G, p.B, p.Cin, p.n_groups,
+                               p.n_param_gs, (double)p.ohw * (p.Cin / p.n_groups), p.n_eps, p.n_coef);
+            if (S > 1) launch_igemm_norm<BM, BN, WM, WN, 1>(dim3(p.mtiles * p.ntiles, S, G), block, st, p);
+            else launch_igemm_norm<BM, BN, WM, WN, 0>(dim3(p.mtiles * p.ntiles, 1, G), block, st, p);
+        }
+        if (S > 1) reduce(S);
+    } else if (S > 1) {
         {
             ProfScope prof(tag, conv_bytes, conv_flops, st);
             if (skip) launch_igemm<BM, BN, WM, WN, 4, 0>(lean, dim3(p.mtiles * p.ntiles, S, G), block, st, p);
@@ -1084,7 +1151,8 @@
         const int rc = launch_conv_h8(p, G, st);
         if (rc != 1) return rc;
     }
-    if (p.n_stats) return fail("conv: a launch that normalises its input needs the fp16 patch kernel (conv_h8.hip)");
+    if (p.n_stats && p.es == 2) return fail("conv: a launch that normalises its input needs the fp16 patch kernel (conv_h8.hip)");
+    if (p.n_stats && !(p.bf16 == 0 && p.kh == 1 && p.kw == 1 && p.stride == 1 && p.pad == 0 && !p.in2 && !p0.dil_g[0] && p.n_relu)) return 1;
     if (p0.dil_g[0]) {
         for (int g = 0; g < G; ++g) {
             ConvP q = p0;
diff --git a/quber_amd/csrc/elementwise.hip b/quber_amd/csrc/elementwise.hip
--- a/quber_amd/csrc/elementwise.hip
+++ b/quber_amd/csrc/elementwise.hip
@@ -469,7 +469,7 @@
     return 0;
 }
 
-template <class T, int CIN>
+template <class T, int CIN, bool NORM = false>
 __global__ void predictor_kernel(const PredHeads hs, int in_cs, float* __restrict__ q, int q_nch, int sm_cs, int B, int HW) {
     const int hd = blockIdx.y;
     const T* __restrict__ in = reinterpret_cast<const T*>(hs.in[hd]);
@@ -480,6 +480,24 @@
     __shared__ float ws[4 * CIN + 4];
     for (int i = threadIdx.x; i < cout * CIN; i += blockDim.x) ws[i] = w[i];
     if ((int)threadIdx.x < cout) ws[4 * CIN + threadIdx.x] = bias[threadIdx.x];
+    __shared__ float2 nc[NORM ? PRED_NORM_PAIRS : 1];
+    if constexpr (NORM) {
+        const double* __restrict__ stats = hs.n_stats[hd];
+        const float* __restrict__ gamma = hs.n_gamma[hd];
+        const float* __restrict__ beta = hs.n_beta[hd];
+        const int cpg = hs.n_cpg, groups = CIN / cpg;
+        const double n = (double)HW * cpg;
+        for (int i = threadIdx.x; i < B * CIN; i += blockDim.x) {
+            const int b = i / CIN, ch = i - b * CIN;
+            const double* sb = stats + ((long)b * groups + ch / cpg) * 2;
+            const double mean = sb[0] / n;
+            double var = sb[1] / n - mean * mean;
+            if (var < 0.0) var = 0.0;
+            const float rstd = (float)(1.0 / sqrt(var + (double)hs.n_eps));
+            const float sc = rstd * gamma[ch];
+            nc[i] = make_float2(sc, beta[ch] - (float)mean * sc);
+        }
+    }
     __syncthreads();
     const long total = (long)B * HW;
     for (long i = blockIdx.x * (long)blockDim.x + threadIdx.x; i < total; i += (long)gridDim.x * blockDim.x) {
@@ -491,6 +509,11 @@
             x[4 * j] = v.x; x[4 * j + 1] = v.y; x[4 * j + 2] = v.z; x[4 * j + 3] = v.w;
         }
         const long b = i / HW, pix = i - b * HW;
+        if constexpr (NORM) {
+            const float2* cb = &nc[(int)b * CIN];
+#pragma unroll
+            for (int j = 0; j < CIN; ++j) x[j] = fmaxf(fmaf(x[j], cb[j].x, cb[j].y), 0.f);
+        }
         float o[4];
         for (int k = 0; k < cout; ++k) {
             float a = 0.f;
@@ -526,6 +549,15 @@
     const long total = (long)B * H * W;
     ProfScope prof("predictor", total * ((double)es * C * hs.n + 4.0 * couts + (double)es * acts), 2.0 * total * C * couts, st);
     const dim3 grid(cap_grid(total, 256), hs.n), block(256);
+    if (hs.n_stats[0]) {
+        if (es != 4 || (long)B * C > PRED_NORM_PAIRS || hs.n_cpg < 1 || C % hs.n_cpg) return fail("predictor: the folded GroupNorm needs fp32 features and batch * channels <= 1024");
+        for (int j = 0; j < hs.n; ++j)
+            if (!hs.n_stats[j] || !hs.n_gamma[j] || !hs.n_beta[j]) return fail("predictor: the folded GroupNorm needs sums, gamma and beta of every head");
+        if (C == 32) hipLaunchKernelGGL((predictor_kernel<float, 32, true>), grid, block, 0, st, hs, in_cs, q, q_nch, sm_cs, B, H * W);
+        else hipLaunchKernelGGL((predictor_kernel<float, 64, true>), grid, block, 0, st, hs, in_cs, q, q_nch, sm_cs, B, H * W);
+        QB_CHECK(hipGetLastError());
+        return 0;
+    }
     if (es == 2 && C == 32) hipLaunchKernelGGL((predictor_kernel<half_t, 32>), grid, block, 0, st, hs, in_cs, q, q_nch, sm_cs, B, H * W);
     else if (es == 2) hipLaunchKernelGGL((predictor_kernel<half_t, 64>), grid, block, 0, st, hs, in_cs, q, q_nch, sm_cs, B, H * W);
     else if (C == 32) hipLaunchKernelGGL((predictor_kernel<float, 32>), grid, block, 0, st, hs, in_cs, q, q_nch, sm_cs, B, H * W);
diff --git a/quber_amd/csrc/plan.h b/quber_amd/csrc/plan.h
--- a/quber_amd/csrc/plan.h
+++ b/quber_amd/csrc/plan.h
@@ -13,6 +13,7 @@
 
 namespace quber {
 
+struct DeferredNorm;
 int* tuning_field(Tuning& t, int key);
 bool tuning_plan_time(int key);
 
@@ -65,6 +66,9 @@
     int* enc_bad = nullptr;
     std::vector<quber::Op> ops;
     std::map<std::string, quber::View> taps;
+    std::map<std::string, std::shared_ptr<quber::DeferredNorm>> tap_norms;
+    hipStream_t last_stream = nullptr;
+    int last_batch = 0;
     float* gauss = nullptr;
     void* enc_ws = nullptr;
     uint8_t* err_ws = nullptr;
@@ -149,7 +153,7 @@
     void conv(const std::vector<std::string>& names, const View& in, int cin_real, const View& out, int k, int stride, int pad, int dil, Affine af, const View* res, bool relu,
               const std::vector<int>& dil_g = {});
     void fuse_shortcut(const std::vector<std::string>& n3, const std::vector<std::string>& ns, const View& y, int mid, const View& x, int cin, int stride, const View& out);
-    void gn_relu(const std::vector<std::string>& names, const View& in, const View& out, bool single_consumer = false);
+    void gn_relu(const std::vector<std::string>& names, const View& in, const View& out, bool single_consumer = false, bool any_width = false);
     void op(std::function<int(int, hipStream_t)> f);
     void fork(int L);
     void back_to_main() { cur_lane = 0; }
diff --git a/quber_amd/csrc/plan.hip b/quber_amd/csrc/plan.hip
--- a/quber_amd/csrc/plan.hip
+++ b/quber_amd/csrc/plan.hip
@@ -185,6 +185,15 @@
         norm16->absorbed = true;
         coef16 = (float*)dalloc_bytes(sizeof(float) * (size_t)G * Bmax * Cin * 2);
     }
+    std::shared_ptr<DeferredNorm> norm1;
+    float* coef1 = nullptr;
+    if (!wino && !norm16 && aes == 4 && tune().fold_norm_1x1 && c->cfg.compute_dtype == 0 && pending_norm && pending_norm->out.p == in.p && pending_norm->C == Cin &&
+        pending_norm->G == G && k == 1 && stride == 1 && pad == 0 && dil_g.empty() && Cin % 32 == 0 && cin_real == Cin && !res && in.C == pending_norm->out.C &&
+        in.cs == pending_norm->out.cs && in.gs == pending_norm->out.gs && in.es == 4 && pending_norm->in.es == 4) {
+        norm1 = pending_norm;
+        norm1->absorbed = true;
+        coef1 = (float*)dalloc_bytes(sizeof(float) * (size_t)G * Bmax * Cin * 2);
+    }
     pending_norm.reset();
     if (wino) {
         WinoP probe = wq;
@@ -206,7 +215,7 @@
     auto fuse = std::make_shared<GnFuse>();
     last_conv = {fuse, out.p, G, Cout};
     const int L = cur_lane;
-    c->ops.push_back({[p, G, ctx, fuse, wq, wino, norm, norm16, coef16, L](int B, hipStream_t st) mutable {
+    c->ops.push_back({[p, G, ctx, fuse, wq, wino, norm, norm16, coef16, norm1, coef1, L](int B, hipStream_t st) mutable {
         const bool side = L && ctx->lane_now == L;
         float* const sk_ws = side ? ctx->lane_splitk_ws[L] : ctx->splitk_ws;
         const size_t sk_floats = side ? ctx->lane_splitk_floats : ctx->splitk_floats;
@@ -234,6 +243,16 @@
             q.n_groups = 32; q.n_param_gs = norm16->C; q.n_relu = 1; q.n_eps = 1e-5f;
             if (conv_h8_patch_takes(q, G, true)) return launch_conv(q, G, st);
             const int rc = launch_gn_apply(norm16->in, norm16->out, B, G, 32, norm16->stats, norm16->gamma, norm16->beta, norm16->C, 1e-5f, 1, st);
+            if (rc) return rc;
+        }
+        if (norm1) {
+            ConvP q = p;
+            q.in = norm1->in.p; q.in_cs = norm1->in.cs; q.in_gs = norm1->in.gs;
+            q.n_stats = norm1->stats; q.n_gamma = norm1->gamma; q.n_beta = norm1->beta; q.n_coef = coef1;
+            q.n_groups = 32; q.n_param_gs = norm1->C; q.n_relu = 1; q.n_eps = 1e-5f;
+            int rc = launch_conv(q, G, st);
+            if (rc != 1) return rc;
+            rc = launch_gn_apply(norm1->in, norm1->out, B, G, 32, norm1->stats, norm1->gamma, norm1->beta, norm1->C, 1e-5f, 1, st);
             if (rc) return rc;
         }
         return launch_conv(p, G, st);
@@ -316,7 +335,7 @@
     }, OP_CONV, op3.name + " + shortcut", op3.flops + ops.flops, 1});
 }
 
-void Builder::gn_relu(const std::vector<std::string>& names, const View& in, const View& out, bool single_consumer) {
+void Builder::gn_relu(const std::vector<std::string>& names, const View& in, const View& out, bool single_consumer, bool any_width) {
     const int G = (int)names.size(), C = in.C;
     std::vector<float> gamma, beta;
     for (int g = 0; g < G; ++g) {
@@ -338,7 +357,7 @@
         last_conv.fuse.reset();
     }
     std::shared_ptr<DeferredNorm> dn;
-    if (single_consumer && C % 32 == 0 && (C / 32) % 4 == 0) {
+    if (single_consumer && C % 32 == 0 && ((C / 32) % 4 == 0 || any_width)) {
         dn = std::make_shared<DeferredNorm>();
         dn->in = in; dn->out = out; dn->stats = stats; dn->gamma = dg; dn->beta = db; dn->C = C; dn->G = G;
     }
@@ -477,6 +496,7 @@
         const std::string n = "backbone.fusion_res" + std::to_string(s + 2) + ".";
         const int C = fch[s], fh = cat[s].H, fw = cat[s].W;
         View t = make(C, fh, fw), a = make(C, fh, fw);
+        std::shared_ptr<DeferredNorm> tap_norm;
         if (cf.fusion_add) {
             View ra = slice(cat[s], 0, C), rb = slice(cat[s], C, C);
             op([=](int B, hipStream_t st) { return launch_add_channels(ra, rb, a, B, st); });
@@ -487,9 +507,12 @@
         if (s != 3) {
             View b2 = make(C, fh, fw), t2 = make(C, fh, fw);
             View cur = a, nxt = b2, traw = t2, tprev = t;
+            const bool fold_last = tune().fold_norm_1x1 && aes == 4 && cf.compute_dtype == 0 && !cf.fusion_add;
             for (int i = 0; i < cf.backbone_fusion_layers; ++i) {
+                const bool last = i + 1 == cf.backbone_fusion_layers;
                 conv({n + "conv" + std::to_string(i)}, cur, C, traw, 3, 1, 1, 1, AF_BIAS, nullptr, false);
-                gn_relu({n + "gn" + std::to_string(i)}, traw, nxt, i + 1 < cf.backbone_fusion_layers);
+                gn_relu({n + "gn" + std::to_string(i)}, traw, nxt, !last || fold_last);
+                if (last && pending_norm) tap_norm = pending_norm;
                 std::swap(cur, nxt);
                 std::swap(traw, tprev);
             }
@@ -497,6 +520,7 @@
         }
         F[s] = a;
         if (!dry) c->taps["res" + std::to_string(s + 2)] = a;
+        if (!dry && tap_norm) c->tap_norms["res" + std::to_string(s + 2)] = tap_norm;
     };
     const std::string Hd = "ins_embed_head.";
     const int CD = cf.convs_dim, HC = cf.head_channels;
@@ -677,7 +701,10 @@
         conv(h0, xin, CD, g128, 3, 1, 1, 1, AF_NONE, nullptr, false);
         gn_relu(n0, g128, g128n, true);
         conv(h1, g128n, CD, g32, 3, 1, 1, 1, AF_NONE, nullptr, false);
-        gn_relu(n1, g32, feat);
+        const bool fold_pred = !next && tune().fold_norm_pred && aes == 4 && cf.compute_dtype == 0 && (HC == 32 || HC == 64) && (long)Bmax * HC <= PRED_NORM_PAIRS;
+        gn_relu(n1, g32, feat, fold_pred, true);
+        const std::shared_ptr<DeferredNorm> pn = fold_pred ? pending_norm : nullptr;
+        pending_norm.reset();
         int act_off = CD + (cf.fusion_feat ? HC * G : 0);
         PredHeads ph{};
         int ph_act_cs = 0;
@@ -688,6 +715,7 @@
             View in = feat;
             in.p = feat.at((long)j * feat.gs);
             if (!dry) c->taps[std::string("feat_") + HN[k]] = in;
+            if (!dry && pn) c->tap_norms[std::string("feat_") + HN[k]] = pn;
             float* act_dst = nullptr;
             int act_cs = 0;
             if (next && cf.fusion_pred) {
@@ -698,14 +726,26 @@
             if (dry || !pw || !pb) continue;
             const float* dw = upload(std::vector<float>(pw, pw + hch[k] * HC));
             const float* db = upload(std::vector<float>(pb, pb + hch[k]));
-            ph.in[ph.n] = in.p; ph.w[ph.n] = dw; ph.bias[ph.n] = db; ph.sm[ph.n] = act_dst; ph.cout[ph.n] = hch[k];
+            ph.in[ph.n] = pn ? (const void*)g32.at((long)j * g32.gs) : (const void*)in.p; ph.w[ph.n] = dw; ph.bias[ph.n] = db; ph.sm[ph.n] = act_dst; ph.cout[ph.n] = hch[k];
             ph.q_ch0[ph.n] = hplane[k]; ph.act[ph.n] = act_dst ? (k >= 3 ? 1 : 2) : 0;
             if (act_dst) ph_act_cs = act_cs;
             ++ph.n;
         }
         if (!dry && ph.n == G) {
-            const int fcs = feat.cs, fes = feat.es, fh = feat.H, fw = feat.W;
-            op([=](int B, hipStream_t st) { return launch_predictors(ph, HC, fcs, fes, fh, fw, q, planes, ph_act_cs, B, st); });
+            const int fcs = pn ? g32.cs : feat.cs, fes = feat.es, fh = feat.H, fw = feat.W;
+            if (pn) pn->absorbed = true;
+            op([=](int B, hipStream_t st) {
+                PredHeads hs = ph;
+                if (pn) {
+                    for (int j = 0; j < hs.n; ++j) {
+                        hs.n_stats[j] = pn->stats + (long)j * B * 32 * 2;
+                        hs.n_gamma[j] = pn->gamma + (long)j * HC;
+                        hs.n_beta[j] = pn->beta + (long)j * HC;
+                    }
+                    hs.n_cpg = HC / 32; hs.n_eps = 1e-5f;
+                }
+                return launch_predictors(hs, HC, fcs, fes, fh, fw, q, planes, ph_act_cs, B, st);
+            });
         }
     }
     quber_ctx* ctx = c;
diff --git a/quber_amd/csrc/runtime.hip b/quber_amd/csrc/runtime.hip
--- a/quber_amd/csrc/runtime.hip
+++ b/quber_amd/csrc/runtime.hip
@@ -25,7 +25,8 @@
     {37, &Tuning::x8_min_nk, false},            {38, &Tuning::h8_narrow, false},
     {39, &Tuning::h8_norm, true},               {41, &Tuning::aspp_lanes, true},
     {42, &Tuning::small_n_64, false},           {43, &Tuning::zone_cols, false},
-    {51, &Tuning::wino_pack, true},
+    {51, &Tuning::wino_pack, true},             {52, &Tuning::fold_norm_1x1, true},
+    {53, &Tuning::fold_norm_pred, true},
 };
 int* tuning_field(Tuning& t, int key) {
     for (const TuneKey& k : TUNE_KEYS)
```

Result: no change. 10260 refined masks/s (median of 6 runs) (+0.8%).
